# peterarmstrong/corda

Hardware: AMD Instinct MI355X
Metric: verified sigs/sec (whole node), Ed25519 + ECDSA-P256, at 1/2/4/8 MI355X (higher is better)
Workload: dtype u32

## Files before the change

corda_amd/csrc/cordagpu.cpp:

```cpp
#include <hip/hip_runtime.h>

#include <algorithm>
#include <atomic>
#include <chrono>
#include <cmath>
#include <cstdio>
#include <cstring>
#include <functional>
#include <initializer_list>
#include <memory>
#include <mutex>
#include <string>
#include <thread>
#include <vector>

#include "../../include/cordagpu.h"
#include "call_scope.h"
#include "engine.h"
#include "host_budget.h"
#include "host_pool.h"
#include "pool.h"
#include "rsa.h"
#include "table_budget.h"
#include "txsig_plan.h"
// ... 21 lines not shown
  snprintf(buf, sizeof buf, "%s: %s", where, hipGetErrorString(e));
  g_err = buf;
  return e == hipErrorOutOfMemory ? CG_ERR_NOMEM : CG_ERR_DEVICE;
}

#define HIP_TRY(expr, where)               \
  do {                                     \
    hipError_t _e = (expr);                \
    if (_e != hipSuccess) return hip_fail(_e, where); \
  } while (0)

bool env_flag(const char* name, bool dflt) {
  const char* v = getenv(name);
  return v ? (dflt ? v[0] != '0' : v[0] == '1') : dflt;
}
uint64_t env_u64(const char* name, uint64_t dflt) {
  const char* v = getenv(name);
  return v ? (uint64_t)strtoull(v, nullptr, 10) : dflt;
}

struct DevBuf {
  void* p = nullptr;
  size_t cap = 0;
  hipError_t ensure(size_t bytes) { return bytes <= cap ? hipSuccess : replace(bytes + bytes / 4 + 256); }
  hipError_t ensure_exact(size_t bytes) { return bytes <= cap ? hipSuccess : replace(bytes); }
  hipError_t replace(size_t want) {
    release();
    const hipError_t e = hipMalloc(&p, want);
    if (e == hipSuccess) cap = want;
    return e;
  }
  void release() {
    if (p) hipFree(p);
    p = nullptr;
    cap = 0;
  }
};

struct Need {
  DevBuf* buf;
  size_t bytes;
};
hipError_t ensure_all(std::initializer_list<Need> needs) {
  bool grow = false;
  for (const Need& n : needs) grow = grow || n.buf->cap < n.bytes;
  if (!grow) return hipSuccess;
  hipError_t e = hipDeviceSynchronize();
  for (const Need& n : needs)
    if (e == hipSuccess) e = n.buf->ensure(n.bytes);
  return e;
}

hipError_t stage(DevBuf& b, const void* src, size_t bytes, hipStream_t s, size_t room = 0) {
  hipError_t e = b.ensure(std::max<size_t>({bytes, room, 1}));
  if (e == hipSuccess && bytes) e = hipMemcpyAsync(b.p, src, bytes, hipMemcpyHostToDevice, s);
  return e;
}
size_t arena_room(uint64_t arena_len) { return ((arena_len + 3) & ~(uint64_t)3) + 16; }

struct HipStreams {
  using Stream = hipStream_t;
  using Event = hipEvent_t;
  using Error = hipError_t;
  static constexpr Error kOk = hipSuccess;
  Error record(Event e, Stream s) { return hipEventRecord(e, s); }
  Error wait(Stream s, Event e) { return hipStreamWaitEvent(s, e, 0); }
  Error sync(Stream s) { return hipStreamSynchronize(s); }
};

}

struct cg_ctx : cg::CallState<HipStreams> {
  int device = 0;
  uint64_t chunk = CG_DEFAULT_CHUNK_ITEMS;
  bool chunk_set = false;
  bool fault = false;
  cg::Fork fork = {{nullptr, nullptr, nullptr}, nullptr, {nullptr, nullptr, nullptr}, nullptr,
                   {nullptr, nullptr, nullptr}, nullptr};
  std::mutex mu;
  DevBuf keyprep, itemws, keys, items, arena, status, aux0, aux1, aux2;
  void* btab = nullptr;
  const cgt::EngineVariant* eng = nullptr;
  uint64_t tab_bytes = 0;
  DevBuf wide;
  bool rsa = false;
  DevBuf rsakeys, rsalist;
  uint32_t wide_max = cg::kKeyWideMax;
  DevBuf kcache;
  uint32_t wide_slots = 0;
  uint32_t wide_slots_max = cg::kKeyWideMax;
  uint32_t kc_bits = 32;
  bool kc_on = true;
  bool kc_dirty = true;
  bool kc_open = false;
  DevBuf txitems, msgs, tmpls, h_txs, h_comps, h_sigs, h_ids, h_txst;
  DevBuf sig12ws;
  DevBuf txvws, txvio;
  DevBuf ftxws;
  DevBuf signers, signws;
  uint32_t n_signers = 0;
  hipStream_t copy2 = nullptr;
  cg::CountScratch count_scratch;
  std::unique_ptr<cg::HostPool> hpool;
  uint32_t host_req = 0;
  uint32_t quota = 1;
  bool counted = false;
  std::vector<hipEvent_t> seg;
  hipEvent_t tev[4] = {};
  std::vector<hipEvent_t> segt;
  std::vector<hipEvent_t> segtab;
  hipEvent_t backt[2] = {nullptr, nullptr};
  std::vector<hipEvent_t> fbt;
  std::vector<double> fbh;
  bool htrace = false;
  cg::StageTimer timer;
};

namespace {

std::atomic<unsigned> g_live_ctx{0};

const cgt::EngineVariant* const kVariants[] = {&cg::variant(), &cg24::variant(), &cg22::variant()};
constexpr int kNumVariants = 3;

std::vector<cgb::TableSet> table_sets() {
  std::vector<cgb::TableSet> v;
  for (const cgt::EngineVariant* e : kVariants) v.push_back({e->fixed_base_bits, (uint64_t)e->btab_bytes()});
  return v;
}

struct SharedTables {
  int device;
  int variant;
  void* p;
  unsigned refs;
};
std::mutex g_tab_mu;
std::vector<SharedTables> g_tabs;

hipError_t acquire_tables(int device, hipStream_t s, uint64_t budget, void** out, int* variant) {
  std::lock_guard<std::mutex> g(g_tab_mu);
  const std::vector<cgb::TableSet> sets = table_sets();
  int held = -1;
  for (const SharedTables& t : g_tabs)
    if (t.device == device && (held < 0 || t.variant < held)) held = t.variant;
  size_t free_b = 0, total_b = 0;
  if (hipMemGetInfo(&free_b, &total_b) != hipSuccess) free_b = 0;
  const int pick = cgb::pick_tables(sets.data(), kNumVariants, budget, free_b, held);
  if (pick < 0) return hipErrorInvalidValue;
  for (SharedTables& t : g_tabs)
    if (t.device == device && t.variant == pick) {
      ++t.refs;
      *out = t.p;
      *variant = pick;
      return hipSuccess;
    }
  hipError_t e = hipErrorOutOfMemory;
  for (int v = pick; v < kNumVariants; ++v) {
    if (budget && sets[v].bytes > budget) continue;
    void* p = nullptr;
    e = hipMalloc(&p, sets[v].bytes);
    if (e == hipSuccess) {
      DevBuf scratch;
      e = scratch.ensure(kVariants[v]->btab_scratch_bytes());
      if (e == hipSuccess) e = kVariants[v]->upload_constants();
      if (e == hipSuccess) e = kVariants[v]->init_btab(p, scratch.p, s);
      if (e == hipSuccess) e = hipStreamSynchronize(s);
      scratch.release();
      if (e == hipSuccess) {
        g_tabs.push_back({device, v, p, 1u});
        *out = p;
        *variant = v;
        return hipSuccess;
      }
      hipFree(p);
    }
    (void)hipGetLastError();
    if (e != hipErrorOutOfMemory || budget) break;
  }
  return e;
}

void release_tables(int device, void* p) {
  std::lock_guard<std::mutex> g(g_tab_mu);
  for (size_t i = 0; i < g_tabs.size(); ++i)
    if (g_tabs[i].device == device && g_tabs[i].p == p) {
      if (--g_tabs[i].refs == 0) {
        hipSetDevice(device);
        hipFree(p);
        g_tabs.erase(g_tabs.begin() + (ptrdiff_t)i);
      }
      return;
    }
}

unsigned host_threads_of(cg_ctx* c, uint64_t n) {
  if (n < (1u << 16)) return 1;
  const unsigned nt = cg::host_threads_for(c->host_req, cg::host_threads_env(), c->quota, g_live_ctx.load());
  if (nt <= 1) c->hpool.reset();
  else if (!c->hpool || c->hpool->threads() != nt) c->hpool.reset(new cg::HostPool(nt - 1));
  return nt;
}

void host_par(cg_ctx* c, uint64_t m, const std::function<void(uint64_t)>& fn) {
  if (m > 1 && c->hpool) {
    c->hpool->run(m, fn);
  } else {
    for (uint64_t t = 0; t < m; ++t) fn(t);
  }
}

HipStreams g_hip;
struct Call : cg::CallScope<HipStreams> {
  Call(cg_ctx* c, Form form) : CallScope(g_hip, *c, form) {}
  hipError_t open(void* hip_stream = nullptr) { return CallScope::open((hipStream_t)hip_stream); }
};

int enter(cg_ctx* c, const char* fn) {
  if (c->fault) return fail(CG_ERR_DEVICE, "%s: device fault (injected by cg_pool_inject_fault)", fn);
  HIP_TRY(hipSetDevice(c->device), "hipSetDevice");
  return CG_OK;
}

uint64_t chunk_of(const cg_ctx* c, uint64_t n) { return cg::equal_chunk(c->chunk, n); }

size_t item_half_bytes(const cg_ctx* c, uint64_t ws_items) { return (c->eng->item_ws_bytes(ws_items) + 255) & ~(size_t)255; }
hipError_t ensure_rsa(cg_ctx* c, uint32_t n_keys, uint64_t n_items) {
  if (!c->rsa) return hipSuccess;
  return ensure_all({{&c->rsakeys, cg::rsa_keys_bytes(n_keys)}, {&c->rsalist, cg::rsa_list_bytes(n_items)}});
}
hipError_t rsa_keyprep(cg_ctx* c, const cg::VerifyReq& r, hipStream_t s) {
  if (!c->rsa) return hipSuccess;
  return cg::launch_rsa_keyprep(r, c->rsakeys.p, s);
}
hipError_t rsa_items(cg_ctx* c, const cg::VerifyReq& r, hipStream_t s) {
  if (!c->rsa || r.n_items == 0) return hipSuccess;
  return cg::launch_rsa_items(r, c->rsakeys.p, c->rsalist.p, s);
}

hipError_t ensure_ws(cg_ctx* c, uint32_t n_keys, uint64_t ws_items, uint64_t call_items = 0) {
  {
    const hipError_t re = ensure_rsa(c, n_keys, call_items > ws_items ? call_items : ws_items);
    if (re != hipSuccess) return re;
  }
  const uint32_t kmax = c->wide_slots_max;
  size_t wide = c->eng->wide_bytes(n_keys, call_items, kmax);
  const size_t items = item_half_bytes(c, ws_items) * (call_items > ws_items ? 2 : 1);
  if (c->keyprep.cap >= c->eng->keyprep_bytes(n_keys) && c->itemws.cap >= items && c->wide.cap >= wide) {
    c->wide_max = kmax;
    return hipSuccess;
  }
  uint32_t cap = kmax;
  if (wide > c->wide.cap) {
    size_t free_b = 0, total_b = 0;
    if (hipMemGetInfo(&free_b, &total_b) == hipSuccess) {
      const size_t need_other = (c->keyprep.cap >= c->eng->keyprep_bytes(n_keys) ? 0 : c->eng->keyprep_bytes(n_keys)) +
                                (c->itemws.cap >= items ? 0 : items);
      const size_t avail = free_b + c->wide.cap;
      const size_t spare = (size_t)1 << 30;
      if (wide + need_other + spare > avail) {
        const size_t room = avail > need_other + spare ? avail - need_other - spare : 0;
        cap = (uint32_t)std::min<size_t>(room / c->eng->wide_slot_bytes(), kmax);
        wide = c->eng->wide_bytes(n_keys, call_items, cap);
      }
    }
  }
  c->wide_max = cap;
  if (c->keyprep.cap >= c->eng->keyprep_bytes(n_keys) && c->itemws.cap >= items && c->wide.cap >= wide)
    return hipSuccess;
  hipError_t e = hipDeviceSynchronize();
  if (e == hipSuccess) e = c->keyprep.ensure(c->eng->keyprep_bytes(n_keys));
  if (e == hipSuccess) e = c->itemws.ensure(items);
  if (e == hipSuccess && wide > c->wide.cap) {
    e = c->wide.ensure_exact(wide);
    c->wide_slots = e == hipSuccess ? c->eng->wide_slots(n_keys, call_items, cap) : 0;
    c->kc_dirty = true;
    if (e == hipSuccess && c->kc_on) e = c->kcache.ensure(c->eng->key_cache_bytes(c->wide_slots));
  }
  return e;
}

cg::WidePool wide_for(cg_ctx* c, uint32_t n_keys, uint64_t n_items) {
  if (c->wide.cap < c->eng->wide_bytes(n_keys, n_items, c->wide_max)) return cg::WidePool{};
  cg::WidePool p = c->eng->make_wide_pool(c->wide.p, n_keys, n_items, c->wide_max, c->wide_slots);
  if (c->kc_on && p.cap_ed && c->kcache.p && c->kcache.cap >= c->eng->key_cache_bytes(p.slots)) {
    if (c->kc_open) {
      (void)hipDeviceSynchronize();
      c->kc_dirty = true;
    }
    p.cache = c->kcache.p;
    p.cache_bits = c->kc_bits;
    p.cache_dirty = c->kc_dirty;
    c->kc_dirty = false;
    c->kc_open = true;
  }
  static const uint32_t min_ed = (uint32_t)env_u64("CG_WIDE_MIN_USES_ED", 0);
  static const uint32_t min_ec = (uint32_t)env_u64("CG_WIDE_MIN_USES_EC", 0);
  if (min_ed) p.min_ed = min_ed;
  if (min_ec) p.min_ec = min_ec;
  return p;
}

struct ChunkOpts {
  const std::function<hipError_t(uint64_t, uint64_t, uint64_t)>* prepare = nullptr;
  const cg::KeyUses* uses = nullptr;
  bool prepare_blocks = false;
};

struct CallEng {
  using Error = hipError_t;
  static constexpr Error kOk = hipSuccess;
  using Clock = std::chrono::steady_clock;
  cg_ctx* c;
  const cg::VerifyReq& r;
  hipStream_t s;
  const cg::WidePool* wp;
  const std::vector<uint64_t>& bounds;
  const ChunkOpts& o;
  uint64_t half_bytes = 0;
  bool closes_cache = true;
  Clock::time_point h0;
  double prep_ms = 0, front_ms = 0, back_ms = 0;
  const char* where = "launch_items";

  static double ms(Clock::time_point a, Clock::time_point b) { return std::chrono::duration<double, std::milli>(b - a).count(); }
  cg::ItemArgs chunk(unsigned k, int half) const {
    cg::ItemArgs a = {r, c->keyprep.p, c->itemws.p, c->btab, wp};
    a.d_items = r.d_items + bounds[k];
    a.n_items = bounds[k + 1] - bounds[k];
    a.d_status = r.d_status + bounds[k];
    a.d_item_ws = (uint8_t*)c->itemws.p + (size_t)half * half_bytes;
    return a;
  }
  Error at(const char* w, Error e) {
    if (e != hipSuccess) where = w;
    return e;
  }
  Error keyprep() { return at("launch_keyprep", c->eng->launch_keyprep(r, c->keyprep.p, s, c->fork, wp, o.uses)); }
  Error rsa_keyprep() { return at("launch_rsa_keyprep", ::rsa_keyprep(c, r, s)); }
  Error key_tables() { return c->eng->launch_key_tables(c->fork, s); }
  Error prepare(unsigned k) {
    h0 = Clock::now();
    const hipError_t w = (*o.prepare)(k, bounds[k], bounds[k + 1] - bounds[k]);
    prep_ms = ms(h0, Clock::now());
    return w;
  }
  Error plan(unsigned k, int half) { return c->eng->launch_items_plan(chunk(k, half), s, c->fork); }
  Error front(unsigned k, int half, bool planned) {
    if (!o.prepare) h0 = Clock::now();
    const hipError_t e = c->eng->launch_items_front(chunk(k, half), s, c->fork, planned);
    front_ms = ms(h0, Clock::now());
    return e;
  }
  Error back(unsigned k, int half) {
    const auto h1 = Clock::now();
    if (k == 0 && c->htrace && c->backt[0]) {
      hipEventRecord(c->backt[0], s);
      hipStream_t t = c->copy2;
      for (int q = 0; q < 3; ++q) hipStreamWaitEvent(t, c->fork.ready[q], 0);
      hipEventRecord(c->backt[1], t);
    }
    c->fork.mark = c->htrace && 3 * (size_t)k + 2 < c->fbt.size() ? c->fbt[3 * k + 2] : nullptr;
    const hipError_t x = c->eng->launch_items_back(chunk(k, half), s, c->fork);
    c->fork.mark = nullptr;
    if (c->htrace && 3 * (size_t)k + 1 < c->fbt.size()) hipEventRecord(c->fbt[3 * k + 1], s);
    back_ms = ms(h1, Clock::now());
    return x;
  }
  void chunk_enqueued(unsigned k) const {
    if (c->htrace)
      fprintf(stderr, "[cg host] chunk %llu enqueue: front %.3f ms (prepare %.3f, with the copies), back %.3f ms\n",
              (unsigned long long)k, front_ms, prep_ms, back_ms);
  }
  Error rsa_pass(Error x) {
    if (x == hipSuccess && closes_cache) c->kc_open = false;
    return x != hipSuccess ? x : at("launch_rsa_items", rsa_items(c, r, s));
  }
  Error wait(cgs::Stream, cgs::Event e) {
    return at("hipStreamWaitEvent", hipStreamWaitEvent(s, c->fork.ready[e - cgs::EV_READY0], 0));
  }
};

hipError_t launch_chunked(cg_ctx* c, const cg::VerifyReq& r, const std::vector<uint64_t>& bounds, hipStream_t s,
                          const ChunkOpts& o) {
  if (r.n_items == 0) return hipSuccess;
  const cg::WidePool wp = wide_for(c, r.n_keys, r.n_items);
  const uint64_t per = cg::largest_chunk(bounds);
  CallEng g = {c, r, s, &wp, bounds, o};
  g.half_bytes = item_half_bytes(c, per);
  cgs::CallPlan p;
  p.chunks = (unsigned)(bounds.size() - 1);
  p.two = p.chunks > 1 && c->itemws.cap >= 2 * g.half_bytes;
  p.hook = o.prepare != nullptr;
  p.hook_blocks = o.prepare_blocks;
  return cgs::chunked(g, p);
}

using cg::Extent;

struct HostPlan {
  std::vector<uint64_t> first;
  std::vector<Extent> ext;
  Extent keys, win;
};

void plan_host(cg_ctx* c, const cg_key* keys, uint32_t n_keys, const cg_item* items, uint64_t n_items,
               uint64_t arena_len, uint64_t per, HostPlan& P) {
  for (uint32_t k = 0; k < n_keys; ++k) P.keys.add(keys[k].off, keys[k].len, arena_len);
  const uint64_t nch = (n_items + per - 1) / per;
  P.first.resize(nch + 1);
  for (uint64_t k = 0; k <= nch; ++k) P.first[k] = n_items * k / nch;
  P.ext.assign(nch, Extent());
  auto scan = [&](uint64_t k) {
    Extent x;
    for (uint64_t i = P.first[k]; i < P.first[k + 1]; ++i) {
      x.add(items[i].sig_off, items[i].sig_len, arena_len);
      x.add(items[i].msg_off, items[i].msg_len, arena_len);
    }
    P.ext[k] = x;
  };
  host_threads_of(c, n_items);
  host_par(c, nch, scan);
  P.win = P.keys;
  for (const Extent& e : P.ext) P.win.merge(e);
  if (P.win.empty()) P.win.lo = P.win.hi = 0;
  P.win.lo &= ~(uint64_t)15;
}

hipError_t copy_missing(cg::Resident& have, const Extent& e, const uint8_t* arena, uint8_t* dwin, uint64_t win_lo,
                        hipStream_t s) {
  for (const auto& g : have.missing(e)) {
    hipError_t r = hipMemcpyAsync(dwin + (g.first - win_lo), arena + g.first, g.second - g.first,
                                  hipMemcpyHostToDevice, s);
    if (r != hipSuccess) return r;
  }
  return hipSuccess;
}

hipError_t ensure_events(std::vector<hipEvent_t>& v, uint64_t n) {
  while (v.size() < n) {
    hipEvent_t e;
    const hipError_t r = hipEventCreateWithFlags(&e, hipEventDisableTiming);
    if (r != hipSuccess) return r;
    v.push_back(e);
  }
  return hipSuccess;
}

void fill_stats(cg_ctx* c, cg_stats* stats, uint64_t n_items, uint32_t n_keys, double ms_key_prep,
                std::chrono::steady_clock::time_point t0) {
  if (!stats) return;
  float a = 0, b = 0, d = 0;
  hipEventElapsedTime(&a, c->tev[0], c->tev[1]);
  hipEventElapsedTime(&b, c->tev[1], c->tev[2]);
  hipEventElapsedTime(&d, c->tev[2], c->tev[3]);
  stats->n_items = n_items;
  stats->n_keys = n_keys;
  stats->ms_h2d = a;
  stats->ms_key_prep = ms_key_prep;
  stats->ms_verify = b;
  stats->ms_d2h = d;
  stats->ms_total = std::chrono::duration<double, std::milli>(std::chrono::steady_clock::now() - t0).count();
}

int verify_host_locked(cg_ctx* c, const cg::VerifyReq& h, cg_stats* stats) {
  const auto t0 = std::chrono::steady_clock::now();
  if (const int rc = enter(c, "cg_verify_batch")) return rc;
  const uint32_t n_keys = h.n_keys;
  const uint64_t n_items = h.n_items;
  const uint64_t pipe = c->chunk < CG_PIPELINE_CHUNK_ITEMS ? c->chunk : CG_PIPELINE_CHUNK_ITEMS;
  HostPlan P;
  plan_host(c, h.d_keys, n_keys, h.d_items, n_items, h.arena_len, pipe, P);
  const uint64_t nch = P.ext.size();
  const uint64_t per_max = (n_items + nch - 1) / nch;
  HIP_TRY(c->keys.ensure(sizeof(cg_key) * (n_keys ? n_keys : 1)), "hipMalloc(keys)");
  HIP_TRY(c->items.ensure(sizeof(cg_item) * n_items), "hipMalloc(items)");
  HIP_TRY(c->arena.ensure((P.win.hi - P.win.lo) + 16), "hipMalloc(arena window)");
  HIP_TRY(c->status.ensure(n_items), "hipMalloc(status)");
  HIP_TRY(ensure_ws(c, n_keys, per_max, n_items), "hipMalloc(workspace)");
  HIP_TRY(ensure_events(c->seg, nch), "hipEventCreate");
  hipStream_t s = c->stream;
  uint8_t* dwin = (uint8_t*)c->arena.p;
  Call call(c, Call::kHost);
  HIP_TRY(call.open(), "hipStreamWaitEvent");
  HIP_TRY(hipEventRecord(c->tev[0], s), "hipEventRecord");
  HIP_TRY(hipStreamWaitEvent(c->copy, c->tev[0], 0), "hipStreamWaitEvent");
  cg::Resident have;
  if (n_keys)
    HIP_TRY(hipMemcpyAsync(c->keys.p, h.d_keys, sizeof(cg_key) * n_keys, hipMemcpyHostToDevice, c->copy), "H2D keys");
  HIP_TRY(copy_missing(have, P.keys, h.d_arena, dwin, P.win.lo, c->copy), "H2D key bytes");
  HIP_TRY(hipMemcpyAsync(c->items.p, h.d_items, sizeof(cg_item) * n_items, hipMemcpyHostToDevice, c->copy), "H2D items");
  HIP_TRY(hipEventRecord(c->seg[0], c->copy), "hipEventRecord");
  HIP_TRY(hipStreamWaitEvent(s, c->seg[0], 0), "hipStreamWaitEvent");
  cg::VerifyReq d = h;
  d.d_keys = (const cg_key*)c->keys.p;
  d.d_items = (const cg_item*)c->items.p;
  d.d_arena = dwin - P.win.lo;
  d.d_status = (uint8_t*)c->status.p;
  const cg::WidePool wp = wide_for(c, n_keys, n_items);
  HIP_TRY(c->eng->launch_keyprep(d, c->keyprep.p, s, c->fork, &wp, nullptr), "launch_keyprep");
  cg::ItemArgs a = {d, c->keyprep.p, c->itemws.p, c->btab, &wp};
  HIP_TRY(rsa_keyprep(c, d, s), "launch_rsa_keyprep");
  for (uint64_t k = 0; k < nch; ++k) {
    HIP_TRY(copy_missing(have, P.ext[k], h.d_arena, dwin, P.win.lo, c->copy), "H2D arena");
    HIP_TRY(hipEventRecord(c->seg[k], c->copy), "hipEventRecord");
    HIP_TRY(hipStreamWaitEvent(s, c->seg[k], 0), "hipStreamWaitEvent");
    if (k == 0) HIP_TRY(hipEventRecord(c->tev[1], s), "hipEventRecord");
    a.d_items = d.d_items + P.first[k];
    a.n_items = P.first[k + 1] - P.first[k];
    a.d_status = d.d_status + P.first[k];
    HIP_TRY(c->eng->launch_items(a, s, c->fork), "launch_items");
  }
  c->kc_open = false;
  HIP_TRY(rsa_items(c, d, s), "launch_rsa_items");
  HIP_TRY(hipEventRecord(c->tev[2], s), "hipEventRecord");
  HIP_TRY(hipMemcpyAsync(h.d_status, d.d_status, n_items, hipMemcpyDeviceToHost, s), "D2H status");
  HIP_TRY(hipEventRecord(c->tev[3], s), "hipEventRecord");
  HIP_TRY(call.close(), "hipEventRecord");
  HIP_TRY(hipStreamSynchronize(s), "hipStreamSynchronize");
  fill_stats(c, stats, n_items, n_keys, 0, t0);
  return CG_OK;
}

int batch_args(const char* fn, const cg::VerifyReq& r, bool host) {
  if (r.n_items && (!r.d_items || !r.d_status)) return fail(CG_ERR_ARG, "%s: NULL buffer", fn);
  if (host && r.n_keys && !r.d_keys) return fail(CG_ERR_ARG, "%s: keys is NULL", fn);
  if (host && r.arena_len && !r.d_arena) return fail(CG_ERR_ARG, "%s: arena is NULL", fn);
  if (r.mode > CG_MODE_ISVALID) return fail(CG_ERR_ARG, "%s: bad mode", fn);
  return CG_OK;
}

}

extern "C" {

int cg_abi_version(void) { return CG_ABI_VERSION; }

const char* cg_build_info(void) {
  return "corda_amd libcordagpu: HIP kernels for gfx950 (Ed25519 i2p-0.2.0 semantics, ECDSA BC-1.57 semantics, "
         "SHA-256/512, Merkle tx ids)";
}

int cg_device_count(void) {
  int n = 0;
  if (hipGetDeviceCount(&n) != hipSuccess) return 0;
  return n;
}

const char* cg_last_error(void) { return g_err.c_str(); }

namespace {
struct HostRange {
  uint64_t lo, hi;
};
std::mutex g_reg_mu;
std::vector<HostRange> g_reg;
}

int cg_host_register(const void* p, uint64_t len) {
  if (!p || !len) return fail(CG_ERR_ARG, "cg_host_register: NULL pointer or empty range");
  const uint64_t lo = (uint64_t)(uintptr_t)p, hi = lo + len;
  if (hi < lo) return fail(CG_ERR_ARG, "cg_host_register: range wraps the address space");
  std::lock_guard<std::mutex> g(g_reg_mu);
  for (const HostRange& r : g_reg)
    if (lo < r.hi && r.lo < hi) return fail(CG_ERR_ARG, "cg_host_register: range overlaps a registered one");
  HIP_TRY(hipHostRegister(const_cast<void*>(p), (size_t)len, hipHostRegisterPortable), "hipHostRegister");
  g_reg.push_back({lo, hi});
  return CG_OK;
}

int cg_host_unregister(const void* p) {
  const uint64_t lo = (uint64_t)(uintptr_t)p;
  std::lock_guard<std::mutex> g(g_reg_mu);
  for (size_t i = 0; i < g_reg.size(); ++i) {
    if (g_reg[i].lo != lo) continue;
    g_reg.erase(g_reg.begin() + (ptrdiff_t)i);
    HIP_TRY(hipHostUnregister(const_cast<void*>(p)), "hipHostUnregister");
    return CG_OK;
  }
  return fail(CG_ERR_ARG, "cg_host_unregister: pointer was not registered");
}

int cg_host_register_advised(uint32_t contexts_per_node) { return cg::host_register_advised(contexts_per_node) ? 1 : 0; }

int cg_host_registered(const void* p, uint64_t len) {
  const uint64_t lo = (uint64_t)(uintptr_t)p, hi = lo + len;
  std::lock_guard<std::mutex> g(g_reg_mu);
  for (const HostRange& r : g_reg)
    if (lo >= r.lo && hi <= r.hi && hi >= lo) return 1;
  return 0;
}

static_assert(sizeof(cg_config) == 56, "cg_config is 56 bytes in ABI v2");
static_assert(sizeof(cg_item) == 32 && sizeof(cg_key) == 16 && sizeof(cg_txsig) == 24 && sizeof(cg_txsig_packed) == 12,
              "ABI struct sizes");

int cg_open(cg_ctx** out, const cg_config* cfg) {
  if (!out) return fail(CG_ERR_ARG, "cg_open: out is NULL");
  *out = nullptr;
  if (cfg && (cfg->reserved0 || cfg->reserved1))
    return fail(CG_ERR_ARG, "cg_open: cg_config.reserved must be 0 (ABI v2: 56-byte cg_config)");
  const uint64_t tab_budget = cfg && cfg->table_bytes_max ? cfg->table_bytes_max
                                                          : cgb::table_bytes_env(getenv("CG_TABLE_BYTES_MAX"));
  if (tab_budget && tab_budget < table_sets().back().bytes) {
    char m[160];
    snprintf(m, sizeof m, "cg_open: table_bytes_max %llu is below the smallest fixed-base tables (%llu bytes, radix 2^%u)",
             (unsigned long long)tab_budget, (unsigned long long)table_sets().back().bytes, table_sets().back().bits);
    return fail(CG_ERR_ARG, "%s", m);
  }
  if (cfg && (cfg->flags & ~(CG_FLAG_STAGE_TIMING | CG_FLAG_RSA | CG_FLAG_NO_KEY_CACHE))) return fail(CG_ERR_ARG, "cg_open: unknown cg_config.flags bits");
  int dev = cfg ? cfg->device : 0;
  int n = 0;
  HIP_TRY(hipGetDeviceCount(&n), "hipGetDeviceCount");
  if (dev < 0 || dev >= n) return fail(CG_ERR_ARG, "cg_open: device ordinal out of range");
  HIP_TRY(hipSetDevice(dev), "hipSetDevice");
  hipDeviceProp_t prop;
  HIP_TRY(hipGetDeviceProperties(&prop, dev), "hipGetDeviceProperties");
  if (strncmp(prop.gcnArchName, "gfx950", 6) != 0)
    return fail(CG_ERR_DEVICE, "cg_open: kernels are built for gfx950, device is %s", prop.gcnArchName);
  cg_ctx* c = new cg_ctx();
  c->device = dev;
  c->host_req = cfg ? cfg->host_threads : 0u;
  c->quota = cg::cpu_quota();
  if (cfg && cfg->chunk_items) {
    c->chunk = cfg->chunk_items;
    c->chunk_set = true;
  }
  if (cfg && (cfg->flags & CG_FLAG_STAGE_TIMING)) c->fork.timer = &c->timer;
  c->rsa = cfg && (cfg->flags & CG_FLAG_RSA);
  c->kc_on = !(cfg && (cfg->flags & CG_FLAG_NO_KEY_CACHE)) && env_flag("CG_KEY_CACHE", true);
  c->wide_slots_max = (uint32_t)std::min<uint64_t>(env_u64("CG_TEST_WIDE_SLOTS", cg::kKeyWideMax), cg::kKeyWideMax);
  c->kc_bits = (uint32_t)std::min<uint64_t>(env_u64("CG_TEST_KEY_CACHE_BITS", 32), 32);
  hipError_t e = hipStreamCreateWithFlags(&c->stream, hipStreamNonBlocking);
  if (e != hipSuccess) {
    delete c;
    return hip_fail(e, "hipStreamCreate");
  }
  for (int k = 0; k < 3 && e == hipSuccess; ++k) e = hipStreamCreateWithFlags(&c->fork.side[k], hipStreamNonBlocking);
  if (e == hipSuccess) e = hipEventCreateWithFlags(&c->fork.start, hipEventDisableTiming);
  for (int k = 0; k < 3 && e == hipSuccess; ++k) e = hipEventCreateWithFlags(&c->fork.ready[k], hipEventDisableTiming);
  for (int k = 0; k < 3 && e == hipSuccess; ++k) e = hipEventCreateWithFlags(&c->fork.row0[k], hipEventDisableTiming);
  if (e == hipSuccess) e = hipEventCreateWithFlags(&c->fork.front, hipEventDisableTiming);
  if (e == hipSuccess) e = hipEventCreateWithFlags(&c->fork.planned, hipEventDisableTiming);
  if (e == hipSuccess) e = hipEventCreateWithFlags(&c->fork.ec_front_go, hipEventDisableTiming);
  for (int k = 0; k < 2 && e == hipSuccess; ++k)
    e = hipEventCreateWithFlags(&c->fork.ec_front_done[k], hipEventDisableTiming);
  {
    hipDeviceProp_t prop;
    const bool own = hipGetDeviceProperties(&prop, c->device) == hipSuccess && prop.multiProcessorCount > 0;
    std::vector<uint32_t> mask(own ? (prop.multiProcessorCount + 31) / 32 : 0, 0u);
    for (int cu = 0; own && cu < prop.multiProcessorCount; ++cu) mask[cu / 32] |= 1u << (cu % 32);
    for (hipStream_t* cs : {&c->copy, &c->copy2})
      if (e == hipSuccess)
        e = own ? hipExtStreamCreateWithCUMask(cs, (uint32_t)mask.size(), mask.data())
                : hipStreamCreateWithFlags(cs, hipStreamNonBlocking);
  }
  for (int k = 0; k < 4 && e == hipSuccess; ++k) e = hipEventCreate(&c->tev[k]);
  if (e == hipSuccess) e = hipEventCreateWithFlags(&c->done, hipEventDisableTiming);
  if (e == hipSuccess) e = hipEventCreateWithFlags(&c->bridge, hipEventDisableTiming);
  c->bridged = env_flag("CG_STREAM_BRIDGE", true);
  int var = 0;
  if (e == hipSuccess) e = acquire_tables(c->device, c->stream, tab_budget, &c->btab, &var);
  if (e == hipSuccess) {
    c->eng = kVariants[var];
    c->tab_bytes = c->eng->btab_bytes();
    e = c->eng->upload_constants();
  }
  if (e == hipSuccess) e = hipStreamSynchronize(c->stream);
  if (e != hipSuccess) {
    const int rc = hip_fail(e, "side streams / upload_constants / fixed-base tables");
    cg_close(c);
    return rc;
  }
  c->counted = true;
  ++g_live_ctx;
  *out = c;
  return CG_OK;
}

static void signers_drop(cg_ctx* c) {
  c->n_signers = 0;
  if (!c->signers.p) return;
  (void)hipDeviceSynchronize();
  (void)hipMemset(c->signers.p, 0, c->signers.cap);
  (void)hipDeviceSynchronize();
  c->signers.release();
}

void cg_close(cg_ctx* c) {
  if (!c) return;
  if (c->counted) --g_live_ctx;
  hipSetDevice(c->device);
  if (c->stream) hipStreamSynchronize(c->stream);
  signers_drop(c);
  c->signws.release();
// ... 198 lines not shown
  HIP_TRY(cgs::verify_items(items, (unsigned)(bounds.size() - 1)), items.where);
  HIP_TRY(call.close(), "hipEventRecord");
  return CG_OK;
}

int cg_verify_batch(cg_ctx* c, const cg_key* keys, uint32_t n_keys, const cg_item* items, uint64_t n_items,
                    const uint8_t* arena, uint64_t arena_len, uint32_t mode, uint8_t* status_out,
                    cg_stats* stats) {
  if (!c) return fail(CG_ERR_ARG, "cg_verify_batch: ctx is NULL");
  const cg::VerifyReq h = {keys, n_keys, items, n_items, arena, arena_len, mode, status_out};
  if (const int a = batch_args("cg_verify_batch", h, true)) return a;
  if (n_items) memset(status_out, CG_NOT_RUN, n_items);
  if (n_items == 0) return CG_OK;
  std::lock_guard<std::mutex> g(c->mu);
  const int rc = verify_host_locked(c, h, stats);
  if (rc != CG_OK) memset(status_out, CG_NOT_RUN, n_items);
  return rc;
}

int cg_sha256_batch_device(cg_ctx* c, const cg_span* d_spans, uint64_t n, const uint8_t* d_arena,
                           uint64_t arena_len, uint8_t* d_digests, void* hip_stream) {
  if (!c) return fail(CG_ERR_ARG, "cg_sha256_batch_device: ctx is NULL");
  std::lock_guard<std::mutex> g(c->mu);
  if (const int rc = enter(c, "cg_sha256_batch_device")) return rc;
  Call call(c, Call::kDevice);
  HIP_TRY(call.open(hip_stream), "hipStreamWaitEvent");
  HIP_TRY(cg::launch_sha256(d_spans, n, d_arena, arena_len, d_digests, call.stream()), "launch_sha256");
  HIP_TRY(call.close(), "hipEventRecord");
  return CG_OK;
}

static int hash_batch(cg_ctx* c, const cg_span* spans, uint64_t n, const uint8_t* arena, uint64_t arena_len,
                      uint8_t* out, int which) {
  if (!c) return fail(CG_ERR_ARG, "hash batch: ctx is NULL");
  if (n && (!spans || !out)) return fail(CG_ERR_ARG, "hash batch: NULL buffer");
  if (n == 0) return CG_OK;
  const size_t dlen = which == 256 ? 32 : 64;
  std::lock_guard<std::mutex> g(c->mu);
  if (const int rc = enter(c, which == 256 ? "cg_sha256_batch" : "cg_sha512_batch")) return rc;
  hipStream_t s = c->stream;
  Call call(c, Call::kHost);
  HIP_TRY(call.open(), "hipStreamWaitEvent");
  HIP_TRY(stage(c->items, spans, sizeof(cg_span) * n, s), "H2D spans");
  HIP_TRY(stage(c->arena, arena, arena_len, s, arena_room(arena_len)), "H2D arena");
  HIP_TRY(c->aux0.ensure(dlen * n), "hipMalloc(digests)");
  HIP_TRY((which == 256 ? cg::launch_sha256 : cg::launch_sha512)((const cg_span*)c->items.p, n, (const uint8_t*)c->arena.p,
                                                                 arena_len, (uint8_t*)c->aux0.p, s), "launch_sha");
  HIP_TRY(hipMemcpyAsync(out, c->aux0.p, dlen * n, hipMemcpyDeviceToHost, s), "D2H digests");
  HIP_TRY(call.close(), "hipEventRecord");
  HIP_TRY(hipStreamSynchronize(s), "hipStreamSynchronize");
  return CG_OK;
}

int cg_sha256_batch(cg_ctx* c, const cg_span* spans, uint64_t n, const uint8_t* arena, uint64_t arena_len,
                    uint8_t* out) {
  return hash_batch(c, spans, n, arena, arena_len, out, 256);
}
int cg_sha512_batch(cg_ctx* c, const cg_span* spans, uint64_t n, const uint8_t* arena, uint64_t arena_len,
                    uint8_t* out) {
  return hash_batch(c, spans, n, arena, arena_len, out, 512);
}

int cg_tx_ids_device(cg_ctx* c, const cg_tx* d_txs, uint64_t n_tx, const cg_component* d_comps, uint64_t n_comps,
                     const uint8_t* d_arena, uint64_t arena_len, uint8_t* d_ids, uint8_t* d_status,
                     void* hip_stream) {
  if (!c) return fail(CG_ERR_ARG, "cg_tx_ids_device: ctx is NULL");
  std::lock_guard<std::mutex> g(c->mu);
  if (const int rc = enter(c, "cg_tx_ids_device")) return rc;
  HIP_TRY(ensure_all({{&c->aux2, cg::tx_ws_bytes(n_comps)}}), "hipMalloc(leaf ws)");
  Call call(c, Call::kDevice);
  HIP_TRY(call.open(hip_stream), "hipStreamWaitEvent");
  HIP_TRY(cg::launch_tx_ids(d_txs, n_tx, d_comps, n_comps, d_arena, arena_len, d_ids, d_status,
                            (uint8_t*)c->aux2.p, call.stream()), "launch_tx_ids");
  HIP_TRY(call.close(), "hipEventRecord");
  return CG_OK;
}

int cg_tx_ids(cg_ctx* c, const cg_tx* txs, uint64_t n_tx, const cg_component* comps, uint64_t n_comps,
              const uint8_t* arena, uint64_t arena_len, uint8_t* ids_out, uint8_t* status_out) {
  if (!c) return fail(CG_ERR_ARG, "cg_tx_ids: ctx is NULL");
  if (n_tx && (!txs || !ids_out || !status_out)) return fail(CG_ERR_ARG, "cg_tx_ids: NULL buffer");
  if (n_tx == 0) return CG_OK;
  std::lock_guard<std::mutex> g(c->mu);
  if (const int rc = enter(c, "cg_tx_ids")) return rc;
  hipStream_t s = c->stream;
  Call call(c, Call::kHost);
  HIP_TRY(call.open(), "hipStreamWaitEvent");
  HIP_TRY(stage(c->keys, txs, sizeof(cg_tx) * n_tx, s), "H2D txs");
  HIP_TRY(stage(c->items, comps, sizeof(cg_component) * n_comps, s), "H2D comps");
  HIP_TRY(stage(c->arena, arena, arena_len, s, arena_room(arena_len)), "H2D arena");
  HIP_TRY(c->aux0.ensure(32 * n_tx), "hipMalloc(ids)");
  HIP_TRY(c->status.ensure(n_tx), "hipMalloc(status)");
  HIP_TRY(c->aux2.ensure(cg::tx_ws_bytes(n_comps)), "hipMalloc(leaf ws)");
  HIP_TRY(cg::launch_tx_ids((const cg_tx*)c->keys.p, n_tx, (const cg_component*)c->items.p, n_comps,
                            (const uint8_t*)c->arena.p, arena_len, (uint8_t*)c->aux0.p, (uint8_t*)c->status.p,
                            (uint8_t*)c->aux2.p, s), "launch_tx_ids");
  HIP_TRY(hipMemcpyAsync(ids_out, c->aux0.p, 32 * n_tx, hipMemcpyDeviceToHost, s), "D2H ids");
  HIP_TRY(hipMemcpyAsync(status_out, c->status.p, n_tx, hipMemcpyDeviceToHost, s), "D2H status");
  HIP_TRY(call.close(), "hipEventRecord");
  HIP_TRY(hipStreamSynchronize(s), "hipStreamSynchronize");
  return CG_OK;
}

int cg_merkle_roots(cg_ctx* c, const uint8_t* leaves, const uint64_t* first, const uint32_t* count, uint64_t n,
                    uint8_t* roots_out, uint8_t* status_out) {
  if (!c) return fail(CG_ERR_ARG, "cg_merkle_roots: ctx is NULL");
  if (n && (!first || !count || !roots_out || !status_out)) return fail(CG_ERR_ARG, "cg_merkle_roots: NULL buffer");
  if (n == 0) return CG_OK;
  uint64_t total = 0, ws = 0;
  std::vector<uint64_t> wsoff(n);
  for (uint64_t j = 0; j < n; ++j) {
    if (first[j] + count[j] > total) total = first[j] + count[j];
    wsoff[j] = ws;
    ws += count[j];
  }
  std::lock_guard<std::mutex> g(c->mu);
  if (const int rc = enter(c, "cg_merkle_roots")) return rc;
  hipStream_t s = c->stream;
  Call call(c, Call::kHost);
  HIP_TRY(call.open(), "hipStreamWaitEvent");
  HIP_TRY(stage(c->arena, leaves, 32 * total, s), "H2D leaves");
  HIP_TRY(stage(c->keys, first, 8 * n, s), "H2D first");
  HIP_TRY(stage(c->items, count, 4 * n, s), "H2D count");
  HIP_TRY(stage(c->aux2, wsoff.data(), 8 * n, s), "H2D wsoff");
  HIP_TRY(c->aux0.ensure(32 * n), "hipMalloc(roots)");
  HIP_TRY(c->status.ensure(n), "hipMalloc(status)");
  HIP_TRY(c->aux1.ensure(32 * (ws ? ws : 1)), "hipMalloc(ws)");
  HIP_TRY(cg::launch_merkle_roots((const uint8_t*)c->arena.p, (const uint64_t*)c->keys.p, (const uint32_t*)c->items.p,
                                  n, (uint8_t*)c->aux0.p, (uint8_t*)c->status.p, (uint8_t*)c->aux1.p,
                                  (const uint64_t*)c->aux2.p, s),
          "launch_merkle_roots");
  HIP_TRY(hipMemcpyAsync(roots_out, c->aux0.p, 32 * n, hipMemcpyDeviceToHost, s), "D2H roots");
  HIP_TRY(hipMemcpyAsync(status_out, c->status.p, n, hipMemcpyDeviceToHost, s), "D2H status");
  HIP_TRY(call.close(), "hipEventRecord");
  HIP_TRY(hipStreamSynchronize(s), "hipStreamSynchronize");
  return CG_OK;
}

static uint64_t tmpl_slot(const cg_signable_tmpl* tmpls, uint32_t n_tmpls) {
  uint64_t maxlen = 0;
  for (uint32_t k = 0; k < n_tmpls; ++k) {
    const uint64_t l = (uint64_t)tmpls[k].prefix_len + 32u + tmpls[k].suffix_len;
    if (l > maxlen) maxlen = l;
  }
  const uint64_t slot = (maxlen + 15) & ~(uint64_t)15;
  return slot ? slot : 16;
}

struct TxnReq {
  const cg_tx* txs;
  uint64_t n_tx;
  const cg_component* comps;
  uint64_t n_comps;
  const cg_key* keys;
  uint32_t n_keys;
  const cg_txsig* sigs;
  uint64_t n_sigs;
  const cg_signable_tmpl* tmpls;
  uint32_t n_tmpls;
  const uint8_t* arena;
  uint64_t arena_len;
  uint32_t mode;
  uint8_t *ids, *tx_status, *sig_status;
};
static int txn_args(const char* fn, const TxnReq& q, bool host) {
  if (q.n_tx && (!q.txs || !q.ids || !q.tx_status)) return fail(CG_ERR_ARG, "%s: NULL tx buffer", fn);
  if (q.n_sigs && (!q.sigs || !q.sig_status)) return fail(CG_ERR_ARG, "%s: NULL sig buffer", fn);
  if (host && q.n_comps && !q.comps) return fail(CG_ERR_ARG, "%s: comps is NULL", fn);
  if (host && q.n_keys && !q.keys) return fail(CG_ERR_ARG, "%s: keys is NULL", fn);
  if (q.n_tmpls && !q.tmpls) return fail(CG_ERR_ARG, "%s: templates is NULL", fn);
  if (host && q.arena_len && !q.arena) return fail(CG_ERR_ARG, "%s: arena is NULL", fn);
  if (q.mode > CG_MODE_ISVALID) return fail(CG_ERR_ARG, "%s: bad mode", fn);
  return CG_OK;
}

static int verify_transactions_locked(cg_ctx* c, const TxnReq& d, hipStream_t s) {
  const uint64_t slot = tmpl_slot(d.tmpls, d.n_tmpls), msgs_len = cg::tx_msgs_head(d.n_tmpls, slot);
  HIP_TRY(ensure_all({{&c->aux2, cg::tx_ws_bytes(d.n_comps)},
                      {&c->txitems, sizeof(cg_item) * (d.n_sigs ? d.n_sigs : 1)},
                      {&c->msgs, msgs_len ? msgs_len : 16},
                      {&c->tmpls, sizeof(cg_signable_tmpl) * (d.n_tmpls ? d.n_tmpls : 1)}}),
          "hipMalloc(transaction workspace)");
  HIP_TRY(ensure_ws(c, d.n_keys, chunk_of(c, d.n_sigs), d.n_sigs), "hipMalloc(workspace)");
  if (d.n_tmpls)
    HIP_TRY(hipMemcpyAsync(c->tmpls.p, d.tmpls, sizeof(cg_signable_tmpl) * d.n_tmpls, hipMemcpyHostToDevice, s),
            "H2D templates");
  HIP_TRY(cg::launch_tx_ids(d.txs, d.n_tx, d.comps, d.n_comps, d.arena, d.arena_len, d.ids, d.tx_status,
                            (uint8_t*)c->aux2.p, s), "launch_tx_ids");
  if (d.n_sigs) {
    HIP_TRY(cg::launch_tx_sig_items(d.sigs, d.n_sigs, (const cg_signable_tmpl*)c->tmpls.p, d.n_tmpls, d.tx_status,
                                    d.n_tx, d.ids, d.arena, d.arena_len, slot, (cg_item*)c->txitems.p,
                                    (uint8_t*)c->msgs.p, s),
            "launch_tx_sig_items");
    const cg::VerifyReq r = {d.keys, d.n_keys, (const cg_item*)c->txitems.p, d.n_sigs, d.arena, d.arena_len, d.mode,
                             d.sig_status, (const uint8_t*)c->msgs.p, msgs_len};
    HIP_TRY(launch_chunked(c, r, cg::equal_bounds(d.n_sigs, chunk_of(c, d.n_sigs)), s, ChunkOpts{}), "launch_verify");
  }
  return CG_OK;
}

int cg_verify_transactions_device(cg_ctx* c, const cg_tx* d_txs, uint64_t n_tx, const cg_component* d_comps,
                                  uint64_t n_comps, const cg_key* d_keys, uint32_t n_keys, const cg_txsig* d_sigs,
                                  uint64_t n_sigs, const cg_signable_tmpl* tmpls, uint32_t n_tmpls,
                                  const uint8_t* d_arena, uint64_t arena_len, uint32_t mode, uint8_t* d_ids,
                                  uint8_t* d_tx_status, uint8_t* d_sig_status, void* hip_stream) {
  if (!c) return fail(CG_ERR_ARG, "cg_verify_transactions_device: ctx is NULL");
  const TxnReq d = {d_txs, n_tx,  d_comps,   n_comps, d_keys, n_keys, d_sigs,      n_sigs,
                    tmpls, n_tmpls, d_arena, arena_len, mode, d_ids,  d_tx_status, d_sig_status};
  if (const int a = txn_args("cg_verify_transactions_device", d, false)) return a;
  std::lock_guard<std::mutex> g(c->mu);
  if (const int rc = enter(c, "cg_verify_transactions_device")) return rc;
  Call call(c, Call::kDevice);
  HIP_TRY(call.open(hip_stream), "hipStreamWaitEvent");
  if (const int rc = verify_transactions_locked(c, d, call.stream())) return rc;
  HIP_TRY(call.close(), "hipEventRecord");
  return CG_OK;
}

static int verify_transactions_host_locked(cg_ctx* c, const TxnReq& h) {
  if (const int rc = enter(c, "cg_verify_transactions")) return rc;
  hipStream_t s = c->stream;
  Call call(c, Call::kHost);
  HIP_TRY(call.open(), "hipStreamWaitEvent");
  HIP_TRY(stage(c->h_txs, h.txs, sizeof(cg_tx) * h.n_tx, s), "H2D txs");
  HIP_TRY(stage(c->h_comps, h.comps, sizeof(cg_component) * h.n_comps, s), "H2D comps");
  HIP_TRY(stage(c->keys, h.keys, sizeof(cg_key) * h.n_keys, s), "H2D keys");
  HIP_TRY(stage(c->h_sigs, h.sigs, sizeof(cg_txsig) * h.n_sigs, s), "H2D sigs");
  HIP_TRY(stage(c->arena, h.arena, h.arena_len, s, arena_room(h.arena_len)), "H2D arena");
  HIP_TRY(c->h_ids.ensure(32 * (h.n_tx ? h.n_tx : 1)), "hipMalloc(ids)");
  HIP_TRY(c->h_txst.ensure(h.n_tx ? h.n_tx : 1), "hipMalloc(tx status)");
  HIP_TRY(c->status.ensure(h.n_sigs ? h.n_sigs : 1), "hipMalloc(sig status)");
  TxnReq d = h;
  d.txs = (const cg_tx*)c->h_txs.p;
  d.comps = (const cg_component*)c->h_comps.p;
  d.keys = (const cg_key*)c->keys.p;
  d.sigs = (const cg_txsig*)c->h_sigs.p;
  d.arena = (const uint8_t*)c->arena.p;
  d.ids = (uint8_t*)c->h_ids.p;
  d.tx_status = (uint8_t*)c->h_txst.p;
  d.sig_status = (uint8_t*)c->status.p;
  if (const int rc = verify_transactions_locked(c, d, s)) return rc;
  if (h.n_tx) {
    HIP_TRY(hipMemcpyAsync(h.ids, d.ids, 32 * h.n_tx, hipMemcpyDeviceToHost, s), "D2H ids");
    HIP_TRY(hipMemcpyAsync(h.tx_status, d.tx_status, h.n_tx, hipMemcpyDeviceToHost, s), "D2H tx status");
  }
  if (h.n_sigs) HIP_TRY(hipMemcpyAsync(h.sig_status, d.sig_status, h.n_sigs, hipMemcpyDeviceToHost, s), "D2H sig status");
  HIP_TRY(call.close(), "hipEventRecord");
  HIP_TRY(hipStreamSynchronize(s), "hipStreamSynchronize");
  return CG_OK;
}

int cg_verify_transactions(cg_ctx* c, const cg_tx* txs, uint64_t n_tx, const cg_component* comps, uint64_t n_comps,
                           const cg_key* keys, uint32_t n_keys, const cg_txsig* sigs, uint64_t n_sigs,
                           const cg_signable_tmpl* tmpls, uint32_t n_tmpls, const uint8_t* arena,
                           uint64_t arena_len, uint32_t mode, uint8_t* ids_out, uint8_t* tx_status_out,
                           uint8_t* sig_status_out) {
  if (!c) return fail(CG_ERR_ARG, "cg_verify_transactions: ctx is NULL");
  const TxnReq h = {txs,   n_tx,    comps, n_comps,   keys, n_keys,  sigs,          n_sigs,
                    tmpls, n_tmpls, arena, arena_len, mode, ids_out, tx_status_out, sig_status_out};
  if (const int a = txn_args("cg_verify_transactions", h, true)) return a;
  for (uint64_t i = 0; i < n_sigs; ++i) sig_status_out[i] = CG_NOT_RUN;
  if (n_tx == 0 && n_sigs == 0) return CG_OK;
  std::lock_guard<std::mutex> g(c->mu);
  return verify_transactions_host_locked(c, h);
}

static hipError_t ensure_txsig_ws(cg_ctx* c, uint64_t n_sigs, uint32_t n_tmpls, uint64_t slot) {
  return ensure_all({{&c->txitems, sizeof(cg_item) * (n_sigs ? n_sigs : 1)},
                     {&c->msgs, cg::tx_msgs_head(n_tmpls, slot)},
                     {&c->tmpls, sizeof(cg_signable_tmpl) * (n_tmpls ? n_tmpls : 1)}});
}

struct TxsigReq {
  const cg_key* keys;
  uint32_t n_keys;
  const uint8_t* ids;
  uint64_t n_ids;
  cg::SigTable sigs;
  uint64_t n_sigs;
  const cg_signable_tmpl* tmpls;
  uint32_t n_tmpls;
  const uint8_t* arena;
  uint64_t arena_len;
  uint32_t mode;
  uint8_t* status;
  const uint8_t* sig_bytes = nullptr;
  uint64_t sig_bytes_off = 0, sig_bytes_len = 0;
};

struct TxsigSched {
  const std::vector<uint64_t>& bounds;
  cg::KeyUses uses;
  const std::function<hipError_t(uint64_t, uint64_t, uint64_t)>* ready = nullptr;
  const std::vector<uint64_t>* chunk_base = nullptr;
  const uint64_t* d_bases = nullptr;
};
static hipError_t launch_txsig(cg_ctx* c, const TxsigReq& d, uint64_t slot, const TxsigSched& p, hipStream_t s) {
  if (d.n_sigs == 0) return hipSuccess;
  hipError_t e = hipSuccess;
  const cg_signable_tmpl* dt = (const cg_signable_tmpl*)c->tmpls.p;
  if (d.n_tmpls) e = hipMemcpyAsync(c->tmpls.p, d.tmpls, sizeof(cg_signable_tmpl) * d.n_tmpls, hipMemcpyHostToDevice, s);
  if (e == hipSuccess)
    e = cg::launch_tx_sig_templates(dt, d.n_tmpls, d.arena, d.arena_len, slot, d.ids, d.n_ids, (uint8_t*)c->msgs.p, s);
  const std::function<hipError_t(uint64_t, uint64_t, uint64_t)> prepare = [&](uint64_t k, uint64_t first,
                                                                               uint64_t cnt) {
    hipError_t r = p.ready ? (*p.ready)(k, first, cnt) : hipSuccess;
    if (r == hipSuccess && d.sigs.packed())
      r = cg::launch_tx_sig12_range((const cg_txsig_packed*)d.sigs.p, first, cnt, d.sig_bytes_off, d.sig_bytes_len,
                                    p.chunk_base ? (*p.chunk_base)[k] : 0, p.d_bases, dt, d.n_tmpls, d.n_ids,
                                    d.arena_len, (cg_item*)c->txitems.p, c->sig12ws.p, s);
    else if (r == hipSuccess)
      r = cg::launch_tx_sig_range((const cg_txsig*)d.sigs.p, first, cnt, dt, d.n_tmpls, nullptr, d.n_ids, d.ids,
                                  d.arena_len, slot, (cg_item*)c->txitems.p, (uint8_t*)c->msgs.p, s);
    return r;
  };
  const cg::VerifyReq r = {d.keys, d.n_keys, (const cg_item*)c->txitems.p, d.n_sigs, d.arena, d.arena_len, d.mode,
                           d.status, (const uint8_t*)c->msgs.p, cg::tx_msgs_head(d.n_tmpls, slot)};
  if (e == hipSuccess) e = launch_chunked(c, r, p.bounds, s, ChunkOpts{&prepare, &p.uses, p.ready != nullptr});
  return e;
}

static double ms_since(std::chrono::steady_clock::time_point t0) {
  return std::chrono::duration<double, std::milli>(std::chrono::steady_clock::now() - t0).count();
}

struct HostTrace {
  cg_ctx* c;
  const std::chrono::steady_clock::time_point t0;
  const bool on;
  std::vector<double> ht;

  double ms() const { return on ? ms_since(t0) : 0; }
  hipError_t begin(uint64_t nch) {
    c->htrace = on;
    if (!on) return hipSuccess;
    hipError_t e = hipSuccess;
    for (int q = 0; q < 2 && e == hipSuccess; ++q)
      if (!c->backt[q]) e = hipEventCreate(&c->backt[q]);
    while (e == hipSuccess && c->fbt.size() < 3 * nch) {
      hipEvent_t ev;
      e = hipEventCreate(&ev);
      if (e == hipSuccess) c->fbt.push_back(ev);
    }
    c->fbh.assign(nch, 0.0);
    ht.assign(3 * nch, 0.0);
    return e;
  }
  void table_staged(uint64_t k, double h0, double h1) {
    if (!on) return;
    ht[3 * k] = h0;
    ht[3 * k + 1] = h1 - h0;
    ht[3 * k + 2] = ms() - h1;
  }
  hipError_t bytes_staged(uint64_t k, hipStream_t cs, double h2, double h3, double table_mb, const Extent& ek) {
    if (!on) return hipSuccess;
    hipError_t e = hipSuccess;
    while (c->segt.size() <= k) {
      hipEvent_t ev;
      if (hipEventCreate(&ev) != hipSuccess) break;
      c->segt.push_back(ev);
    }
    if (c->segt.size() > k) e = hipEventRecord(c->segt[k], cs);
    fprintf(stderr, "[cg host] chunk %llu at %.3f: scan %.3f sigs %.3f (%.1f MB) ids %.3f arena %.3f (%.1f MB) ms\n",
            (unsigned long long)k, ht[3 * k], ht[3 * k + 1], ht[3 * k + 2], table_mb, h3 - h2, ms() - h3,
            ek.empty() ? 0.0 : (ek.hi - ek.lo) / 1e6);
    return e;
  }
  hipError_t front_reached(uint64_t k, hipStream_t s) {
    if (!on || 3 * k >= c->fbt.size()) return hipSuccess;
    c->fbh[k] = ms();
    return hipEventRecord(c->fbt[3 * k], s);
  }
  void report(uint64_t nch, double h_enq) {
    if (!on) return;
    fprintf(stderr, "[cg host] enqueued at %.3f, done at %.3f ms; copies landed (device ms after the call's first event):",
            h_enq, ms());
    for (uint64_t k = 0; k < nch && k < c->segt.size(); ++k) {
      float t = 0;
      hipEventElapsedTime(&t, c->tev[0], c->segt[k]);
      fprintf(stderr, " %.3f", t);
    }
    float t = 0, f0 = 0, tb = 0;
    hipEventElapsedTime(&t, c->tev[0], c->tev[2]);
    hipEventElapsedTime(&f0, c->tev[0], c->backt[0]);
    hipEventElapsedTime(&tb, c->tev[0], c->backt[1]);
    fprintf(stderr, "; chunk 0 front done %.3f, tables built %.3f, verify done %.3f\n", f0, tb, t);
    for (uint64_t k = 0; k < nch && 3 * k + 2 < c->fbt.size(); ++k) {
      float fs = 0, be = 0, bj = 0;
      hipEventElapsedTime(&fs, c->tev[0], c->fbt[3 * k]);
      hipEventElapsedTime(&bj, c->tev[0], c->fbt[3 * k + 2]);
      hipEventElapsedTime(&be, c->tev[0], c->fbt[3 * k + 1]);
      fprintf(stderr, "[cg host] chunk %llu: front enqueued (host) %.3f, front reached (device) %.3f, back's "
              "kernels done %.3f, joins done %.3f\n", (unsigned long long)k, c->fbh[k], fs, bj, be);
    }
  }
};

struct TxsigFeed {
  cg_ctx* c;
  HostTrace& tr;
  const std::vector<uint64_t>& bounds;
  const TxsigReq& h;
  const TxsigReq& d;
  const uint64_t nt;
  const cg::ParFor& par;
  std::vector<Extent> ext_e, ext_i;
  std::vector<uint64_t> cbase;
  cg::Resident have, have_ids, have_sig;
  hipError_t copy_err = hipSuccess;
  uint64_t mid_k = 0;
  const std::function<hipError_t()> mid_hook = [this] { return mid(); };
  const std::function<hipError_t(uint64_t, uint64_t, uint64_t)> before_hook = [this](uint64_t k, uint64_t, uint64_t) {
    return before(k);
  };

  TxsigFeed(cg_ctx* ctx, HostTrace& trace, const std::vector<uint64_t>& b, const TxsigReq& host, const TxsigReq& dev,
            uint64_t threads, const cg::ParFor& pf)
      : c(ctx), tr(trace), bounds(b), h(host), d(dev), nt(threads), par(pf), ext_e(b.size() - 1),
        ext_i(b.size() - 1), cbase(b.size(), 0) {}
  TxsigFeed(const TxsigFeed&) = delete;
  ~TxsigFeed() { c->fork.mid_front = nullptr; }

  hipError_t copy_table(uint64_t k) {
    const uint64_t first = bounds[k], cnt = bounds[k + 1] - bounds[k];
    const double h0 = tr.ms();
    const cg::ChunkScan x = cg::with_records(h.sigs, [&](auto* recs) {
      return cg::scan_chunk(recs, first, first + cnt, h.n_ids, d.arena_len, nt, par);
    });
    ext_e[k] = x.sig;
    ext_i[k] = x.ids;
    if (h.sigs.packed()) {
      cbase[k + 1] = cbase[k] + x.span;
      ext_e[k] = Extent();
      ext_e[k].add(cbase[k], x.span, h.sig_bytes_len);
    }
    const double h1 = tr.ms();
    const hipError_t e = hipMemcpyAsync((uint8_t*)c->h_sigs.p + (size_t)h.sigs.stride * first, h.sigs.from(first).p,
                                        (size_t)h.sigs.stride * cnt, hipMemcpyHostToDevice, c->copy);
    tr.table_staged(k, h0, h1);
    return e;
  }
  hipError_t copy_bytes(uint64_t k) {
    const Extent& ek = ext_e[k];
    uint8_t* dwin = (uint8_t*)c->arena.p;
    const double h2 = tr.ms();
    hipError_t e = copy_missing(have_ids, ext_i[k], h.ids, (uint8_t*)c->h_ids.p, 0, c->copy);
    const double h3 = tr.ms();
    if (e == hipSuccess && h.sigs.packed()) e = copy_missing(have_sig, ek, h.sig_bytes, dwin + d.sig_bytes_off, 0, c->copy);
    else if (e == hipSuccess) e = copy_missing(have, ek, h.arena, dwin, 0, c->copy);
    if (e == hipSuccess) e = hipEventRecord(c->seg[k], c->copy);
    if (e == hipSuccess) e = tr.bytes_staged(k, c->copy, h2, h3, h.sigs.stride * (bounds[k + 1] - bounds[k]) / 1e6, ek);
    return e;
  }
  hipError_t mid() {
    c->fork.mid_front = nullptr;
    const uint64_t k = mid_k;
    hipStream_t s = c->stream;
    hipError_t e = copy_bytes(k);
    if (e == hipSuccess) e = hipStreamWaitEvent(s, c->seg[k], 0);
    if (e == hipSuccess) e = tr.front_reached(k, s);
    if (e == hipSuccess && k == 0) e = hipEventRecord(c->tev[1], s);
    if (e != hipSuccess) copy_err = e;
    return e;
  }
  hipError_t before(uint64_t k) {
    hipStream_t s = c->stream;
    hipError_t e = c->fork.mid_front ? mid() : hipSuccess;
    if (e == hipSuccess) e = copy_table(k);
    if (e == hipSuccess) e = hipEventRecord(c->segtab[k], c->copy);
    if (e == hipSuccess) e = hipStreamWaitEvent(s, c->segtab[k], 0);
    if (e == hipSuccess) {
      mid_k = k;
      c->fork.mid_front = &mid_hook;
    }
    if (e != hipSuccess) copy_err = e;
    return e;
  }
};

static hipError_t txv_stage(cg_ctx* c, const cg::TxvSet& h, uint32_t n_keys, cg::TxvSet* d) {
  auto up = [](size_t x) { return (x + 15) & ~(size_t)15; };
  const size_t o_checks = 0, o_nodes = o_checks + up(sizeof(cg_tx_check) * h.n_tx),
               o_verd = o_nodes + up(sizeof(cg_req_node) * h.n_nodes),
               o_reqs = o_verd + up(sizeof(cg_tx_verdict) * h.n_tx),
               o_class = o_reqs + up(sizeof(uint32_t) * h.n_reqs),
               o_rst = o_class + up(h.key_class ? sizeof(uint32_t) * n_keys : 0), need = o_rst + up(h.n_reqs) + 16;
  const hipError_t e = ensure_all({{&c->txvws, cg::tx_verdicts_ws_bytes(h.n_tx)}, {&c->txvio, need}});
  if (e != hipSuccess) return e;
  uint8_t* b = (uint8_t*)c->txvio.p;
  *d = h;
  d->checks = (cg_tx_check*)(b + o_checks);
  d->nodes = (cg_req_node*)(b + o_nodes);
  d->verdicts = (cg_tx_verdict*)(b + o_verd);
  d->reqs = (uint32_t*)(b + o_reqs);
  d->key_class = h.key_class ? (uint32_t*)(b + o_class) : nullptr;
  d->req_status = b + o_rst;
  return hipSuccess;
}
static hipError_t txv_upload(const cg::TxvSet& h, uint32_t n_keys, const cg::TxvSet& d, hipStream_t s) {
  hipError_t e = hipSuccess;
  if (h.n_tx) e = hipMemcpyAsync((void*)d.checks, h.checks, sizeof(cg_tx_check) * h.n_tx, hipMemcpyHostToDevice, s);
  if (e == hipSuccess && h.n_nodes)
    e = hipMemcpyAsync((void*)d.nodes, h.nodes, sizeof(cg_req_node) * h.n_nodes, hipMemcpyHostToDevice, s);
  if (e == hipSuccess && h.n_reqs)
    e = hipMemcpyAsync((void*)d.reqs, h.reqs, sizeof(uint32_t) * h.n_reqs, hipMemcpyHostToDevice, s);
  if (e == hipSuccess && h.key_class && n_keys)
    e = hipMemcpyAsync((void*)d.key_class, h.key_class, sizeof(uint32_t) * n_keys, hipMemcpyHostToDevice, s);
  return e;
}
static hipError_t txv_download(const cg::TxvSet& h, const cg::TxvSet& d, hipStream_t s) {
  hipError_t e = hipSuccess;
  if (h.n_tx) e = hipMemcpyAsync(h.verdicts, d.verdicts, sizeof(cg_tx_verdict) * h.n_tx, hipMemcpyDeviceToHost, s);
  if (e == hipSuccess && h.n_reqs) e = hipMemcpyAsync(h.req_status, d.req_status, h.n_reqs, hipMemcpyDeviceToHost, s);
  return e;
}
static void txv_fill_not_run(const cg::TxvSet& h) {
  for (uint64_t t = 0; t < h.n_tx; ++t) h.verdicts[t] = cg_tx_verdict{0xFFFFFFFFu, CG_NOT_RUN, CG_TXV_SPAN_BAD, 0};
  if (h.n_reqs) memset(h.req_status, CG_REQ_HOST, h.n_reqs);
}

static int verify_txsig_host_locked(cg_ctx* c, const TxsigReq& q, cg_stats* stats, const cg::TxvSet* txv) {
  const auto t0 = std::chrono::steady_clock::now();
  const bool packed = q.sigs.packed();
  const uint32_t n_keys = q.n_keys, n_tmpls = q.n_tmpls;
  const uint64_t n_sigs = q.n_sigs, n_ids = q.n_ids;
  TxsigReq h = q;
  TxsigReq d = q;
  d.sig_bytes_off = packed ? ((q.arena_len + 15) & ~(uint64_t)15) : 0;
  if (packed) d.arena_len = d.sig_bytes_off + q.sig_bytes_len;
  std::vector<cg_key> keys_fix;
  std::vector<cg_signable_tmpl> tmpls_fix;
  if (packed) {
    cg::txsig_packed_fixup(q.keys, n_keys, q.tmpls, n_tmpls, q.arena_len, keys_fix, tmpls_fix);
    if (!keys_fix.empty()) h.keys = keys_fix.data();
    if (!tmpls_fix.empty()) h.tmpls = tmpls_fix.data();
  }
  d.tmpls = h.tmpls;
  if (const int rc = enter(c, "cg_verify_tx_signatures")) return rc;
  static const uint64_t first_div = env_u64("CG_TXSIG_FIRST_DIV", cg::kTxsigFirstDiv);
  const std::vector<uint64_t> bounds = cg::txsig_bounds(n_sigs, c->chunk, c->chunk_set, first_div);
  const uint64_t nch = bounds.size() - 1, per = cg::largest_chunk(bounds);
  const Extent head = cg::txsig_head_extent(h.keys, n_keys, h.tmpls, n_tmpls, q.arena_len);
  const uint64_t nt = host_threads_of(c, n_sigs);
  const cg::ParFor par = [c](uint64_t m, const std::function<void(uint64_t)>& fn) { host_par(c, m, fn); };
  std::vector<uint32_t> counts(n_keys ? n_keys : 1, 0u);
  const uint64_t slot = tmpl_slot(h.tmpls, n_tmpls);
  HIP_TRY(c->keys.ensure(sizeof(cg_key) * (n_keys ? n_keys : 1)), "hipMalloc(keys)");
  HIP_TRY(c->h_sigs.ensure(q.sigs.stride * n_sigs), "hipMalloc(sigs)");
  if (packed) HIP_TRY(c->sig12ws.ensure(cg::tx_sig12_scratch_bytes(per)), "hipMalloc(signature offsets)");
  HIP_TRY(c->aux1.ensure(sizeof(uint32_t) * counts.size()), "hipMalloc(key use counts)");
  HIP_TRY(c->h_ids.ensure(32 * (n_ids ? n_ids : 1)), "hipMalloc(ids)");
  HIP_TRY(c->arena.ensure(d.arena_len + 16), "hipMalloc(arena window)");
  HIP_TRY(c->status.ensure(n_sigs), "hipMalloc(status)");
  HIP_TRY(ensure_txsig_ws(c, n_sigs, n_tmpls, slot), "hipMalloc(tx signature workspace)");
  HIP_TRY(ensure_ws(c, n_keys, per, n_sigs), "hipMalloc(workspace)");
  cg::TxvSet txd;
  if (txv) HIP_TRY(txv_stage(c, *txv, n_keys, &txd), "hipMalloc(verdict tables)");
  HIP_TRY(ensure_events(c->seg, nch + 1), "hipEventCreate");
  HIP_TRY(ensure_events(c->segtab, nch), "hipEventCreate");
  static const bool htrace = env_flag("CG_HOST_TRACE", false);
  HostTrace tr{c, t0, htrace, {}};
  HIP_TRY(tr.begin(nch), "hipEventCreate");
  hipStream_t s = c->stream;
  d.keys = (const cg_key*)c->keys.p;
  d.ids = (const uint8_t*)c->h_ids.p;
  d.sigs.p = c->h_sigs.p;
  d.arena = (const uint8_t*)c->arena.p;
  d.status = (uint8_t*)c->status.p;
  Call call(c, Call::kHost);
  HIP_TRY(call.open(), "hipStreamWaitEvent");
  HIP_TRY(hipEventRecord(c->tev[0], s), "hipEventRecord");
  HIP_TRY(hipStreamWaitEvent(c->copy, c->tev[0], 0), "hipStreamWaitEvent");
  TxsigFeed feed(c, tr, bounds, h, d, nt, par);
  if (n_keys)
    HIP_TRY(hipMemcpyAsync(c->keys.p, h.keys, sizeof(cg_key) * n_keys, hipMemcpyHostToDevice, c->copy), "H2D keys");
  HIP_TRY(copy_missing(feed.have, head, h.arena, (uint8_t*)c->arena.p, 0, c->copy), "H2D key / template bytes");
  {
    static const uint32_t S_env = cg::sample_override((uint32_t)env_u64("CG_TXSIG_SAMPLE", 0));
    static const uint32_t B = cg::sample_block((uint32_t)env_u64("CG_TXSIG_SAMPLE_BLOCK", cg::kTxsigSampleBlock));
    const uint32_t S = cg::sample_rate(S_env, n_sigs, n_keys);
    const cg::WidePool thr = c->eng->make_wide_pool(nullptr, n_keys, n_sigs, cg::kKeyWideMax, 0);
    cg::with_records(h.sigs, [&](auto* recs) {
      cg::key_use_counts(recs, n_sigs, h.keys, n_keys, nt, par, S, B, thr.min_ed, thr.min_ec, c->count_scratch,
                         counts.data());
    });
  }
  const double ms_plan = ms_since(t0);
  HIP_TRY(hipMemcpyAsync(c->aux1.p, counts.data(), sizeof(uint32_t) * counts.size(), hipMemcpyHostToDevice, c->copy),
          "H2D key use counts");
  HIP_TRY(hipEventRecord(c->seg[nch], c->copy), "hipEventRecord");
  HIP_TRY(hipStreamWaitEvent(s, c->seg[nch], 0), "hipStreamWaitEvent");
  TxsigSched sched{bounds, {}, &feed.before_hook, packed ? &feed.cbase : nullptr, nullptr};
  sched.uses.counts = (const uint32_t*)c->aux1.p;
  sched.uses.n = n_sigs;
  sched.uses.host_keys = h.keys;
  sched.uses.host_counts = counts.data();
  const hipError_t le = launch_txsig(c, d, slot, sched, s);
  if (le == hipSuccess && c->fork.mid_front) feed.mid();
  if (feed.copy_err != hipSuccess) return hip_fail(feed.copy_err, "H2D signature bytes");
  HIP_TRY(le, "launch_txsig");
  if (txv) {
    HIP_TRY(txv_upload(*txv, n_keys, txd, c->copy), "H2D verdict tables");
    HIP_TRY(hipEventRecord(c->seg[nch], c->copy), "hipEventRecord");
    HIP_TRY(hipStreamWaitEvent(s, c->seg[nch], 0), "hipStreamWaitEvent");
    HIP_TRY(cg::launch_tx_verdicts(d.sigs, n_sigs, d.status, d.keys, n_keys, txd, c->txvws.p, s), "launch_tx_verdicts");
  }
  HIP_TRY(hipEventRecord(c->tev[2], s), "hipEventRecord");
  if (q.status) HIP_TRY(hipMemcpyAsync(q.status, d.status, n_sigs, hipMemcpyDeviceToHost, s), "D2H status");
  if (txv) HIP_TRY(txv_download(*txv, txd, s), "D2H verdicts");
  HIP_TRY(hipEventRecord(c->tev[3], s), "hipEventRecord");
  HIP_TRY(call.close(), "hipEventRecord");
  const double h_enq = tr.ms();
  HIP_TRY(hipStreamSynchronize(s), "hipStreamSynchronize");
  tr.report(nch, h_enq);
  fill_stats(c, stats, n_sigs, n_keys, ms_plan, t0);
  return CG_OK;
// ... 794 lines not shown
```

corda_amd/csrc/engine.h:

```cpp
#pragma once
#include <functional>
#include <stdlib.h>
#include <hip/hip_runtime.h>
#include <stdint.h>

#include <vector>

#include "../../include/cordagpu.h"
#include "launch_schedule.h"

namespace cgt {


struct DeviceConsts;
struct WidePool {
  void* ed = nullptr;
  void* ec = nullptr;
  uint32_t cap_ed = 0, cap_ec = 0;
  uint32_t min_ed = 0, min_ec = 0;
  uint32_t slots = 0;
  void* cache = nullptr;
  uint32_t cache_bits = 32;
  bool cache_dirty = false;
};

struct StageTimer {
  struct Rec {
    int stage;
    hipEvent_t a, b;
  };
  static constexpr size_t kMaxRecs = 4096;
  std::vector<Rec> recs, spare;
  int mark(int stage, hipStream_t s) {
    if (recs.size() >= kMaxRecs) return -1;
    Rec r{stage, nullptr, nullptr};
    if (!spare.empty()) {
      r.a = spare.back().a;
      r.b = spare.back().b;
      spare.pop_back();
    } else {
      if (hipEventCreate(&r.a) != hipSuccess) return -1;
      if (hipEventCreate(&r.b) != hipSuccess) {
        (void)hipEventDestroy(r.a);
        return -1;
      }
    }
    (void)hipEventRecord(r.a, s);
    recs.push_back(r);
    return (int)recs.size() - 1;
  }
  void done(int idx, hipStream_t s) {
    if (idx >= 0) (void)hipEventRecord(recs[idx].b, s);
  }
};
#define CG_TIME(fork, stage, stream, launch)                                   \
  do {                                                                          \
    const int _t = (fork).timer ? (fork).timer->mark((stage), (stream)) : -1;  \
    launch;                                                                     \
    if (_t >= 0) (fork).timer->done(_t, (stream));                             \
  } while (0)

struct PendingTabs : cgs::Pending {
  const cg_key* keys = nullptr;
  uint32_t n_keys = 0;
  void* keyprep = nullptr;
  WidePool wide;
};

struct Fork {
  hipStream_t side[3];
  hipEvent_t start, ready[3], front, row0[3];
  StageTimer* timer;
  hipEvent_t planned = nullptr;
  hipEvent_t ec_front_go = nullptr, ec_front_done[2] = {nullptr, nullptr};
  mutable PendingTabs pending;
  hipEvent_t mark = nullptr;
  const std::function<hipError_t()>* mid_front = nullptr;
};

struct SigTable {
  const void* p = nullptr;
  uint32_t stride = sizeof(cg_txsig);
  bool packed() const { return stride == sizeof(cg_txsig_packed); }
  SigTable from(uint64_t first) const { return {(const uint8_t*)p + first * stride, stride}; }
};
template <class F>
auto with_records(const SigTable& t, F&& f) {
  return !t.packed() ? f((const cg_txsig*)t.p) : f((const cg_txsig_packed*)t.p);
}

struct VerifyReq {
  const cg_key* d_keys;
  uint32_t n_keys;
  const cg_item* d_items;
  uint64_t n_items;
  const uint8_t* d_arena;
  uint64_t arena_len;
  uint32_t mode;
  uint8_t* d_status;
  const uint8_t* d_msgs = nullptr;
  uint64_t msgs_len = 0;
};

struct ItemArgs : VerifyReq {
  const void* d_keyprep;
  void* d_item_ws;
  const void* d_btab;
  const WidePool* wide;
};

struct KeyUses {
  SigTable sigs;
  const uint32_t* counts = nullptr;
  uint64_t n = 0;
  const cg_key* host_keys = nullptr;
  const uint32_t* host_counts = nullptr;
};

struct SignArgs {
  const void* d_reqs;
  uint64_t n;
  bool fused;
  const void* d_signers;
  uint32_t n_signers;
  const uint8_t* d_arena;
  uint64_t arena_len;
  const uint8_t* d_msgs;
  const cg_signable_tmpl* d_tmpls;
  uint32_t n_tmpls;
  uint64_t n_ids;
  uint8_t* d_sigs;
  uint8_t* d_status;
  void* d_ws;
  const void* d_btab;
};

struct EngineVariant {
  uint32_t fixed_base_bits;
  hipError_t (*upload_constants)();
  size_t (*keyprep_bytes)(uint32_t n_keys);
  size_t (*wide_bytes)(uint32_t n_keys, uint64_t n_items, uint32_t max_slots);
  size_t (*wide_slot_bytes)();
  WidePool (*make_wide_pool)(void* base, uint32_t n_keys, uint64_t n_items, uint32_t max_slots, uint32_t alloc_slots);
  uint32_t (*wide_slots)(uint32_t n_keys, uint64_t n_items, uint32_t max_slots);
  size_t (*key_cache_bytes)(uint32_t slots);
  size_t (*btab_bytes)();
  size_t (*btab_scratch_bytes)();
  hipError_t (*init_btab)(void* d_btab, void* d_scratch, hipStream_t stream);
  size_t (*item_ws_bytes)(uint64_t n_items);
  hipError_t (*launch_keyprep)(const VerifyReq& r, void* d_keyprep, hipStream_t stream, const Fork& fork,
                               const WidePool* wide, const KeyUses* src);
  hipError_t (*launch_key_tables)(const Fork& fork, hipStream_t stream);
  hipError_t (*launch_items)(const ItemArgs& a, hipStream_t stream, const Fork& fork);
  hipError_t (*launch_items_plan)(const ItemArgs& a, hipStream_t stream, const Fork& fork);
  hipError_t (*launch_items_front)(const ItemArgs& a, hipStream_t stream, const Fork& fork, bool planned);
  hipError_t (*launch_items_back)(const ItemArgs& a, hipStream_t stream, const Fork& fork);
  size_t (*signer_bytes)();
  size_t (*sign_ws_bytes)(uint64_t n);
  hipError_t (*launch_signer_expand)(const uint8_t* d_seeds, uint32_t n, void* d_signers, uint8_t* d_pubkeys,
                                     const void* d_btab, hipStream_t stream);
  hipError_t (*launch_sign)(const SignArgs& a, hipStream_t stream);
};

}

namespace cg {

using cgt::EngineVariant;
using cgt::Fork;
using cgt::ItemArgs;
using cgt::PendingTabs;
using cgt::SignArgs;
using cgt::SigTable;
using cgt::StageTimer;
using cgt::VerifyReq;
using cgt::WidePool;
using cgt::with_records;

const EngineVariant& variant();

hipError_t upload_constants();

size_t keyprep_bytes(uint32_t n_keys);
size_t wide_bytes(uint32_t n_keys, uint64_t n_items, uint32_t max_slots = 8192u);
size_t wide_slot_bytes();
constexpr uint32_t kKeyWideMax = 8192u;
WidePool make_wide_pool(void* base, uint32_t n_keys, uint64_t n_items, uint32_t max_slots = 8192u,
                        uint32_t alloc_slots = 0);
uint32_t wide_slots(uint32_t n_keys, uint64_t n_items, uint32_t max_slots);
size_t key_cache_bytes(uint32_t slots);

size_t btab_bytes();
size_t btab_scratch_bytes();
hipError_t init_btab(void* d_btab, void* d_scratch, hipStream_t stream);
size_t item_ws_bytes(uint64_t n_items);
using cgt::KeyUses;
hipError_t launch_keyprep(const VerifyReq& r, void* d_keyprep, hipStream_t stream, const Fork& fork,
                          const WidePool* wide, const KeyUses* src);
hipError_t launch_key_tables(const Fork& fork, hipStream_t stream);
hipError_t launch_items(const ItemArgs& a, hipStream_t stream, const Fork& fork);
hipError_t launch_items_plan(const ItemArgs& a, hipStream_t stream, const Fork& fork);
hipError_t launch_items_front(const ItemArgs& a, hipStream_t stream, const Fork& fork, bool planned);
hipError_t launch_items_back(const ItemArgs& a, hipStream_t stream, const Fork& fork);

size_t signer_bytes();
size_t sign_ws_bytes(uint64_t n);
hipError_t launch_signer_expand(const uint8_t* d_seeds, uint32_t n, void* d_signers, uint8_t* d_pubkeys,
                                const void* d_btab, hipStream_t stream);
hipError_t launch_sign(const SignArgs& a, hipStream_t stream);

constexpr uint64_t kRsaSegment = 1ull << 30;
size_t rsa_keys_bytes(uint32_t n_keys);
size_t rsa_list_bytes(uint64_t n_items);
hipError_t launch_rsa_keyprep(const VerifyReq& r, void* d_rsakeys, hipStream_t stream);
hipError_t launch_rsa_items(const VerifyReq& r, const void* d_rsakeys, void* d_rsalist, hipStream_t stream);

hipError_t launch_sha256(const cg_span* d_spans, uint64_t n, const uint8_t* d_arena, uint64_t arena_len,
                         uint8_t* d_out, hipStream_t stream);
hipError_t launch_sha512(const cg_span* d_spans, uint64_t n, const uint8_t* d_arena, uint64_t arena_len,
                         uint8_t* d_out, hipStream_t stream);

size_t tx_ws_bytes(uint64_t n_comps);
hipError_t launch_tx_ids(const cg_tx* d_txs, uint64_t n_tx, const cg_component* d_comps, uint64_t n_comps,
                         const uint8_t* d_arena, uint64_t arena_len, uint8_t* d_ids, uint8_t* d_status,
                         uint8_t* d_leaf_ws, hipStream_t stream);

uint64_t tx_msgs_head(uint32_t n_tmpls, uint64_t slot);
hipError_t launch_tx_sig_items(const cg_txsig* d_sigs, uint64_t n_sigs, const cg_signable_tmpl* d_tmpls,
                               uint32_t n_tmpls, const uint8_t* d_tx_status, uint64_t n_tx, const uint8_t* d_ids,
                               const uint8_t* d_arena, uint64_t arena_len, uint64_t slot, cg_item* d_items,
                               uint8_t* d_msgs, hipStream_t stream);
hipError_t launch_tx_sig_templates(const cg_signable_tmpl* d_tmpls, uint32_t n_tmpls, const uint8_t* d_arena,
                                   uint64_t arena_len, uint64_t slot, const uint8_t* d_ids, uint64_t n_ids,
                                   uint8_t* d_msgs, hipStream_t stream);
hipError_t launch_tx_sig_range(const cg_txsig* d_sigs, uint64_t first, uint64_t n, const cg_signable_tmpl* d_tmpls,
                               uint32_t n_tmpls, const uint8_t* d_tx_status, uint64_t n_tx, const uint8_t* d_ids,
                               uint64_t arena_len, uint64_t slot, cg_item* d_items, uint8_t* d_msgs,
                               hipStream_t stream);

size_t tx_sig12_scratch_bytes(uint64_t n);
hipError_t launch_tx_sig12_bases(const cg_txsig_packed* d_sigs, uint64_t first, uint64_t n, uint64_t base,
                                 uint64_t* d_bases, hipStream_t stream);
hipError_t launch_tx_sig12_range(const cg_txsig_packed* d_sigs, uint64_t first, uint64_t n, uint64_t sig_region,
                                 uint64_t sig_bytes_len, uint64_t base, const uint64_t* d_bases,
                                 const cg_signable_tmpl* d_tmpls,
                                 uint32_t n_tmpls, uint64_t n_tx, uint64_t arena_len, cg_item* d_items,
                                 void* d_scratch, hipStream_t stream);

hipError_t launch_merkle_roots(const uint8_t* d_leaves, const uint64_t* d_first, const uint32_t* d_count,
                               uint64_t n, uint8_t* d_roots, uint8_t* d_status, uint8_t* d_ws,
                               const uint64_t* d_wsoff, hipStream_t stream);

size_t ftx_ws_bytes(uint64_t n_leaves);
hipError_t launch_filtered(const cg_filtered_tx* d_ftxs, uint64_t n_ftx, const cg_pmt_node* d_nodes, uint64_t n_nodes,
                           const cg_filtered_leaf* d_leaves, uint64_t n_leaves, const uint8_t* d_arena,
                           uint64_t arena_len, uint8_t* d_status, uint8_t* d_ws, hipStream_t stream);


struct TxvSet {
  const uint32_t* key_class = nullptr;
  const cg_tx_check* checks = nullptr;
  uint64_t n_tx = 0;
  const uint32_t* reqs = nullptr;
  uint32_t n_reqs = 0;
  const cg_req_node* nodes = nullptr;
  uint32_t n_nodes = 0;
  cg_tx_verdict* verdicts = nullptr;
  uint8_t* req_status = nullptr;
};
size_t tx_verdicts_ws_bytes(uint64_t n_tx);
hipError_t launch_tx_verdicts(const SigTable& d_sigs, uint64_t n_sigs, const uint8_t* d_status, const cg_key* d_keys,
                              uint32_t n_keys, const TxvSet& d, void* d_ws, hipStream_t stream);

}
```

corda_amd/csrc/keyws.h:

```cpp
#pragma once
#include <hip/hip_runtime.h>

#include "ecdsa.h"
#include "ecdsa_rows.h"
#include "ed25519.h"
#include "ed25519_rows.h"
#include "engine.h"
#include "key_cache.h"
#include "sha2.h"

namespace cg {

__device__ __forceinline__ uint64_t round4(uint64_t x) { return (x + 3) & ~(uint64_t)3; }

#define CG_XCDS 8u
struct Walk {
  uint64_t u, end, step;
};
__device__ __forceinline__ Walk walk_units(uint64_t n) {
  const uint32_t groups = gridDim.x >= CG_XCDS ? CG_XCDS : 1u;
  const uint32_t g = blockIdx.x % groups;
  const uint32_t bpg = gridDim.x / groups;
  const uint64_t span = (n + groups - 1) / groups;
  const uint64_t lo = (uint64_t)g * span;
  const uint64_t hi = lo + span < n ? lo + span : n;
  Walk w;
  w.u = lo + (uint64_t)(blockIdx.x / groups) * blockDim.x + threadIdx.x;
  w.end = hi;
  w.step = (uint64_t)bpg * blockDim.x;
  return w;
}
static inline unsigned walk_grid(uint64_t units, uint32_t block, uint32_t cap) {
  uint64_t g = (units + block - 1) / block;
  if (g > cap) g = cap;
  g = (g + CG_XCDS - 1) / CG_XCDS * CG_XCDS;
  return (unsigned)(g ? g : CG_XCDS);
}
#define CG_CUS 256u
#define WALK_CAP(waves_per_simd) (CG_CUS * (waves_per_simd) * 2u)

__device__ __forceinline__ bool in_arena(uint64_t off, uint64_t len, uint64_t arena_len) {
  return off <= arena_len && len <= arena_len - off;
}

#define CG_ITEM_MSG_WS 1u
#define CG_ITEM_TMPL 2u
#define CG_ITEM_FUSED 4u
struct SpliceHdr {
  uint64_t ids;
  uint64_t n_ids;
  uint64_t img_off;
  uint64_t slot;
  uint64_t w512_off;
};
#define SPLICE_HDR_BYTES 256u
struct TmplMid {
  uint32_t state[8];
  uint32_t blocks;
  uint32_t prefix_len;
  uint32_t ed_mid;
  uint32_t pad;
};
static_assert(sizeof(TmplMid) == 48, "template midstate record");
struct TmplW512 {
  uint64_t wk[80];
};
#define TMPL_ED_MID_MIN_PREFIX 192u
CG_HD uint64_t tmpl_w512_off(uint32_t n_tmpls) {
  return SPLICE_HDR_BYTES + (((uint64_t)n_tmpls * sizeof(TmplMid) + 255) & ~(uint64_t)255);
}
CG_HD uint64_t tmpl_mid_bytes(uint32_t n_tmpls) { return tmpl_w512_off(n_tmpls) + (uint64_t)n_tmpls * sizeof(TmplW512); }
__device__ __forceinline__ bool item_fused(const cg_item& it, const uint8_t* msgs) {
  return msgs && (it.reserved0 & (CG_ITEM_MSG_WS | CG_ITEM_TMPL | CG_ITEM_FUSED)) ==
                     (CG_ITEM_MSG_WS | CG_ITEM_TMPL | CG_ITEM_FUSED);
}
__device__ __forceinline__ const TmplMid* item_tmpl_mid(const cg_item& it, const uint8_t* msgs) {
  return (it.reserved0 & CG_ITEM_TMPL) && (it.reserved0 & CG_ITEM_MSG_WS) && msgs
             ? (const TmplMid*)(msgs + SPLICE_HDR_BYTES) + it.reserved1
             : nullptr;
}
__device__ __forceinline__ SpliceLd tmpl_splice(uint32_t tmpl, uint64_t tx, const uint8_t* msgs) {
  const SpliceHdr* h = (const SpliceHdr*)msgs;
  const TmplMid* m = (const TmplMid*)(msgs + SPLICE_HDR_BYTES) + tmpl;
  SpliceLd ld;
  ld.img = msgs + h->img_off + (uint64_t)tmpl * h->slot;
  ld.img_len = h->slot;
  ld.id = (const uint32_t*)(uintptr_t)h->ids + 8ull * tx;
  ld.at = m->prefix_len;
  return ld;
}
__device__ __forceinline__ SpliceLd item_splice(const cg_item& it, const uint8_t* msgs) {
  return tmpl_splice(it.reserved1, it.msg_off, msgs);
}
__device__ __forceinline__ bool item_in_ws(const cg_item& it, const uint8_t* msgs) {
  return (it.reserved0 & CG_ITEM_MSG_WS) && msgs != nullptr;
}
__device__ __forceinline__ const uint8_t* item_msg_arena(const cg_item& it, const uint8_t* arena,
                                                         const uint8_t* msgs) {
  return item_in_ws(it, msgs) ? msgs : arena;
}
__device__ __forceinline__ uint64_t item_msg_len(const cg_item& it, uint64_t arena_len, uint64_t msgs_len,
                                                 const uint8_t* msgs) {
  return item_in_ws(it, msgs) ? msgs_len : arena_len;
}

typedef EdRowsCfg<ED_W, ED_K> EdCfg;
typedef EdRowTabW<ED_W, ED_K> EdTab;
#define ED_QK 11
typedef EdRowsCfg<ED_W, ED_QK> EdQCfg;
typedef EdRowTabW<ED_W, ED_QK> EdQTab;
static_assert(EdQCfg::kRows <= EdCfg::kRows && EdQCfg::kMult == EdCfg::kMult, "quarter rows fit the full table");
#define KEY_BASES (EdCfg::kRows > EC_ROWS ? EdCfg::kRows : EC_ROWS)
static_assert(EC_QROWS <= EC_ROWS, "ECDSA quarter rows fit the full table");
typedef EdBCfg<ED_W, ED_K, ED_WB> EdBCfgT;
typedef EdBTabW<ED_W, ED_K, ED_WB> EdBTab;

__device__ __forceinline__ void chain_prio() { __builtin_amdgcn_s_setprio(3); }

struct EdKeyHdr {
  uint32_t status;
  uint32_t abyte[8];
  uint32_t pad[7];
};

union TabSlot {
  EdTab ed;
  EcRowTab ec;
};
union BaseSlot {
  ge_p3 ed;
  Jac ec;
};

#define PLAN_ED 0
#define PLAN_R1 1
#define PLAN_K1 2
#define PLAN_CLASSES 3
#define PLAN_FULL 4
#define PLAN_WIDE 7
#define PLAN_QUART 10
#define PLAN_MODE_ROW0 0u
#define PLAN_MODE_QUART 1u
#define PLAN_MODE_FULL 2u
#define PLAN_MODE_WIDE 3u
#define ITEM_LONG_MIN 1024u
__device__ __forceinline__ int plan_class_of_curve(int curve) { return curve == 1 ? PLAN_R1 : PLAN_K1; }

static inline size_t al256(size_t x) { return (x + 255) & ~(size_t)255; }
#define TAB_PARK_LANES 131072u
static inline uint32_t tab_park_lanes(uint32_t n_keys, uint32_t rows) {
  uint64_t l = (uint64_t)(n_keys ? n_keys : 1) * rows;
  if (l > TAB_PARK_LANES) l = TAB_PARK_LANES;
  return (uint32_t)((l + 63) & ~(uint64_t)63);
}
#define KC_CTR_HITS 0
#define KC_CTR_BUILT 1
#define KC_CTR_EVICTED 2
#define KC_CTR_FELL_BACK 3
#define KC_CTRS 8
struct KeyCache {
  uint32_t* ctr = nullptr;
  KcOwner* owners[2] = {nullptr, nullptr};
  uint32_t* live[2] = {nullptr, nullptr};
  uint32_t* freel[2] = {nullptr, nullptr};
  uint32_t* index[2] = {nullptr, nullptr};
  uint32_t slots = 0, size = 0, bits = 0;
  bool dirty = false;
  __host__ __device__ bool on() const { return ctr != nullptr; }
};
static inline size_t key_cache_total(uint32_t slots) {
  if (!slots) return 0;
  return 256 + 2 * (al256((size_t)slots * sizeof(KcOwner)) + 2 * al256((size_t)slots * sizeof(uint32_t)) +
                    al256((size_t)kc_index_size(slots) * sizeof(uint32_t)));
}
static inline KeyCache key_cache(void* base, uint32_t slots, uint32_t bits, bool dirty) {
  KeyCache k;
  if (!base || !slots) return k;
  uint8_t* p = (uint8_t*)base;
  k.ctr = (uint32_t*)p;
  p += 256;
  for (int q = 0; q < 2; ++q) {
    k.owners[q] = (KcOwner*)p;
    p += al256((size_t)slots * sizeof(KcOwner));
  }
  for (int q = 0; q < 2; ++q) {
    k.live[q] = (uint32_t*)p;
    p += al256((size_t)slots * sizeof(uint32_t));
  }
  for (int q = 0; q < 2; ++q) {
    k.freel[q] = (uint32_t*)p;
    p += al256((size_t)slots * sizeof(uint32_t));
  }
  k.size = kc_index_size(slots);
  for (int q = 0; q < 2; ++q) {
    k.index[q] = (uint32_t*)p;
    p += al256((size_t)k.size * sizeof(uint32_t));
  }
  k.slots = slots;
  k.bits = bits;
  k.dirty = dirty;
  return k;
}

#define ED_ROW_PARK_BYTES ((size_t)EdCfg::kMult * ED_PARK_DWORDS * 4)
#define EC_ROW_PARK_BYTES ((size_t)EC_MULT * EC_ROW_PARK * 4)
#define ROW0_COUNT_AT 8
#define QUART_COUNT_AT 16
#define SKIP_MISMATCH_AT 24
struct KeyWs {
  EdKeyHdr* hdr;
  TabSlot* tab;
  BaseSlot* bases;
  uint32_t* park_ed;
  uint32_t* park_ec[2];
  uint32_t park_lanes_ed, park_lanes_ec;
  uint32_t* uses;
  uint32_t* full;
  uint32_t* full_count;
  uint32_t* row0;
  uint32_t* row0_count;
  uint32_t* quart;
  uint32_t* quart_count;
  uint8_t* seen;
  uint32_t* wide_idx;
  uint32_t* wide;
  uint32_t* wide_count;
  struct EdWideSlot* wed;
  struct EcWideSlot* wec;
  uint32_t cap_ed, cap_ec;
  uint32_t min_ed, min_ec;
  KeyCache kc;
};

#ifndef KEY_WIDE_MIN_USES_ED
#define KEY_WIDE_MIN_USES_ED 1536u
#endif
#ifndef KEY_WIDE_MIN_USES_EC
#define KEY_WIDE_MIN_USES_EC 512u
#endif
#define KEY_WIDE_MIN_USES (KEY_WIDE_MIN_USES_EC < KEY_WIDE_MIN_USES_ED ? KEY_WIDE_MIN_USES_EC : KEY_WIDE_MIN_USES_ED)
#define KEY_NOT_WIDE 0xffffffffu
#define KEY_WIDE_MAX 8192u
#define KEY_USES_ALL 0xffffffffu
#define KEY_USES_SAMPLE 4u
#ifndef KEY_QUARTER_MIN_USES
#define KEY_QUARTER_MIN_USES 3u
#endif
#ifndef ED_DIRECT_MAX_USES
#define ED_DIRECT_MAX_USES 32u
#endif
struct EdWideSlot {
  EdWideTab tab;
  ge_p3 bases[EdWideCfg::kRows];
  union {
    fe zpre[EdWideCfg::kRows][EdWideCfg::kMult];
    uint32_t park[EdWideCfg::kRows * EdWideCfg::kMult * ED_PARK_DWORDS];
  };
};
struct EcWideSlot {
  EcWideTab tab;
  EcAff bases[EC_WIDE_DIGITS];
  Jac jbases[EC_WIDE_DIGITS];
  union {
    EcWideScratch s[EC_WIDE_ROWS];
    uint32_t park[EC_WIDE_ROWS * EC_WIDE_MULT * EC_PARK_DWORDS];
  };
};
static_assert(sizeof(EdWideSlot) == 1184768 && sizeof(EcWideSlot) == 766080, "the wide pools' layout is fixed");
static inline uint32_t wide_cap(uint32_t n_keys, uint64_t n_items, uint32_t max_slots = KEY_WIDE_MAX,
                                uint32_t min_uses = KEY_WIDE_MIN_USES) {
  uint64_t c = n_items / min_uses;
  if (c > n_keys) c = n_keys;
  if (c > KEY_WIDE_MAX) c = KEY_WIDE_MAX;
  if (c > max_slots) c = max_slots;
  return (uint32_t)c;
}
static inline size_t wide_pool_bytes(uint32_t cap) {
  return cap ? al256((size_t)cap * sizeof(EdWideSlot)) + al256((size_t)cap * sizeof(EcWideSlot)) : 0;
}
static inline WidePool wide_pool(void* base, uint32_t cap, uint32_t slots = 0) {
  WidePool p;
  p.min_ed = KEY_WIDE_MIN_USES_ED;
  p.min_ec = KEY_WIDE_MIN_USES_EC;
  if (!slots) slots = cap;
  if (!base || !cap || cap > slots) return p;
  p.ed = base;
  p.ec = (uint8_t*)base + al256((size_t)slots * sizeof(EdWideSlot));
  p.cap_ed = p.cap_ec = cap;
  p.slots = slots;
  return p;
}

static inline KeyWs key_ws(void* base, uint32_t n_keys, const WidePool* wp = nullptr) {
  const size_t n = n_keys ? n_keys : 1;
  uint8_t* p = (uint8_t*)base;
  KeyWs w;
  w.hdr = (EdKeyHdr*)p;
  p += al256(n * sizeof(EdKeyHdr));
  w.tab = (TabSlot*)p;
  p += al256(n * sizeof(TabSlot));
  w.bases = (BaseSlot*)p;
  p += al256(n * KEY_BASES * sizeof(BaseSlot));
  w.park_lanes_ed = tab_park_lanes(n_keys, EdCfg::kRows);
  w.park_lanes_ec = tab_park_lanes(n_keys, EC_ROWS);
  w.park_ed = (uint32_t*)p;
  p += al256(w.park_lanes_ed * ED_ROW_PARK_BYTES);
  for (int c = 0; c < 2; ++c) {
    w.park_ec[c] = (uint32_t*)p;
    p += al256(w.park_lanes_ec * EC_ROW_PARK_BYTES);
  }
  w.uses = (uint32_t*)p;
  p += al256(n * sizeof(uint32_t));
  w.full = (uint32_t*)p;
  p += al256(3 * n * sizeof(uint32_t));
  w.full_count = (uint32_t*)p;
  w.row0_count = w.full_count + ROW0_COUNT_AT;
  p += 256;
  w.quart_count = w.full_count + QUART_COUNT_AT;
  w.row0 = (uint32_t*)p;
  p += al256(3 * n * sizeof(uint32_t));
  w.quart = (uint32_t*)p;
  p += al256(3 * n * sizeof(uint32_t));
  w.seen = p;
  p += al256(n);
  w.wide_idx = (uint32_t*)p;
  p += al256(n * sizeof(uint32_t));
  w.wide = (uint32_t*)p;
  p += al256(3 * n * sizeof(uint32_t));
  w.wide_count = (uint32_t*)p;
  p += 256;
  w.wed = wp ? (EdWideSlot*)wp->ed : nullptr;
  w.wec = wp ? (EcWideSlot*)wp->ec : nullptr;
  w.cap_ed = wp ? wp->cap_ed : 0;
  w.cap_ec = wp ? wp->cap_ec : 0;
  w.min_ed = wp && wp->min_ed ? wp->min_ed : KEY_WIDE_MIN_USES_ED;
  w.min_ec = wp && wp->min_ec ? wp->min_ec : KEY_WIDE_MIN_USES_EC;
  w.kc = wp && wp->cache && wp->cap_ed ? key_cache(wp->cache, wp->slots, wp->cache_bits, wp->cache_dirty) : KeyCache{};
  return w;
}
static inline size_t key_ws_bytes(uint32_t n_keys) {
  const size_t n = n_keys ? n_keys : 1;
  return al256(n * sizeof(EdKeyHdr)) + al256(n * sizeof(TabSlot)) + al256(n * KEY_BASES * sizeof(BaseSlot)) +
         al256(tab_park_lanes(n_keys, EdCfg::kRows) * ED_ROW_PARK_BYTES) +
         2 * al256(tab_park_lanes(n_keys, EC_ROWS) * EC_ROW_PARK_BYTES) + al256(n * sizeof(uint32_t)) +
         al256(3 * n * sizeof(uint32_t)) + 256 + 2 * al256(3 * n * sizeof(uint32_t)) + al256(n) +
         al256(n * sizeof(uint32_t)) + al256(3 * n * sizeof(uint32_t)) + 256;
}

constexpr size_t ITEM_SLOT = sizeof(ge_p2);
static_assert(sizeof(EcItemWs) == ITEM_SLOT, "ECDSA stage hand-off must fill one item slot");
size_t plan_sort_temp_bytes(uint64_t n_items);
struct EdCols {
  uint32_t* r;
  uint8_t* pend;
  uint32_t* key;
  uint64_t n;
};
struct ItemWs {
  void* slots;
  uint32_t* perm;
  uint32_t* ranges;
  uint32_t *skey_in, *skey_out, *sval_in;
  void* sort_temp;
  size_t sort_temp_bytes;
  EdCols ed;
};
static inline ItemWs item_ws(void* base, uint64_t n_items) {
  const size_t n = n_items ? n_items : 1;
  uint8_t* p = (uint8_t*)base;
  ItemWs w;
  w.slots = p;
  p += al256(n * ITEM_SLOT);
  w.perm = (uint32_t*)p;
  p += al256(n * sizeof(uint32_t));
  w.ranges = (uint32_t*)p;
  p += 256;
  w.skey_in = (uint32_t*)p;
  p += al256(n * sizeof(uint32_t));
  w.skey_out = (uint32_t*)p;
  p += al256(n * sizeof(uint32_t));
  w.sval_in = (uint32_t*)p;
  p += al256(n * sizeof(uint32_t));
  w.sort_temp = p;
  w.sort_temp_bytes = plan_sort_temp_bytes(n);
  p += al256(w.sort_temp_bytes);
  w.ed.n = n;
  w.ed.r = (uint32_t*)p;
  p += al256(8 * n * sizeof(uint32_t));
  w.ed.key = (uint32_t*)p;
  p += al256(n * sizeof(uint32_t));
  w.ed.pend = p;
  return w;
}
static inline size_t item_ws_total(uint64_t n_items) {
  const size_t n = n_items ? n_items : 1;
  return al256(n * ITEM_SLOT) + 4 * al256(n * sizeof(uint32_t)) + 256 + al256(plan_sort_temp_bytes(n)) +
         al256(8 * n * sizeof(uint32_t)) + al256(n * sizeof(uint32_t)) + al256(n);
}
hipError_t launch_plan(const cg_item* d_items, uint64_t n_items, const cg_key* d_keys, uint32_t n_keys,
                       const KeyWs& w, const ItemWs& iw, hipStream_t stream);

#define EC_GTAB_LANES (EC_G_DIGITS * (EC_G_MULT / EC_MULT))
#define EC_GWIDE_LANES (EC_WIDE_GDIGITS * (EC_WIDE_GMULT / EC_MULT))
#define CONST_SCRATCH_MAX 131072
#define CONST_SCRATCH_LANES                                                                        \
  ((EC_GWIDE_LANES < CONST_SCRATCH_MAX ? EC_GWIDE_LANES : CONST_SCRATCH_MAX) > EC_GTAB_LANES       \
       ? (EC_GWIDE_LANES < CONST_SCRATCH_MAX ? EC_GWIDE_LANES : CONST_SCRATCH_MAX)                 \
       : EC_GTAB_LANES)
static inline size_t const_tab_bytes() {
  return sizeof(EdBTab) + 2 * sizeof(EcGTab) + sizeof(EdBWideTab) + 2 * sizeof(EcGWideTab);
}
static inline size_t const_scratch_bytes() { return (size_t)CONST_SCRATCH_LANES * sizeof(EcRowScratch); }
static inline const EcGTab* gtab(const void* d_btab, int curve) {
  return (const EcGTab*)((const uint8_t*)d_btab + sizeof(EdBTab)) + curve;
}
static inline const EdBWideTab* bwide(const void* d_btab) {
  return (const EdBWideTab*)((const uint8_t*)d_btab + sizeof(EdBTab) + 2 * sizeof(EcGTab));
}
static inline const EcGWideTab* gwide(const void* d_btab, int curve) {
  return (const EcGWideTab*)((const uint8_t*)bwide(d_btab) + sizeof(EdBWideTab)) + curve;
}

#define ED_PENDING 254u
#define EC_PENDING_BASE 250u

void kc_launch_commit(int c, uint32_t n_keys, const KeyWs& w, hipStream_t stream);

hipError_t ed_upload_constants();
hipError_t ed_init_const(void* d_btab, void* d_scratch, hipStream_t stream);
void ed_launch_key_abyte(const cg_key* d_keys, uint32_t n_keys, const uint8_t* d_arena, uint64_t arena_len,
                         const KeyWs& w, hipStream_t stream);
void ed_launch_keyprep_chains(const cg_key* d_keys, uint32_t n_keys, const uint8_t* d_arena, uint64_t arena_len,
                              const KeyWs& w, hipStream_t stream);
void ed_launch_keyprep_tabs(const cg_key* d_keys, uint32_t n_keys, const KeyWs& w, hipStream_t stream, bool full,
                            bool wide);
void ed_launch_front(const cg_item* d_items, uint64_t n_items, const uint8_t* d_arena, uint64_t arena_len,
                     uint32_t mode, uint8_t* d_status, const KeyWs& w, const uint8_t* d_msgs, uint64_t msgs_len,
                     const ItemWs& iw, hipStream_t stream);
void ed_launch_ladder(bool full, const cg_item* d_items, uint64_t n_items, uint8_t* d_status, const KeyWs& w,
                      const ItemWs& iw, const void* d_btab, hipStream_t stream);
void ed_launch_ladder_wide(const cg_item* d_items, uint64_t n_items, uint8_t* d_status, const KeyWs& w,
                           const ItemWs& iw, const void* d_btab, hipStream_t stream);
void ed_launch_finish(const cg_item* d_items, uint64_t n_items, const uint8_t* d_arena, uint64_t arena_len,
                      uint8_t* d_status, const ItemWs& iw, hipStream_t stream);
hipError_t ec_upload_constants();
hipError_t ec_init_const(void* d_btab, void* d_scratch, hipStream_t stream);
void ec_launch_keyprep_chains(int curve, const cg_key* d_keys, uint32_t n_keys, const uint8_t* d_arena,
                              uint64_t arena_len, const KeyWs& w, hipStream_t stream);
void ec_launch_keyprep_tabs(int curve, const cg_key* d_keys, uint32_t n_keys, const KeyWs& w, hipStream_t stream,
                            bool full, bool wide);
void ec_launch_front(int curve, const cg_item* d_items, uint64_t n_items, const uint8_t* d_arena,
                     uint64_t arena_len, uint32_t mode, uint8_t* d_status, const KeyWs& w, const uint8_t* d_msgs,
                     uint64_t msgs_len, const ItemWs& iw, hipStream_t stream);
void ec_launch_ladder(int curve, bool full, const cg_item* d_items, uint64_t n_items, uint8_t* d_status,
                      const KeyWs& w, const ItemWs& iw, const void* d_btab, hipStream_t stream);
void ec_launch_ladder_wide(int curve, const cg_item* d_items, uint64_t n_items, uint8_t* d_status, const KeyWs& w,
                           const ItemWs& iw, const void* d_btab, hipStream_t stream);

}
```

corda_amd/csrc/plan_sort.hip:

```cpp
#include <hip/hip_runtime.h>

#include <rocprim/device/device_radix_sort.hpp>

#include "keyws.h"

namespace cg {

typedef rocprim::radix_sort_config<rocprim::default_config, rocprim::default_config, rocprim::default_config, 0>
    PlanSortConfig;

static uint32_t key_bits(uint32_t n_keys) {
  uint32_t b = 1;
  while (b < 27 && (1u << b) < n_keys) ++b;
  return b;
}

__global__ void __launch_bounds__(256) k_plan_keys(const cg_item* __restrict__ items, uint64_t n_items,
                                                   const cg_key* __restrict__ keys, uint32_t n_keys, uint32_t kb,
                                                   const uint32_t* __restrict__ uses,
                                                   const uint32_t* __restrict__ wide_idx,
                                                   uint32_t* __restrict__ skey, uint32_t* __restrict__ sval) {
  const uint64_t i = (uint64_t)blockIdx.x * blockDim.x + threadIdx.x;
  if (i >= n_items) return;
  const uint32_t k = items[i].key_idx;
  uint32_t c = PLAN_CLASSES;
  if (k < n_keys) {
    const uint8_t s = keys[k].scheme;
    c = s == CG_EDDSA_ED25519_SHA512 ? PLAN_ED
      : s == CG_ECDSA_SECP256R1_SHA256 ? PLAN_R1
      : s == CG_ECDSA_SECP256K1_SHA256 ? PLAN_K1
                                       : PLAN_CLASSES;
  }
  uint32_t mode = 0;
  if (c < PLAN_CLASSES)
    mode = wide_idx[k] != KEY_NOT_WIDE         ? PLAN_MODE_WIDE
         : uses[k] >= ED_DIRECT_MAX_USES      ? PLAN_MODE_FULL
         : uses[k] >= KEY_QUARTER_MIN_USES    ? PLAN_MODE_QUART
                                              : PLAN_MODE_ROW0;
  const uint32_t lng = items[i].msg_len > ITEM_LONG_MIN ? 1u : 0u;
  skey[i] = (c << kb) |
            (c < PLAN_CLASSES ? (mode << (kb - 2)) | (lng << (kb - 3)) | (k & ((1u << (kb - 3)) - 1u)) : 0u);
  sval[i] = (uint32_t)i;
}

__global__ void k_plan_ranges(const uint32_t* __restrict__ skey, uint64_t n_items, uint32_t kb,
                              uint32_t* __restrict__ ranges) {
  const uint32_t t = threadIdx.x;
  if (t >= PLAN_QUART + PLAN_CLASSES) return;
  uint32_t c, target;
  if (t <= PLAN_CLASSES) {
    c = t;
    target = c << kb;
  } else if (t < PLAN_WIDE) {
    c = t - PLAN_FULL;
    target = (c << kb) | (PLAN_MODE_FULL << (kb - 2));
  } else if (t < PLAN_QUART) {
    c = t - PLAN_WIDE;
    target = (c << kb) | (PLAN_MODE_WIDE << (kb - 2));
  } else {
    c = t - PLAN_QUART;
    target = (c << kb) | (PLAN_MODE_QUART << (kb - 2));
  }
  uint64_t lo = 0, hi = n_items;
  while (lo < hi) {
    const uint64_t mid = (lo + hi) >> 1;
    if (skey[mid] < target) lo = mid + 1;
    else hi = mid;
  }
  ranges[t] = (uint32_t)lo;
}

size_t plan_sort_temp_bytes(uint64_t n_items) {
  size_t bytes = 0;
  rocprim::radix_sort_pairs<PlanSortConfig>((void*)nullptr, bytes, (const uint32_t*)nullptr, (uint32_t*)nullptr,
                            (const uint32_t*)nullptr, (uint32_t*)nullptr, (size_t)(n_items ? n_items : 1), 0u,
                            32u);
  return bytes;
}

hipError_t launch_plan(const cg_item* d_items, uint64_t n_items, const cg_key* d_keys, uint32_t n_keys,
                       const KeyWs& w, const ItemWs& iw, hipStream_t stream) {
  const uint32_t B = 256;
  const uint32_t kb = key_bits(n_keys) + 3;
  hipLaunchKernelGGL(k_plan_keys, dim3((unsigned)((n_items + B - 1) / B)), dim3(B), 0, stream, d_items, n_items,
                     d_keys, n_keys, kb, (const uint32_t*)w.uses, (const uint32_t*)w.wide_idx, iw.skey_in, iw.sval_in);
  size_t bytes = iw.sort_temp_bytes;
  hipError_t e = rocprim::radix_sort_pairs<PlanSortConfig>(iw.sort_temp, bytes, (const uint32_t*)iw.skey_in, iw.skey_out,
                                           (const uint32_t*)iw.sval_in, iw.perm, (size_t)n_items, 0u, kb + 2,
                                           stream);
  if (e != hipSuccess) return e;
  hipLaunchKernelGGL(k_plan_ranges, dim3(1), dim3(64), 0, stream, (const uint32_t*)iw.skey_out, n_items, kb,
                     iw.ranges);
  return hipGetLastError();
}

}
```

corda_amd/csrc/txpipe.hip:

```cpp
#include <hip/hip_runtime.h>

#include "engine.h"
#include "keyws.h"
#include "sha2.h"

namespace cg {

__device__ __forceinline__ bool tmpl_ok(const cg_signable_tmpl& t, uint64_t arena_len) {
  return in_arena(t.prefix_off, t.prefix_len, arena_len) && in_arena(t.suffix_off, t.suffix_len, arena_len);
}

__global__ void __launch_bounds__(256) k_txsig_items(const cg_txsig* __restrict__ sigs, uint64_t first, uint64_t n_sigs,
                                                     const cg_signable_tmpl* __restrict__ tmpls, uint32_t n_tmpls,
                                                     const uint8_t* __restrict__ tx_status, uint64_t n_tx,
                                                     uint64_t arena_len, cg_item* __restrict__ items) {
  const uint64_t j = first + (uint64_t)blockIdx.x * blockDim.x + threadIdx.x;
  if (j >= first + n_sigs) return;
  const cg_txsig s = sigs[j];
  cg_item it;
  it.sig_off = s.sig_off;
  it.sig_len = s.sig_len;
  it.reserved1 = 0;
  bool ok = s.tx_idx < n_tx && s.tmpl < n_tmpls;
  if (ok && tx_status) ok = tx_status[s.tx_idx] == 0;
  cg_signable_tmpl t = {0, 0, 0, 0};
  if (ok) {
    t = tmpls[s.tmpl];
    ok = tmpl_ok(t, arena_len);
  }
  if (ok) {
    it.msg_off = s.tx_idx;
    it.msg_len = t.prefix_len + 32u + t.suffix_len;
    it.key_idx = s.key_idx;
    it.reserved0 = CG_ITEM_MSG_WS | CG_ITEM_TMPL | CG_ITEM_FUSED;
    it.reserved1 = s.tmpl;
  } else {
    it.msg_off = 0;
    it.msg_len = 0;
    it.key_idx = 0xffffffffu;
    it.reserved0 = 0;
  }
  items[j] = it;
}

#define SIG12_BLOCK 256
__device__ __forceinline__ uint32_t sig12_span(uint32_t len) { return (len + 3u) & ~3u; }

__device__ __forceinline__ uint32_t wave_incl_scan(uint32_t v) {
  const int lane = (int)(threadIdx.x & 63);
#pragma unroll
  for (int d = 1; d < 64; d <<= 1) {
    const uint32_t u = __shfl_up(v, d, 64);
    if (lane >= d) v += u;
  }
  return v;
}

__global__ void __launch_bounds__(SIG12_BLOCK) k_sig12_blocksum(const cg_txsig_packed* __restrict__ sigs,
                                                                uint64_t first, uint64_t n, uint64_t* __restrict__ sums) {
  const uint64_t j = (uint64_t)blockIdx.x * SIG12_BLOCK + threadIdx.x;
  uint32_t v = j < n ? sig12_span(sigs[first + j].sig_len) : 0u;
#pragma unroll
  for (int d = 32; d >= 1; d >>= 1) v += __shfl_xor(v, d, 64);
  __shared__ uint32_t part[SIG12_BLOCK / 64];
  if ((threadIdx.x & 63) == 0) part[threadIdx.x >> 6] = v;
  __syncthreads();
  if (threadIdx.x == 0) {
    uint64_t t = 0;
    for (int w = 0; w < SIG12_BLOCK / 64; ++w) t += part[w];
    sums[blockIdx.x] = t;
  }
}

__global__ void __launch_bounds__(1024) k_sig12_scan(uint64_t* __restrict__ sums, uint64_t nb, uint64_t base) {
  __shared__ uint64_t sh[1024];
  const uint32_t t = threadIdx.x;
  const uint64_t per = (nb + 1023) / 1024, lo = t * per, hi = lo + per < nb ? lo + per : nb;
  uint64_t s = 0;
  for (uint64_t i = lo; i < hi; ++i) s += sums[i];
  sh[t] = s;
  __syncthreads();
  for (uint32_t d = 1; d < 1024; d <<= 1) {
    const uint64_t u = t >= d ? sh[t - d] : 0;
    __syncthreads();
    sh[t] += u;
    __syncthreads();
  }
  uint64_t run = base + sh[t] - s;
  for (uint64_t i = lo; i < hi; ++i) {
    const uint64_t x = sums[i];
    sums[i] = run;
    run += x;
  }
}

__global__ void __launch_bounds__(SIG12_BLOCK) k_txsig12_items(const cg_txsig_packed* __restrict__ sigs, uint64_t first,
                                                               uint64_t n_sigs, const uint64_t* __restrict__ bases,
                                                               uint64_t sig_region, uint64_t sig_bytes_len,
                                                               const cg_signable_tmpl* __restrict__ tmpls,
                                                               uint32_t n_tmpls, uint64_t n_tx, uint64_t arena_len,
                                                               cg_item* __restrict__ items) {
  const uint64_t jj = (uint64_t)blockIdx.x * SIG12_BLOCK + threadIdx.x;
  const bool live = jj < n_sigs;
  cg_txsig_packed s = {0, 0, 0, 0};
  if (live) s = sigs[first + jj];
  const uint32_t span = live ? sig12_span(s.sig_len) : 0u;
  const uint32_t incl = wave_incl_scan(span);
  __shared__ uint32_t wtot[SIG12_BLOCK / 64];
  if ((threadIdx.x & 63) == 63) wtot[threadIdx.x >> 6] = incl;
  __syncthreads();
  uint32_t wbase = 0;
  for (uint32_t w = 0; w < (threadIdx.x >> 6); ++w) wbase += wtot[w];
  if (!live) return;
  cg_item it;
  const uint64_t so = bases[blockIdx.x] + (wbase + incl - span);
  it.sig_off = sig_region + so;
  it.sig_len = s.sig_len;
  it.reserved1 = 0;
  bool ok = s.tx_idx < n_tx && s.tmpl < n_tmpls && so <= sig_bytes_len && s.sig_len <= sig_bytes_len - so;
  cg_signable_tmpl t = {0, 0, 0, 0};
  if (ok) {
    t = tmpls[s.tmpl];
    ok = tmpl_ok(t, arena_len);
  }
  if (ok) {
    it.msg_off = s.tx_idx;
    it.msg_len = t.prefix_len + 32u + t.suffix_len;
    it.key_idx = s.key_idx;
    it.reserved0 = CG_ITEM_MSG_WS | CG_ITEM_TMPL | CG_ITEM_FUSED;
    it.reserved1 = s.tmpl;
  } else {
    it.msg_off = 0;
    it.msg_len = 0;
    it.key_idx = 0xffffffffu;
    it.reserved0 = 0;
  }
  items[first + jj] = it;
}

size_t tx_sig12_scratch_bytes(uint64_t n) { return 8 * ((n + SIG12_BLOCK - 1) / SIG12_BLOCK + 1); }

hipError_t launch_tx_sig12_bases(const cg_txsig_packed* d_sigs, uint64_t first, uint64_t n, uint64_t base,
                                 uint64_t* d_bases, hipStream_t stream) {
  if (n == 0) return hipSuccess;
  const uint64_t nb = (n + SIG12_BLOCK - 1) / SIG12_BLOCK;
  hipLaunchKernelGGL(k_sig12_blocksum, dim3((unsigned)nb), dim3(SIG12_BLOCK), 0, stream, d_sigs, first, n, d_bases);
  hipLaunchKernelGGL(k_sig12_scan, dim3(1), dim3(1024), 0, stream, d_bases, nb, base);
  return hipGetLastError();
}

hipError_t launch_tx_sig12_range(const cg_txsig_packed* d_sigs, uint64_t first, uint64_t n, uint64_t sig_region,
                                 uint64_t sig_bytes_len, uint64_t base, const uint64_t* d_bases,
                                 const cg_signable_tmpl* d_tmpls,
                                 uint32_t n_tmpls, uint64_t n_tx, uint64_t arena_len, cg_item* d_items,
                                 void* d_scratch, hipStream_t stream) {
  if (n == 0) return hipSuccess;
  const uint64_t* bases = d_bases ? d_bases + first / SIG12_BLOCK : (const uint64_t*)d_scratch;
  if (d_bases && first % SIG12_BLOCK) return hipErrorInvalidValue;
  if (!d_bases) {
    const hipError_t e = launch_tx_sig12_bases(d_sigs, first, n, base, (uint64_t*)d_scratch, stream);
    if (e != hipSuccess) return e;
  }
  hipLaunchKernelGGL(k_txsig12_items, dim3((unsigned)((n + SIG12_BLOCK - 1) / SIG12_BLOCK)), dim3(SIG12_BLOCK), 0,
                     stream, d_sigs, first, n, bases, sig_region, sig_bytes_len, d_tmpls, n_tmpls, n_tx, arena_len,
                     d_items);
  return hipGetLastError();
}

static __host__ __device__ inline uint64_t tx_img_off(uint32_t n_tmpls) { return tmpl_mid_bytes(n_tmpls); }
uint64_t tx_msgs_head(uint32_t n_tmpls, uint64_t slot) {
  return (tx_img_off(n_tmpls) + (uint64_t)n_tmpls * slot + 255) & ~(uint64_t)255;
}

__global__ void __launch_bounds__(64) k_tmpl_prep(const cg_signable_tmpl* __restrict__ tmpls, uint32_t n_tmpls,
                                                  const uint8_t* __restrict__ arena, uint64_t arena_len,
                                                  uint64_t slot, const uint8_t* __restrict__ ids, uint64_t n_ids,
                                                  uint8_t* __restrict__ msgs) {
  const uint32_t t = blockIdx.x;
  if (t == 0 && threadIdx.x == 0) {
    SpliceHdr h;
    h.ids = (uint64_t)(uintptr_t)ids;
    h.n_ids = n_ids;
    h.img_off = tx_img_off(n_tmpls);
    h.slot = slot;
    h.w512_off = tmpl_w512_off(n_tmpls);
    *(SpliceHdr*)msgs = h;
  }
  if (t >= n_tmpls) return;
  const cg_signable_tmpl tm = tmpls[t];
  const bool ok = tmpl_ok(tm, arena_len);
  const uint64_t lr = round4(arena_len);
  auto byte_at = [&](uint64_t x) -> uint32_t {
    if (!ok) return 0u;
    if (x < tm.prefix_len) return cg_ld_bytes4(arena, lr, tm.prefix_off + x) & 0xffu;
    if (x < tm.prefix_len + 32u) return 0u;
    if (x < (uint64_t)tm.prefix_len + 32u + tm.suffix_len)
      return cg_ld_bytes4(arena, lr, tm.suffix_off + (x - tm.prefix_len - 32u)) & 0xffu;
    return 0u;
  };
  uint32_t* img = (uint32_t*)(msgs + tx_img_off(n_tmpls) + (uint64_t)t * slot);
  for (uint32_t w = threadIdx.x; w < slot / 4; w += 64) {
    uint32_t v = 0;
    for (int q = 0; q < 4; ++q) v |= byte_at(4ull * w + q) << (8 * q);
    img[w] = v;
  }
  const bool ed_mid = ok && tm.prefix_len >= TMPL_ED_MID_MIN_PREFIX;
  if (threadIdx.x == 1) {
    uint64_t* wk = ((TmplW512*)(msgs + tmpl_w512_off(n_tmpls)) + t)->wk;
    uint64_t w[16];
    for (int j = 0; j < 16; ++j) {
      uint64_t v = 0;
      for (int q = 0; q < 8; ++q) v = (v << 8) | (ed_mid ? byte_at(64ull + 8u * j + q) : 0u);
      w[j] = v;
      wk[j] = v + cg_k512(j);
    }
    for (int r = 16; r < 80; r += 16)
      for (int j = 0; j < 16; ++j) wk[r + j] = sha512_sched(w, j) + cg_k512(r + j);
  }
  if (threadIdx.x != 0) return;
  TmplMid r;
  sha256_init(r.state);
  r.blocks = 0;
  r.prefix_len = tm.prefix_len;
  r.ed_mid = ed_mid ? 1u : 0u;
  r.pad = 0;
  if (ok) {
    for (uint32_t b = 0; b < tm.prefix_len / 64; ++b) {
      uint32_t w[16];
      for (int j = 0; j < 16; ++j) {
        uint32_t v = 0;
        for (int q = 0; q < 4; ++q) v = (v << 8) | byte_at(64ull * b + 4u * j + q);
        w[j] = v;
      }
      sha256_compress(r.state, w);
      r.blocks = b + 1;
    }
  }
  ((TmplMid*)(msgs + SPLICE_HDR_BYTES))[t] = r;
}

hipError_t launch_tx_sig_templates(const cg_signable_tmpl* d_tmpls, uint32_t n_tmpls, const uint8_t* d_arena,
                                   uint64_t arena_len, uint64_t slot, const uint8_t* d_ids, uint64_t n_ids,
                                   uint8_t* d_msgs, hipStream_t stream) {
  hipLaunchKernelGGL(k_tmpl_prep, dim3(n_tmpls ? n_tmpls : 1), dim3(64), 0, stream, d_tmpls, n_tmpls, d_arena,
                     arena_len, slot, d_ids, n_ids, d_msgs);
  return hipGetLastError();
}

hipError_t launch_tx_sig_range(const cg_txsig* d_sigs, uint64_t first, uint64_t n, const cg_signable_tmpl* d_tmpls,
                               uint32_t n_tmpls, const uint8_t* d_tx_status, uint64_t n_tx, const uint8_t* d_ids,
                               uint64_t arena_len, uint64_t slot, cg_item* d_items, uint8_t* d_msgs,
                               hipStream_t stream) {
  if (n == 0) return hipSuccess;
  const uint32_t B = 256;
  (void)d_ids;
  (void)slot;
  (void)d_msgs;
  hipLaunchKernelGGL(k_txsig_items, dim3((unsigned)((n + B - 1) / B)), dim3(B), 0, stream, d_sigs, first, n, d_tmpls,
                     n_tmpls, d_tx_status, n_tx, arena_len, d_items);
  return hipGetLastError();
}

hipError_t launch_tx_sig_items(const cg_txsig* d_sigs, uint64_t n_sigs, const cg_signable_tmpl* d_tmpls,
                               uint32_t n_tmpls, const uint8_t* d_tx_status, uint64_t n_tx, const uint8_t* d_ids,
                               const uint8_t* d_arena, uint64_t arena_len, uint64_t slot, cg_item* d_items,
                               uint8_t* d_msgs, hipStream_t stream) {
  if (n_sigs == 0) return hipSuccess;
  hipError_t e = launch_tx_sig_templates(d_tmpls, n_tmpls, d_arena, arena_len, slot, d_ids, n_tx, d_msgs, stream);
  if (e == hipSuccess)
    e = launch_tx_sig_range(d_sigs, 0, n_sigs, d_tmpls, n_tmpls, d_tx_status, n_tx, d_ids, arena_len, slot, d_items,
                            d_msgs, stream);
  return e;
}

}
```

corda_amd/csrc/verify.hip:

```cpp
#include "keyws.h"

namespace cg {

__global__ void k_misc_status(const cg_item* __restrict__ items, uint64_t n_items, const cg_key* __restrict__ keys,
                              uint32_t n_keys, uint8_t* __restrict__ status) {
  const uint64_t i = (uint64_t)blockIdx.x * blockDim.x + threadIdx.x;
  if (i >= n_items) return;
  const uint32_t ki = items[i].key_idx;
  if (ki >= n_keys) {
    status[i] = CG_NOT_RUN;
    return;
  }
  const uint8_t s = keys[ki].scheme;
  if (s != CG_EDDSA_ED25519_SHA512 && s != CG_ECDSA_SECP256R1_SHA256 && s != CG_ECDSA_SECP256K1_SHA256)
    status[i] = CG_UNSUPPORTED;
  else if (s == CG_EDDSA_ED25519_SHA512)
    status[i] = CG_NOT_RUN;
}

__global__ void __launch_bounds__(256) k_key_init(uint32_t n_keys, uint32_t all, uint32_t* __restrict__ uses,
                                                  uint8_t* __restrict__ seen, uint32_t* __restrict__ full_count,
                                                  uint32_t* __restrict__ wide_idx, uint32_t* __restrict__ wide_count) {
  const uint32_t i = blockIdx.x * blockDim.x + threadIdx.x;
  if (i < PLAN_CLASSES) full_count[i] = full_count[ROW0_COUNT_AT + i] = full_count[QUART_COUNT_AT + i] = 0;
  if (i == 0) full_count[SKIP_MISMATCH_AT] = 0;
  if (i < PLAN_CLASSES + 2) wide_count[i] = 0;
  if (i >= n_keys) return;
  uses[i] = all ? KEY_USES_ALL : 0u;
  seen[i] = all ? 1 : 0;
  wide_idx[i] = KEY_NOT_WIDE;
}

__global__ void __launch_bounds__(256) k_key_uses(const cg_item* __restrict__ items, uint64_t n_items,
                                                  uint32_t n_keys, uint32_t* __restrict__ uses,
                                                  uint8_t* __restrict__ seen) {
  const uint64_t i = (uint64_t)blockIdx.x * blockDim.x + threadIdx.x;
  if (i >= n_items) return;
  const uint32_t k = items[i].key_idx;
  if (k >= n_keys) return;
  seen[k] = 1;
  if (((uint32_t)i * 0x9E3779B1u) >> 30 == 0) atomicAdd(&uses[k], KEY_USES_SAMPLE);
}

template <class Sig>
__global__ void __launch_bounds__(256) k_key_uses_txsig(const Sig* __restrict__ sigs, uint64_t n,
                                                        uint32_t n_keys, uint32_t* __restrict__ uses,
                                                        uint8_t* __restrict__ seen) {
  const uint64_t i = (uint64_t)blockIdx.x * blockDim.x + threadIdx.x;
  if (i >= n) return;
  const uint32_t k = sigs[i].key_idx;
  if (k >= n_keys) return;
  seen[k] = 1;
  if (((uint32_t)i * 0x9E3779B1u) >> 30 == 0) atomicAdd(&uses[k], KEY_USES_SAMPLE);
}

__global__ void __launch_bounds__(256) k_key_counts(const uint32_t* __restrict__ counts, uint32_t n_keys,
                                                    uint32_t* __restrict__ uses, uint8_t* __restrict__ seen) {
  const uint32_t i = blockIdx.x * blockDim.x + threadIdx.x;
  if (i >= n_keys) return;
  uses[i] = counts[i];
  seen[i] = counts[i] != 0;
}

__device__ __forceinline__ void list_append(int c, uint32_t i, uint32_t n_keys, uint32_t* __restrict__ list,
                                            uint32_t* __restrict__ count) {
  const uint32_t lane = threadIdx.x & 63u;
#pragma unroll
  for (int k = 0; k < PLAN_CLASSES; ++k) {
    const uint64_t m = __ballot(c == k);
    if (m == 0) continue;
    const int leader = __ffsll((long long)m) - 1;
    uint32_t base = 0;
    if ((int)lane == leader) base = atomicAdd(&count[k], (uint32_t)__popcll(m));
    base = __shfl(base, leader, 64);
    if (c == k) list[(size_t)k * n_keys + base + (uint32_t)__popcll(m & ((1ull << lane) - 1ull))] = i;
  }
}

#define KC_BLOCK 1024
__global__ void __launch_bounds__(KC_BLOCK) k_kc_begin(KeyCache kc) {
  const int pool = blockIdx.x;
  KcOwner* owners = kc.owners[pool];
  uint32_t* index = kc.index[pool];
  if (threadIdx.x < KC_CTRS) kc.ctr[pool * KC_CTRS + threadIdx.x] = 0;
  for (uint32_t b = threadIdx.x; b < kc.size; b += KC_BLOCK) index[b] = 0;
  for (uint32_t s = threadIdx.x; s < kc.slots; s += KC_BLOCK) kc_begin_slot(owners, kc.live[pool], s, kc.dirty);
  __syncthreads();
  for (uint32_t s = threadIdx.x; s < kc.slots; s += KC_BLOCK)
    if (owners[s].state == KC_VALID) kc_index_insert(index, kc.size, kc.bits, owners, s);
}

__device__ __forceinline__ void kc_load_key(KcKey& k, const cg_key& key, const uint8_t* arena, uint64_t arena_len) {
  kc_key_load(k, key.scheme, key.fmt, key.len, arena, arena_len, key.off);
}

__global__ void __launch_bounds__(64) k_key_classify(const cg_key* __restrict__ keys, uint32_t n_keys,
                                                     uint32_t* __restrict__ uses, const uint8_t* __restrict__ seen,
                                                     uint32_t* __restrict__ full, uint32_t* __restrict__ full_count,
                                                     uint32_t* __restrict__ wide_idx, uint32_t* __restrict__ wide,
                                                     uint32_t* __restrict__ wide_count, uint32_t* __restrict__ row0,
                                                     uint32_t* __restrict__ quart, uint32_t cap_ed, uint32_t cap_ec,
                                                     uint32_t min_ed, uint32_t min_ec, uint32_t skip_mask,
                                                     const uint8_t* __restrict__ arena, uint64_t arena_len,
                                                     KeyCache kc) {
  const uint32_t i = blockIdx.x * 64 + threadIdx.x;
  int c = -1, cw = -1, c0 = -1, cq = -1;
  bool is_wide = false;
  uint32_t u = 0;
  if (i < n_keys) {
    u = uses[i];
    if (!seen[i]) u = 0;
    else if (u == 0) u = 1;
    uses[i] = u;
  }
  if (i < n_keys && u >= ED_DIRECT_MAX_USES) {
    const uint8_t s = keys[i].scheme;
    c = s == CG_EDDSA_ED25519_SHA512 ? PLAN_ED
      : s == CG_ECDSA_SECP256R1_SHA256 ? PLAN_R1
      : s == CG_ECDSA_SECP256K1_SHA256 ? PLAN_K1
                                       : -1;
    const int pool = c == PLAN_ED ? 0 : 1;
    if (c >= 0 && u >= (pool == 0 ? min_ed : min_ec) && u != KEY_USES_ALL) {
      const uint32_t cap = pool == 0 ? cap_ed : cap_ec;
      if (cap) {
        const uint32_t slot = atomicAdd(&wide_count[PLAN_CLASSES + pool], 1u);
        if (slot < cap) {
          is_wide = true;
          if (!kc.on()) {
            wide_idx[i] = slot;
            cw = c;
          } else {
            KcKey k;
            kc_load_key(k, keys[i], arena, arena_len);
            const uint32_t hit = kc_probe(kc.index[pool], kc.size, kc.bits, kc.owners[pool], k);
            if (hit != KC_NONE) {
              wide_idx[i] = hit;
              kc.live[pool][hit] = 1;
              atomicAdd(&kc.ctr[pool * KC_CTRS + KC_CTR_HITS], 1u);
            } else {
              cw = c;
            }
          }
          c = -1;
        } else if (kc.on()) {
          atomicAdd(&kc.ctr[pool * KC_CTRS + KC_CTR_FELL_BACK], 1u);
        }
      }
    }
  }
  if (i < n_keys && u >= 1 && !is_wide) {
    const uint8_t s = keys[i].scheme;
    c0 = s == CG_EDDSA_ED25519_SHA512 ? PLAN_ED
       : s == CG_ECDSA_SECP256R1_SHA256 ? PLAN_R1
       : s == CG_ECDSA_SECP256K1_SHA256 ? PLAN_K1
                                        : -1;
    if (u >= KEY_QUARTER_MIN_USES && u < ED_DIRECT_MAX_USES) cq = c0;
  }
  if (skip_mask && (c >= 0 || c0 >= 0)) {
    const int cls = c >= 0 ? c : c0;
    const uint32_t f = cls == PLAN_R1 ? 0u : cls == PLAN_K1 ? 1u : 2u;
    if ((skip_mask >> f) & 1u) atomicOr(&full_count[SKIP_MISMATCH_AT], 1u << f);
  }
  list_append(c, i, n_keys, full, full_count);
  list_append(cw, i, n_keys, wide, wide_count);
  list_append(c0, i, n_keys, row0, full_count + ROW0_COUNT_AT);
  list_append(cq, i, n_keys, quart, full_count + QUART_COUNT_AT);
}

__global__ void __launch_bounds__(KC_BLOCK) k_kc_claim(const cg_key* __restrict__ keys, uint32_t n_keys,
                                                       const uint8_t* __restrict__ arena, uint64_t arena_len,
                                                       uint32_t* __restrict__ wide_idx, uint32_t* __restrict__ wide,
                                                       uint32_t* __restrict__ wide_count, uint32_t* __restrict__ full,
                                                       uint32_t* __restrict__ full_count, uint32_t* __restrict__ row0,
                                                       uint32_t skip_mask, KeyCache kc) {
  __shared__ uint32_t sc[2][KC_BLOCK];
  __shared__ uint32_t tot[2];
  const int pool = blockIdx.x;
  const uint32_t t = threadIdx.x;
  KcOwner* owners = kc.owners[pool];
  uint32_t cnt[2];
  kc_free_count(owners, kc.live[pool], kc.slots, t, KC_BLOCK, cnt);
  sc[0][t] = cnt[0];
  sc[1][t] = cnt[1];
  __syncthreads();
  for (uint32_t d = 1; d < KC_BLOCK; d <<= 1) {
    const uint32_t a = t >= d ? sc[0][t - d] : 0u, b = t >= d ? sc[1][t - d] : 0u;
    __syncthreads();
    sc[0][t] += a;
    sc[1][t] += b;
    __syncthreads();
  }
  if (t == KC_BLOCK - 1) {
    tot[0] = sc[0][t];
    tot[1] = sc[1][t];
  }
  __syncthreads();
  kc_free_fill(owners, kc.live[pool], kc.slots, t, KC_BLOCK, sc[0][t] - cnt[0], tot[0] + sc[1][t] - cnt[1],
               kc.freel[pool]);
  const uint32_t nfree = tot[0] + tot[1];
  const int c_lo = pool == 0 ? PLAN_ED : PLAN_R1, c_hi = pool == 0 ? PLAN_ED : PLAN_K1;
  static_assert(PLAN_R1 + 1 == PLAN_K1, "the ECDSA pool's classes are adjacent");
  uint32_t n_c[2] = {0, 0};
  for (int c = c_lo; c <= c_hi; ++c) n_c[c - c_lo] = wide_count[c];
  __syncthreads();
  uint32_t base = 0;
  for (int c = c_lo; c <= c_hi; ++c) {
    const uint32_t n = n_c[c - c_lo];
    for (uint32_t l = t; l < n; l += KC_BLOCK) {
      const uint32_t i = wide[(size_t)c * n_keys + l];
      KcKey k;
      kc_load_key(k, keys[i], arena, arena_len);
      bool evicted;
      const uint32_t s = kc_claim(owners, kc.freel[pool], nfree, base + l, k, &evicted);
      if (s != KC_NONE) {
        wide_idx[i] = s;
        if (evicted) atomicAdd(&kc.ctr[pool * KC_CTRS + KC_CTR_EVICTED], 1u);
      } else {
        full[(size_t)c * n_keys + atomicAdd(&full_count[c], 1u)] = i;
        row0[(size_t)c * n_keys + atomicAdd(&full_count[ROW0_COUNT_AT + c], 1u)] = i;
        const uint32_t f = c == PLAN_R1 ? 0u : c == PLAN_K1 ? 1u : 2u;
        if ((skip_mask >> f) & 1u) atomicOr(&full_count[SKIP_MISMATCH_AT], 1u << f);
        atomicAdd(&kc.ctr[pool * KC_CTRS + KC_CTR_FELL_BACK], 1u);
      }
    }
    if (t == 0) wide_count[c] = base >= nfree ? 0u : (n < nfree - base ? n : nfree - base);
    base += n;
  }
}

__global__ void __launch_bounds__(256) k_kc_commit(int c, uint32_t n_keys, const EdKeyHdr* __restrict__ hdr,
                                                   const uint32_t* __restrict__ wide,
                                                   const uint32_t* __restrict__ wide_count,
                                                   const uint32_t* __restrict__ wide_idx, KeyCache kc) {
  const int pool = c == PLAN_ED ? 0 : 1;
  const uint32_t n = wide_count[c];
  for (uint32_t l = blockIdx.x * blockDim.x + threadIdx.x; l < n; l += gridDim.x * blockDim.x) {
    const uint32_t i = wide[(size_t)c * n_keys + l];
    if (kc_commit(kc.owners[pool], wide_idx[i], hdr[i].status == 0))
      atomicAdd(&kc.ctr[pool * KC_CTRS + KC_CTR_BUILT], 1u);
  }
}
void kc_launch_commit(int c, uint32_t n_keys, const KeyWs& w, hipStream_t stream) {
  if (!w.kc.on()) return;
  hipLaunchKernelGGL(k_kc_commit, dim3(8), dim3(256), 0, stream, c, n_keys, (const EdKeyHdr*)w.hdr,
                     (const uint32_t*)w.wide, (const uint32_t*)w.wide_count, (const uint32_t*)w.wide_idx, w.kc);
}

__global__ void __launch_bounds__(256) k_mode_guard(const uint32_t* __restrict__ ranges,
                                                    const uint32_t* __restrict__ perm,
                                                    const uint32_t* __restrict__ full_count, uint32_t skip_mask,
                                                    uint8_t* __restrict__ status) {
  const uint32_t bad = full_count[SKIP_MISMATCH_AT] & skip_mask;
  if (!bad) return;
  for (int f = 0; f < 3; ++f) {
    if (!((bad >> f) & 1u)) continue;
    const int cls = f == 0 ? PLAN_R1 : f == 1 ? PLAN_K1 : PLAN_ED;
    const uint32_t beg = ranges[cls], end = ranges[PLAN_WIDE + cls];
    for (uint32_t p = beg + blockIdx.x * blockDim.x + threadIdx.x; p < end; p += gridDim.x * blockDim.x)
      status[perm[p]] = CG_NOT_RUN;
  }
}

hipError_t upload_constants() {
  hipError_t e = ed_upload_constants();
  if (e != hipSuccess) return e;
  return ec_upload_constants();
}

size_t keyprep_bytes(uint32_t n_keys) { return key_ws_bytes(n_keys); }
size_t wide_bytes(uint32_t n_keys, uint64_t n_items, uint32_t max_slots) {
  return wide_pool_bytes(wide_cap(n_keys, n_items, max_slots));
}
size_t wide_slot_bytes() { return wide_pool_bytes(1); }
static_assert(kKeyWideMax == KEY_WIDE_MAX, "engine.h mirrors keyws.h");
WidePool make_wide_pool(void* base, uint32_t n_keys, uint64_t n_items, uint32_t max_slots, uint32_t alloc_slots) {
  return wide_pool(base, wide_cap(n_keys, n_items, max_slots), alloc_slots);
}
uint32_t wide_slots(uint32_t n_keys, uint64_t n_items, uint32_t max_slots) { return wide_cap(n_keys, n_items, max_slots); }
size_t key_cache_bytes(uint32_t slots) { return key_cache_total(slots); }
size_t item_ws_bytes(uint64_t n_items) { return item_ws_total(n_items); }
size_t btab_bytes() { return const_tab_bytes(); }
size_t btab_scratch_bytes() { return const_scratch_bytes(); }

hipError_t init_btab(void* d_btab, void* d_scratch, hipStream_t stream) {
  hipError_t e = ed_init_const(d_btab, d_scratch, stream);
  if (e != hipSuccess) return e;
  return ec_init_const(d_btab, d_scratch, stream);
}


static void families_needing_full(const KeyUses& src, uint32_t n_keys, const KeyWs& w, bool need[3]) {
  uint32_t hot[2] = {0, 0};
  bool low[3] = {false, false, false};
  for (uint32_t i = 0; i < n_keys; ++i) {
    const uint32_t u = src.host_counts[i];
    if (u == 0) continue;
    const uint8_t s = src.host_keys[i].scheme;
    const int f = s == CG_ECDSA_SECP256R1_SHA256 ? 0 : s == CG_ECDSA_SECP256K1_SHA256 ? 1 : s == CG_EDDSA_ED25519_SHA512 ? 2 : -1;
    if (f < 0) continue;
    const int pool = f == 2 ? 0 : 1;
    const uint32_t cap = pool == 0 ? w.cap_ed : w.cap_ec;
    if (u >= ED_DIRECT_MAX_USES && u >= (pool == 0 ? w.min_ed : w.min_ec) && u != KEY_USES_ALL && cap) ++hot[pool];
    else low[f] = true;
  }
  const bool over[2] = {hot[0] > w.cap_ed, hot[1] > w.cap_ec};
  for (int f = 0; f < 3; ++f) need[f] = low[f] || over[f == 2 ? 0 : 1];
}

struct KeyArgs {
  const VerifyReq& r;
  const cg_item* d_items;
  uint64_t n_items;
  const KeyUses* src;
  KeyWs w;
  uint32_t all;
};

struct HipOps {
  using Error = hipError_t;
  static constexpr Error kOk = hipSuccess;
  hipStream_t main;
  const Fork& fork;
  const KeyArgs* key = nullptr;
  const ItemArgs* a = nullptr;
  KeyWs w{};
  ItemWs iw{};

  HipOps(hipStream_t s, const Fork& f, const KeyArgs* k, const ItemArgs* items) : main(s), fork(f), key(k), a(items) {
    if (!a) return;
    w = key_ws((void*)a->d_keyprep, a->n_keys, a->wide);
    iw = item_ws(a->d_item_ws, a->n_items);
  }
  hipStream_t st(cgs::Stream s) const { return s == cgs::MAIN ? main : fork.side[s - cgs::SIDE0]; }
  hipEvent_t ev(cgs::Event e) const {
    switch (e) {
      case cgs::EV_START: return fork.start;
      case cgs::EV_PLANNED: return fork.planned;
      case cgs::EV_READY0: case cgs::EV_READY1: case cgs::EV_READY2: return fork.ready[e - cgs::EV_READY0];
      case cgs::EV_FRONT: return fork.front;
      case cgs::EV_ROW0_0: case cgs::EV_ROW0_1: case cgs::EV_ROW0_2: return fork.row0[e - cgs::EV_ROW0_0];
      case cgs::EV_EC_FRONT_GO: return fork.ec_front_go;
      case cgs::EV_EC_FRONT_DONE0: case cgs::EV_EC_FRONT_DONE1: return fork.ec_front_done[e - cgs::EV_EC_FRONT_DONE0];
      default: return nullptr;
    }
  }
  Error record(cgs::Event e, cgs::Stream s) { return hipEventRecord(ev(e), st(s)); }
  Error wait(cgs::Stream s, cgs::Event e) { return hipStreamWaitEvent(st(s), ev(e), 0); }
  bool mid_hook() const { return fork.mid_front != nullptr; }
  void before_joins() {
    if (fork.mark) hipEventRecord(fork.mark, main);
  }

  Error run(cgs::Stage stage, cgs::Stream on, int, int) {
    hipStream_t s = st(on);
    switch (stage) {
      case cgs::ST_KEY_INIT: {
        const uint32_t n = key->r.n_keys, kl = n > PLAN_CLASSES + 2 ? n : PLAN_CLASSES + 2;
        hipLaunchKernelGGL(k_key_init, dim3((kl + 255) / 256), dim3(256), 0, s, n, key->all, key->w.uses, key->w.seen,
                           key->w.full_count, key->w.wide_idx, key->w.wide_count);
        return kOk;
      }
      case cgs::ST_KEY_USES:
        hipLaunchKernelGGL(k_key_uses, dim3((unsigned)((key->n_items + 255) / 256)), dim3(256), 0, s, key->d_items,
                           key->n_items, key->r.n_keys, key->w.uses, key->w.seen);
        return kOk;
      case cgs::ST_KEY_COUNTS:
        hipLaunchKernelGGL(k_key_counts, dim3((key->r.n_keys + 255) / 256), dim3(256), 0, s, key->src->counts,
                           key->r.n_keys, key->w.uses, key->w.seen);
        return kOk;
      case cgs::ST_KEY_USES_TXSIG:
        with_records(key->src->sigs, [&](auto* recs) {
          using Rec = std::remove_const_t<std::remove_pointer_t<decltype(recs)>>;
          hipLaunchKernelGGL(k_key_uses_txsig<Rec>, dim3((unsigned)((key->src->n + 255) / 256)), dim3(256), 0, s, recs,
                             key->src->n, key->r.n_keys, key->w.uses, key->w.seen);
        });
        return kOk;
      case cgs::ST_KC_BEGIN:
        hipLaunchKernelGGL(k_kc_begin, dim3(2), dim3(KC_BLOCK), 0, s, key->w.kc);
        return kOk;
      case cgs::ST_KEY_CLASSIFY: {
        const KeyWs& kw = key->w;
        hipLaunchKernelGGL(k_key_classify, dim3((key->r.n_keys + 63) / 64), dim3(64), 0, s, key->r.d_keys, key->r.n_keys,
                           kw.uses, (const uint8_t*)kw.seen, kw.full, kw.full_count, kw.wide_idx, kw.wide, kw.wide_count,
                           kw.row0, kw.quart, kw.cap_ed, kw.cap_ec, kw.min_ed, kw.min_ec, fork.pending.skip_mask,
                           key->r.d_arena, key->r.arena_len, kw.kc);
        return kOk;
      }
      case cgs::ST_KC_CLAIM: {
        const KeyWs& kw = key->w;
        hipLaunchKernelGGL(k_kc_claim, dim3(2), dim3(KC_BLOCK), 0, s, key->r.d_keys, key->r.n_keys, key->r.d_arena,
                           key->r.arena_len, kw.wide_idx, kw.wide, kw.wide_count, kw.full, kw.full_count, kw.row0,
                           fork.pending.skip_mask, kw.kc);
        return kOk;
      }
      case cgs::ST_CHAINS_R1: case cgs::ST_CHAINS_K1:
        ec_launch_keyprep_chains(stage == cgs::ST_CHAINS_R1 ? CG_CURVE_R1 : CG_CURVE_K1, key->r.d_keys, key->r.n_keys,
                                 key->r.d_arena, key->r.arena_len, key->w, s);
        return kOk;
      case cgs::ST_CHAINS_ED:
        ed_launch_keyprep_chains(key->r.d_keys, key->r.n_keys, key->r.d_arena, key->r.arena_len, key->w, s);
        return kOk;
      case cgs::ST_WIDE_TABS_R1: case cgs::ST_WIDE_TABS_K1: case cgs::ST_WIDE_TABS_ED:
      case cgs::ST_FULL_TABS_R1: case cgs::ST_FULL_TABS_K1: case cgs::ST_FULL_TABS_ED: {
        const PendingTabs& p = fork.pending;
        const KeyWs pw = key_ws(p.keyprep, p.n_keys, &p.wide);
        const bool full = stage >= cgs::ST_FULL_TABS_R1;
        const int k = stage - (full ? cgs::ST_FULL_TABS_R1 : cgs::ST_WIDE_TABS_R1);
        if (k == 2) ed_launch_keyprep_tabs(p.keys, p.n_keys, pw, s, full, !full);
        else ec_launch_keyprep_tabs(k == 0 ? CG_CURVE_R1 : CG_CURVE_K1, p.keys, p.n_keys, pw, s, full, !full);
        return kOk;
      }
      case cgs::ST_ED_ABYTE:
        ed_launch_key_abyte(key->r.d_keys, key->r.n_keys, key->r.d_arena, key->r.arena_len, key->w, s);
        return kOk;
      case cgs::ST_MISC_STATUS:
        hipLaunchKernelGGL(k_misc_status, dim3((unsigned)((a->n_items + 255) / 256)), dim3(256), 0, s, a->d_items,
                           a->n_items, a->d_keys, a->n_keys, a->d_status);
        return kOk;
      case cgs::ST_PLAN: {
        Error e = kOk;
        CG_TIME(fork, CG_STAGE_PLAN, s, e = launch_plan(a->d_items, a->n_items, a->d_keys, a->n_keys, w, iw, s));
        return e;
      }
      case cgs::ST_MID_HOOK: return (*fork.mid_front)();
      case cgs::ST_EC_FRONT_R1: case cgs::ST_EC_FRONT_K1: {
        const bool r1 = stage == cgs::ST_EC_FRONT_R1;
        CG_TIME(fork, r1 ? CG_STAGE_R1_FRONT : CG_STAGE_K1_FRONT, s,
                ec_launch_front(r1 ? CG_CURVE_R1 : CG_CURVE_K1, a->d_items, a->n_items, a->d_arena, a->arena_len, a->mode,
                                a->d_status, w, a->d_msgs, a->msgs_len, iw, s));
        return kOk;
      }
      case cgs::ST_ED_FRONT:
        CG_TIME(fork, CG_STAGE_ED_HASH, s,
                ed_launch_front(a->d_items, a->n_items, a->d_arena, a->arena_len, a->mode, a->d_status, w, a->d_msgs,
                                a->msgs_len, iw, s));
        return kOk;
      case cgs::ST_ROW0_LADDER_ED:
        CG_TIME(fork, CG_STAGE_ED_LADDER_ROW0, s,
                ed_launch_ladder(false, a->d_items, a->n_items, a->d_status, w, iw, a->d_btab, s));
        return kOk;
      case cgs::ST_ROW0_LADDER_R1: case cgs::ST_ROW0_LADDER_K1: {
        const bool r1 = stage == cgs::ST_ROW0_LADDER_R1;
        CG_TIME(fork, r1 ? CG_STAGE_R1_LADDER_ROW0 : CG_STAGE_K1_LADDER_ROW0, s,
                ec_launch_ladder(r1 ? CG_CURVE_R1 : CG_CURVE_K1, false, a->d_items, a->n_items, a->d_status, w, iw,
                                 a->d_btab, s));
        return kOk;
      }
      case cgs::ST_FULL_LADDER_ED:
        CG_TIME(fork, CG_STAGE_ED_LADDER, s,
                ed_launch_ladder(true, a->d_items, a->n_items, a->d_status, w, iw, a->d_btab, s));
        return kOk;
      case cgs::ST_WIDE_LADDER_ED:
        CG_TIME(fork, CG_STAGE_ED_LADDER_WIDE, s,
                ed_launch_ladder_wide(a->d_items, a->n_items, a->d_status, w, iw, a->d_btab, s));
        return kOk;
      case cgs::ST_ED_FINISH:
        CG_TIME(fork, CG_STAGE_ED_FINISH, s,
                ed_launch_finish(a->d_items, a->n_items, a->d_arena, a->arena_len, a->d_status, iw, s));
        return kOk;
      case cgs::ST_FULL_LADDER_R1: case cgs::ST_FULL_LADDER_K1: {
        const bool r1 = stage == cgs::ST_FULL_LADDER_R1;
        CG_TIME(fork, r1 ? CG_STAGE_R1_LADDER : CG_STAGE_K1_LADDER, s,
                ec_launch_ladder(r1 ? CG_CURVE_R1 : CG_CURVE_K1, true, a->d_items, a->n_items, a->d_status, w, iw,
                                 a->d_btab, s));
        return kOk;
      }
      case cgs::ST_WIDE_LADDER_R1: case cgs::ST_WIDE_LADDER_K1: {
        const bool r1 = stage == cgs::ST_WIDE_LADDER_R1;
        CG_TIME(fork, r1 ? CG_STAGE_R1_LADDER_WIDE : CG_STAGE_K1_LADDER_WIDE, s,
                ec_launch_ladder_wide(r1 ? CG_CURVE_R1 : CG_CURVE_K1, a->d_items, a->n_items, a->d_status, w, iw,
                                      a->d_btab, s));
        return kOk;
      }
      case cgs::ST_MODE_GUARD:
        hipLaunchKernelGGL(k_mode_guard, dim3(64), dim3(256), 0, s, (const uint32_t*)iw.ranges, (const uint32_t*)iw.perm,
                           (const uint32_t*)w.full_count, fork.pending.skip_mask, a->d_status);
        return kOk;
      default: return hipErrorInvalidValue;
    }
  }
};
using Sched = cgs::Schedule<HipOps>;

static cgs::Chunk chunk_of(const HipOps& ops) {
  cgs::Chunk c;
  c.wide_ed = ops.w.cap_ed != 0;
  c.wide_ec = ops.w.cap_ec != 0;
  return c;
}

hipError_t launch_key_tables(const Fork& fork, hipStream_t stream) {
  HipOps ops(stream, fork, nullptr, nullptr);
  return Sched(ops, fork.pending).key_tables();
}

hipError_t launch_keyprep(const VerifyReq& r, void* d_keyprep, hipStream_t stream, const Fork& fork,
                          const WidePool* wide, const KeyUses* src) {
  const uint32_t n_keys = r.n_keys;
  const cg_item* d_items = src ? nullptr : r.d_items;
  const uint64_t n_items = src ? src->n : r.n_items;
  const bool counted = d_items || src;
  const KeyArgs key = {r, d_items, n_items, src, key_ws(d_keyprep, n_keys, counted ? wide : nullptr), counted ? 0u : 1u};
  cgs::KeyPlan k;
  k.any_keys = n_keys != 0;
  k.counted = counted;
  if (d_items && n_items) k.uses = cgs::ST_KEY_USES;
  else if (src && src->counts) k.uses = cgs::ST_KEY_COUNTS;
  else if (src && src->sigs.p && src->n) k.uses = cgs::ST_KEY_USES_TXSIG;
  if (n_keys && !d_items && src && src->counts && src->host_counts && src->host_keys)
    families_needing_full(*src, n_keys, key.w, k.need_full);
  static const uint32_t test_skip = [] {
    const char* v = getenv("CG_TEST_SKIP_FAMILIES");
    return v ? (uint32_t)strtoul(v, nullptr, 0) & 7u : 0u;
  }();
  for (int f = 0; f < 3; ++f)
    if ((test_skip >> f) & 1u) k.need_full[f] = false;
  k.cache = key.w.kc.on();
  k.wide_ed = key.w.cap_ed != 0;
  k.wide_ec = key.w.cap_ec != 0;
  if (n_keys) {
    fork.pending.keys = r.d_keys;
    fork.pending.n_keys = n_keys;
    fork.pending.keyprep = d_keyprep;
    fork.pending.wide = counted && wide ? *wide : WidePool{};
  }
  HipOps ops(stream, fork, &key, nullptr);
  const hipError_t e = Sched(ops, fork.pending).keyprep(k);
  return e != hipSuccess || n_keys == 0 ? e : hipGetLastError();
}

hipError_t launch_items_plan(const ItemArgs& a, hipStream_t stream, const Fork& fork) {
  if (a.n_items == 0) return hipSuccess;
  HipOps ops(stream, fork, nullptr, &a);
  return Sched(ops, fork.pending).items_plan(chunk_of(ops));
}

hipError_t launch_items_front(const ItemArgs& a, hipStream_t stream, const Fork& fork, bool planned) {
  if (a.n_items == 0) return hipSuccess;
  HipOps ops(stream, fork, nullptr, &a);
  const hipError_t e = Sched(ops, fork.pending).items_front(chunk_of(ops), planned);
  return e != hipSuccess ? e : hipGetLastError();
}

hipError_t launch_items_back(const ItemArgs& a, hipStream_t stream, const Fork& fork) {
  if (a.n_items == 0) return hipSuccess;
  HipOps ops(stream, fork, nullptr, &a);
  const hipError_t e = Sched(ops, fork.pending).items_back(chunk_of(ops));
  return e != hipSuccess ? e : hipGetLastError();
}

hipError_t launch_items(const ItemArgs& a, hipStream_t stream, const Fork& fork) {
  const hipError_t e = launch_items_front(a, stream, fork, false);
  return e != hipSuccess ? e : launch_items_back(a, stream, fork);
}

static_assert(ED_WIDE_BW == EC_WIDE_GW, "one fixed-base radix per build (Makefile VARIANTS)");
const EngineVariant& variant() {
  static const EngineVariant v = {(uint32_t)ED_WIDE_BW, upload_constants, keyprep_bytes, wide_bytes, wide_slot_bytes,
                                  make_wide_pool, wide_slots, key_cache_bytes, btab_bytes, btab_scratch_bytes, init_btab, item_ws_bytes,
                                  launch_keyprep, launch_key_tables, launch_items, launch_items_plan,
                                  launch_items_front, launch_items_back,
                                  signer_bytes, sign_ws_bytes, launch_signer_expand, launch_sign};
  return v;
}

}
```

corda_amd/csrc/verify_ed.hip:

```cpp
#include "ed_lds.h"
#include "keyws.h"

namespace cg {

__constant__ Ed25519Consts c_ed;

static const uint8_t ED_SPKI_PREFIX[12] = {0x30, 0x2a, 0x30, 0x05, 0x06, 0x03, 0x2b, 0x65, 0x70, 0x03, 0x21, 0x00};
static const uint8_t ED_SPKI_PREFIX_NULL[14] = {0x30, 0x2c, 0x30, 0x07, 0x06, 0x03, 0x2b,
                                                0x65, 0x70, 0x05, 0x00, 0x03, 0x21, 0x00};

__device__ __forceinline__ bool ed_key_locate(const cg_key& k, const uint8_t* arena, uint64_t arena_len,
                                              uint64_t& a_off) {
  const uint64_t lr = round4(arena_len);
  a_off = k.off;
  if (!in_arena(k.off, k.len, arena_len)) return false;
  if (k.fmt == CG_KEY_RAW) return k.len == 32;
  if (k.fmt != CG_KEY_SPKI) return false;
  if (k.len == 44) {
    for (int b = 0; b < 12; ++b)
      if ((cg_ld_bytes4(arena, lr, k.off + b) & 0xffu) != ED_SPKI_PREFIX[b]) return false;
    a_off = k.off + 12;
    return true;
  }
  if (k.len == 46) {
// ... 336 lines not shown
  const uint32_t beg = ranges[PLAN_ED], wbeg = ranges[PLAN_WIDE + PLAN_ED];
  for (Walk w = walk_units(ranges[PLAN_ED + 1] - beg); w.u < w.end; w.u += w.step)
    ed_hash_one<Fused>(beg + w.u, items, perm, hdr, arena, arena_len, msgs, msgs_len, mode, status, dig,
                       beg + w.u >= wbeg, ec);
}

struct PickGlobal {
  __device__ __forceinline__ void operator()(ge_niels& out, const ge_niels* row, int d) const { pick(out, row, d); }
};

#ifndef ED_LADDER_WAVES_PER_SIMD
#define ED_LADDER_WAVES_PER_SIMD 3
#endif


struct EdOps {
  static constexpr int kNa1 = (EdCfg::kDigits - 1 + ED_K - 1) / ED_K;
  static constexpr int kNa0 = (EdCfg::kDigits + ED_K - 1) / ED_K;
  static constexpr int kOps1 = kNa1;
  static constexpr int kOps = kNa1 + kNa0 + EdWideCfg::kBDigits;
  static constexpr uint32_t kWaveBytes = 64 * sizeof(ge_niels);
};
static_assert(ED_K == 2, "the flat op sequence is written for 2 windows");
static_assert(sizeof(ge_niels) == 120, "LDS chunking assumes 120-B niels entries");

__device__ __forceinline__ void ed_op_info(int o, int& widx, int& sh, bool& is_b, int& row) {
  if (o < EdOps::kNa1 + EdOps::kNa0) {
    const bool w1 = o < EdOps::kOps1;
    const int k = w1 ? o : o - EdOps::kOps1;
    const int t = ED_K * k + (w1 ? 1 : 0);
    widx = t >> 2;
    sh = (t & 3) * 8;
    is_b = false;
    row = k;
  } else {
    constexpr int per = 32 / EdWideCfg::kBBits;
    const int u = o - EdOps::kNa1 - EdOps::kNa0;
    widx = EdCfg::kPackedWords + u / per;
    sh = (u % per) * EdWideCfg::kBBits;
    is_b = true;
    row = u;
  }
}

__device__ __forceinline__ int ed_op_digit(uint32_t w, int sh, bool is_b) {
  if (!is_b) return (int)(int8_t)(uint8_t)(w >> sh);
  return EdWideCfg::kBBits == 16 ? (int)(int16_t)(uint16_t)(w >> sh) : (int)w;
}

__device__ __forceinline__ void ed_glds_niels(const ge_niels* src, uint32_t wave_lds_off) {
  const uint8_t* s = (const uint8_t*)src;
#pragma unroll
  for (int c = 0; c < 7; ++c)
    __builtin_amdgcn_global_load_lds((cg_gbl_ptr)(s + 16 * c), ed_lds_at(wave_lds_off, 64 * 16 * c), 16, 0, 0);
  __builtin_amdgcn_global_load_lds((cg_gbl_ptr)(s + 112), ed_lds_at(wave_lds_off, 64 * 112), 4, 0, 0);
  __builtin_amdgcn_global_load_lds((cg_gbl_ptr)(s + 116), ed_lds_at(wave_lds_off, 64 * 116), 4, 0, 0);
}

__device__ __forceinline__ void ed_lds_niels(ge_niels& n, const uint8_t* wave_lds, uint32_t lane) {
  uint32_t* d = (uint32_t*)&n;
#pragma unroll
  for (int c = 0; c < 7; ++c) {
    const uint4 v = *(const uint4*)(wave_lds + 64 * 16 * c + 16 * lane);
    d[4 * c] = v.x;
    d[4 * c + 1] = v.y;
    d[4 * c + 2] = v.z;
    d[4 * c + 3] = v.w;
  }
  d[28] = *(const uint32_t*)(wave_lds + 64 * 112 + 4 * lane);
  d[29] = *(const uint32_t*)(wave_lds + 64 * 116 + 4 * lane);
}

static_assert(64 * 7 * 16 <= EdOps::kWaveBytes, "the LDS image (7 chunks a lane) holds either entry form");

__device__ __forceinline__ const ge_niels* ed_op_src(const EdTab& TA, int row, int d) {
  const int a = d < 0 ? -d : d;
  return &TA.t[row][a > 0 ? a - 1 : 0];
}

__device__ __forceinline__ void ed_double_scalar_pf(ge_p2& out, const uint32_t* __restrict__ dw, const EdTab& TA,
                                                    const EdBWideTab& TB, uint8_t* wave_lds, uint32_t lane) {
  constexpr int N = EdOps::kOps, NA = EdOps::kNa1 + EdOps::kNa0;
  const uint32_t wl = __builtin_amdgcn_readfirstlane((uint32_t)(uintptr_t)(cg_lds_ptr)wave_lds);
  int widx, sh, row;
  bool is_b;
  ed_op_info(0, widx, sh, is_b, row);
  int d_cur = ed_op_digit(dw[widx], sh, is_b);
  ed_glds_niels(ed_op_src(TA, row, d_cur), wl);
  ed_op_info(1, widx, sh, is_b, row);
  uint32_t w_next = dw[widx];
  ge_p3 R;
  ge_p3_0(R);
  ge_p1p1 t;
  ge_p2 q;
  for (int o = 0; o < NA; ++o) {
    if (o == EdOps::kOps1) {
      for (int d = 0; d < ED_W - 1; ++d) {
        ge_p2_dbl(t, q);
        ge_p1p1_to_p2(q, t);
      }
      ge_p2_dbl(t, q);
      ge_p1p1_to_p3(R, t);
    }
    asm volatile("s_waitcnt vmcnt(0)" ::: "memory");
    ge_niels n;
    ed_lds_niels(n, wave_lds, lane);
    asm volatile("s_waitcnt lgkmcnt(0)" ::: "memory");
    if (d_cur == 0) ge_niels_identity(n);
    const bool neg = d_cur < 0;
    ed_op_info(o + 1, widx, sh, is_b, row);
    d_cur = ed_op_digit(w_next, sh, is_b);
    if (is_b) ed_glds_niels9(ed_b_src(TB, row, d_cur), wl);
    else ed_glds_niels(ed_op_src(TA, row, d_cur), wl);
    ed_op_info(o + 2, widx, sh, is_b, row);
    w_next = dw[widx];
    ge_madd_signed(t, R, n, neg);
    if (o + 1 == EdOps::kOps1) ge_p1p1_to_p2(q, t);
    else ge_p1p1_to_p3(R, t);
  }
  ge9_p3 R9;
  ge9_from_p3(R9, R);
  for (int o = NA; o < N; ++o) {
    asm volatile("s_waitcnt vmcnt(0)" ::: "memory");
    ge9_niels n;
    ed_lds_niels9(n, wave_lds, lane);
    asm volatile("s_waitcnt lgkmcnt(0)" ::: "memory");
    const bool neg = d_cur < 0;
    if (o + 1 < N) {
      ed_op_info(o + 1, widx, sh, is_b, row);
      d_cur = ed_op_digit(w_next, sh, is_b);
      ed_glds_niels9(ed_b_src(TB, row, d_cur), wl);
      if (o + 2 < N) {
        ed_op_info(o + 2, widx, sh, is_b, row);
        w_next = dw[widx];
      }
      ge9_madd_half<true>(R9, R9, n, neg);
    } else {
      ge9_madd_half<false>(R9, R9, n, neg);
    }
  }
  ge9_to_p2(out, R9);
}

#ifndef ED_LADDER_PF_WAVES
#define ED_LADDER_PF_WAVES 2
#endif
__global__ void __launch_bounds__(256, ED_LADDER_PF_WAVES) k_ed_ladder_pf(
    const cg_item* __restrict__ items, const uint32_t* __restrict__ perm, const uint32_t* __restrict__ ranges,
    const EdKeyHdr* __restrict__ hdr, const TabSlot* __restrict__ tabs, const EdBWideTab* __restrict__ btab,
    uint8_t* __restrict__ status, void* __restrict__ slots, EdCols ec) {
  __shared__ __attribute__((aligned(16))) uint8_t stage[4 * EdOps::kWaveBytes];
  const uint32_t beg = ranges[PLAN_FULL + PLAN_ED];
  uint8_t* wave_lds = stage + (threadIdx.x >> 6) * EdOps::kWaveBytes;
  for (Walk w = walk_units(ranges[PLAN_WIDE + PLAN_ED] - beg); w.u < w.end; w.u += w.step) {
    const uint64_t p = beg + w.u;
    const uint32_t key = ec.key[p];
    if (hdr[key].status != 0) {
      status[perm[p]] = CG_KEY_INVALID;
      ec.pend[p] = 0;
      continue;
    }
    if (!ec.pend[p]) continue;
    ge_p2 q;
    ed_double_scalar_pf(q, (const uint32_t*)((const uint8_t*)slots + (size_t)p * ITEM_SLOT), tabs[key].ed, *btab,
                        wave_lds, __lane_id());
    ((ge_p2*)slots)[p] = q;
  }
}

__device__ __forceinline__ void ed_wide_op(int o, int& widx, int& sh, bool& is_b, int& row) {
  is_b = o >= EdWideCfg::kRows;
  if (!is_b) {
    widx = o >> 2;
    sh = (o & 3) * 8;
    row = o;
  } else {
    constexpr int per = 32 / EdWideCfg::kBBits;
    const int u = o - EdWideCfg::kRows;
    widx = EdWideCfg::kPackedWords + u / per;
    sh = (u % per) * EdWideCfg::kBBits;
    row = u;
  }
}
__device__ __forceinline__ int ed_wide_digit(uint32_t w, int sh, bool is_b) {
  if (!is_b) return (int)(int8_t)(uint8_t)(w >> sh);
  return EdWideCfg::kBBits == 16 ? (int)(int16_t)(uint16_t)(w >> sh) : (int)w;
}

__device__ __forceinline__ const ge9_niels* ed_wide_src(const EdWideTab& TA, const EdBWideTab& TB, bool is_b, int row,
                                                        int d) {
  const int a = d < 0 ? -d : d;
  if (a == 0) return &TB.ident;
  return is_b ? &TB.t[row][a - 1] : &TA.t[row][a - 1];
}

__device__ __forceinline__ void ed_double_scalar_wide_pf(ge_p2& out, const uint32_t* __restrict__ dw,
                                                         const EdWideTab& TA, const EdBWideTab& TB, uint8_t* wave_lds,
                                                         uint32_t lane) {
  constexpr int N = EdWideCfg::kOps;
  const uint32_t wl = __builtin_amdgcn_readfirstlane((uint32_t)(uintptr_t)(cg_lds_ptr)wave_lds);
  int widx, sh, row;
  bool is_b;
  ed_wide_op(0, widx, sh, is_b, row);
  int d_cur = ed_wide_digit(dw[widx], sh, is_b);
  ed_glds_niels9(ed_wide_src(TA, TB, is_b, row, d_cur), wl);
  ed_wide_op(1, widx, sh, is_b, row);
  uint32_t w_next = dw[widx];
  ge9_p3 R;
  auto next = [&](int o, ge9_niels& n, bool& neg) {
    asm volatile("s_waitcnt vmcnt(0)" ::: "memory");
    ed_lds_niels9(n, wave_lds, lane);
    asm volatile("s_waitcnt lgkmcnt(0)" ::: "memory");
    neg = d_cur < 0;
    ed_wide_op(o + 1, widx, sh, is_b, row);
    d_cur = ed_wide_digit(w_next, sh, is_b);
    ed_glds_niels9(ed_wide_src(TA, TB, is_b, row, d_cur), wl);
    if (o + 2 < N) {
      ed_wide_op(o + 2, widx, sh, is_b, row);
      w_next = dw[widx];
    }
  };
  {
    ge9_niels n;
    bool neg;
    next(0, n, neg);
    ge9_from_niels_half(R, n, neg != (d_cur < 0));
  }
  for (int o = 1; o + 1 < N; ++o) {
    ge9_niels n;
    bool neg;
    next(o, n, neg);
    ge9_madd_half_flip<true>(R, R, n, neg != (d_cur < 0));
  }
  {
    asm volatile("s_waitcnt vmcnt(0)" ::: "memory");
    ge9_niels n;
    ed_lds_niels9(n, wave_lds, lane);
    ge9_madd_half_flip<false>(R, R, n, d_cur < 0);
  }
  ge9_to_p2(out, R);
}

#ifndef ED_LADDER_WIDE_WAVES
#define ED_LADDER_WIDE_WAVES ED_LADDER_PF_WAVES
#endif
#ifndef ED_LADDER_WIDE_OCC
#define ED_LADDER_WIDE_OCC 4
#endif
__global__ void __launch_bounds__(256, ED_LADDER_WIDE_WAVES) k_ed_ladder_wide(
    const cg_item* __restrict__ items, const uint32_t* __restrict__ perm, const uint32_t* __restrict__ ranges,
    const EdKeyHdr* __restrict__ hdr, const uint32_t* __restrict__ wide_idx, const EdWideSlot* __restrict__ wed,
    const EdBWideTab* __restrict__ btab, uint8_t* __restrict__ status, void* __restrict__ slots, EdCols ec) {
  __shared__ __attribute__((aligned(16))) uint8_t stage[4 * EdOps::kWaveBytes];
  const uint32_t beg = ranges[PLAN_WIDE + PLAN_ED];
  uint8_t* wave_lds = stage + (threadIdx.x >> 6) * EdOps::kWaveBytes;
  for (Walk w = walk_units(ranges[PLAN_ED + 1] - beg); w.u < w.end; w.u += w.step) {
    const uint64_t p = beg + w.u;
    const uint32_t key = ec.key[p];
    if (hdr[key].status != 0) {
      status[perm[p]] = CG_KEY_INVALID;
      ec.pend[p] = 0;
      continue;
    }
    if (!ec.pend[p]) continue;
    ge_p2 q;
    ed_double_scalar_wide_pf(q, (const uint32_t*)((const uint8_t*)slots + (size_t)p * ITEM_SLOT),
                             wed[wide_idx[key]].tab, *btab, wave_lds, __lane_id());
    ((ge_p2*)slots)[p] = q;
  }
}

template <int Mode>
__global__ void __launch_bounds__(256, ED_LADDER_WAVES_PER_SIMD) k_ed_ladder(
    const cg_item* __restrict__ items, const uint32_t* __restrict__ perm, const uint32_t* __restrict__ ranges,
    const EdKeyHdr* __restrict__ hdr, const TabSlot* __restrict__ tabs, const EdBWideTab* __restrict__ btab,
    uint8_t* __restrict__ status, void* __restrict__ slots, EdCols ec) {
  static_assert(Mode == PLAN_MODE_ROW0 || Mode == PLAN_MODE_QUART, "row-0 and quarter tables");
  const uint32_t beg = Mode == PLAN_MODE_QUART ? ranges[PLAN_QUART + PLAN_ED] : ranges[PLAN_ED];
  const uint32_t end = Mode == PLAN_MODE_QUART ? ranges[PLAN_FULL + PLAN_ED] : ranges[PLAN_QUART + PLAN_ED];
  for (Walk w = walk_units(end - beg); w.u < w.end; w.u += w.step) {
    const uint64_t p = beg + w.u;
    const uint32_t key = ec.key[p];
    if (hdr[key].status != 0) {
      status[perm[p]] = CG_KEY_INVALID;
      ec.pend[p] = 0;
      continue;
    }
    if (!ec.pend[p]) continue;
    const EdDigits d = ((const EdDigits*)slots)[p];
    ge_p2 q;
    if (Mode == PLAN_MODE_QUART) {
      ed_double_scalar_fw<ED_W, ED_QK>(q, d.eh, d.es, *(const EdQTab*)&tabs[key].ed, *btab, PickGlobal(),
                                       PickGlobal());
    } else {
      ed_double_scalar_row0w<ED_W, ED_K>(q, d.eh, d.es, tabs[key].ed.t[0], *btab, PickGlobal(), PickGlobal());
    }
    ((ge_p2*)slots)[p] = q;
  }
}

#ifndef ED_FINISH_K
#define ED_FINISH_K 16
#endif
__device__ __forceinline__ void ed_finish_one(uint64_t unit, uint32_t beg, uint32_t end,
                                              const uint32_t* __restrict__ perm, uint8_t* __restrict__ status,
                                              const ge_p2* __restrict__ rin, const EdCols& ec) {
  const uint64_t base = beg + (unit >> 6) * (64 * ED_FINISH_K) + (unit & 63);
  fe acc[ED_FINISH_K];
  fe run;
  fe_1(run);
  uint32_t pend = 0;
  for (uint32_t k = 0; k < ED_FINISH_K; ++k) {
    const uint64_t p = base + 64 * k;
    const bool pd = p < end && ec.pend[p];
    pend |= (uint32_t)pd << k;
    if (pd) fe_mul(run, run, rin[p].Z);
    fe_copy(acc[k], run);
  }
  if (!pend) return;
  fe inv;
  fe_invert(inv, run);
  for (int k = ED_FINISH_K - 1; k >= 0; --k) {
    if (!((pend >> k) & 1u)) continue;
    const uint64_t p = base + 64 * (uint32_t)k;
    const ge_p2 P = rin[p];
    fe zi, t;
    if (k > 0) fe_mul(zi, inv, acc[k - 1]);
    else fe_copy(zi, inv);
    fe_mul(t, inv, P.Z);
    fe_copy(inv, t);
    uint32_t rw[8];
#pragma unroll
    for (int w = 0; w < 8; ++w) rw[w] = ec.r[(size_t)w * ec.n + p];
    status[perm[p]] = (uint8_t)ed_encode_cmp(P, zi, rw);
  }
}

__global__ void __launch_bounds__(256) k_ed_finish(const uint32_t* __restrict__ perm,
                                                   const uint32_t* __restrict__ ranges, uint8_t* __restrict__ status,
                                                   const ge_p2* __restrict__ rin, EdCols ec) {
  const uint32_t beg = ranges[PLAN_ED], end = ranges[PLAN_ED + 1];
  const uint64_t units = ((uint64_t)(end - beg) + 64 * ED_FINISH_K - 1) / (64 * ED_FINISH_K) * 64;
  for (Walk w = walk_units(units); w.u < w.end; w.u += w.step)
    ed_finish_one(w.u, beg, end, perm, status, rin, ec);
}

hipError_t ed_upload_constants() {
  Ed25519Consts h;
  ed_consts_init(h);
  return hipMemcpyToSymbol(HIP_SYMBOL(c_ed), &h, sizeof h, 0, hipMemcpyHostToDevice);
}

hipError_t ed_init_const(void* d_btab, void* d_scratch, hipStream_t stream) {
  const uint32_t lanes = EdBCfgT::kDigits * (EdBCfgT::kMult / 8);
  hipLaunchKernelGGL(k_ed_btab_init, dim3((lanes + 63) / 64), dim3(64), 0, stream, (EdBTab*)d_btab);
  static_assert(EdWideCfg::kBDigits * sizeof(ge_p3) <= sizeof(EcRowScratch), "B row bases fit the scratch");
  ge_p3* bases = (ge_p3*)d_scratch;
  hipLaunchKernelGGL(k_ed_bwide_bases, dim3(1), dim3(64), 0, stream, bases);
  const uint64_t wlanes = (uint64_t)EdWideCfg::kBDigits * (EdWideCfg::kBMult / 8);
  hipLaunchKernelGGL(k_ed_bwide_init, dim3((unsigned)((wlanes + 63) / 64)), dim3(64), 0, stream,
                     (EdBWideTab*)bwide(d_btab), (const ge_p3*)bases);
  return hipGetLastError();
}

void ed_launch_key_abyte(const cg_key* d_keys, uint32_t n_keys, const uint8_t* d_arena, uint64_t arena_len,
                         const KeyWs& w, hipStream_t stream) {
  const uint32_t B = 64;
  hipLaunchKernelGGL(k_ed_key_abyte, dim3((n_keys + B - 1) / B), dim3(B), 0, stream, d_keys, n_keys, d_arena,
                     arena_len, w.hdr);
}

void ed_launch_keyprep_chains(const cg_key* d_keys, uint32_t n_keys, const uint8_t* d_arena, uint64_t arena_len,
                              const KeyWs& w, hipStream_t stream) {
  const uint32_t B = 64;
  hipLaunchKernelGGL(k_ed_keyprep_decode, dim3((n_keys + B - 1) / B), dim3(B), 0, stream, d_keys, n_keys, d_arena,
                     arena_len, w.hdr, w.bases);
  hipLaunchKernelGGL(k_ed_keyprep_chain, dim3((n_keys + B - 1) / B), dim3(B), 0, stream, n_keys, w.hdr,
                     (const uint32_t*)w.full, (const uint32_t*)w.quart, (const uint32_t*)w.full_count, w.bases);
  if (w.cap_ed)
    hipLaunchKernelGGL(k_ed_wide_chain, dim3((w.cap_ed + B - 1) / B), dim3(B), 0, stream, n_keys, w.hdr,
                       (const uint32_t*)w.wide, (const uint32_t*)w.wide_count, (const uint32_t*)w.wide_idx,
                       (const BaseSlot*)w.bases, w.wed);
}

void ed_launch_keyprep_tabs(const cg_key* d_keys, uint32_t n_keys, const KeyWs& w, hipStream_t stream, bool full,
                            bool wide) {
  const uint32_t B = 64;
  if (full)
    hipLaunchKernelGGL(k_ed_keyprep_tab, dim3(w.park_lanes_ed / B), dim3(B), 0, stream, n_keys, w.hdr, w.bases,
                       (const uint32_t*)w.row0, (const uint32_t*)w.full, (const uint32_t*)w.quart,
                       (const uint32_t*)w.full_count, w.tab, w.park_ed, w.park_lanes_ed);
  if (wide && w.cap_ed) {
    const uint64_t rl = (uint64_t)w.cap_ed * EdWideCfg::kRows;
    hipLaunchKernelGGL(k_ed_wide_rows, dim3((unsigned)((rl * ED_WIDE_ROW_LANES + B - 1) / B)), dim3(B), 0, stream,
                       n_keys, w.hdr, (const uint32_t*)w.wide, (const uint32_t*)w.wide_count,
                       (const uint32_t*)w.wide_idx, w.wed);
    kc_launch_commit(PLAN_ED, n_keys, w, stream);
  }
}

void ed_launch_front(const cg_item* d_items, uint64_t n_items, const uint8_t* d_arena, uint64_t arena_len,
                     uint32_t mode, uint8_t* d_status, const KeyWs& w, const uint8_t* d_msgs, uint64_t msgs_len,
                     const ItemWs& iw, hipStream_t stream) {
  const uint32_t B = 256;
  const unsigned grid = walk_grid(n_items, B, WALK_CAP(ED_HASH_WAVES_PER_SIMD));
  if (d_msgs)
    hipLaunchKernelGGL(k_ed_hash<true>, dim3(grid), dim3(B), 0, stream, d_items, iw.perm, iw.ranges, w.hdr, d_arena,
                       arena_len, d_msgs, msgs_len, mode, d_status, (EdDigits*)iw.slots, iw.ed);
  else
    hipLaunchKernelGGL(k_ed_hash<false>, dim3(grid), dim3(B), 0, stream, d_items, iw.perm, iw.ranges, w.hdr, d_arena,
                       arena_len, d_msgs, msgs_len, mode, d_status, (EdDigits*)iw.slots, iw.ed);
}

void ed_launch_ladder(bool full, const cg_item* d_items, uint64_t n_items, uint8_t* d_status, const KeyWs& w,
                      const ItemWs& iw, const void* d_btab, hipStream_t stream) {
  const uint32_t B = 256;
  const unsigned grid = walk_grid(n_items, B, WALK_CAP(full ? ED_LADDER_PF_WAVES : ED_LADDER_WAVES_PER_SIMD));
  if (full) {
    hipLaunchKernelGGL(k_ed_ladder_pf, dim3(grid), dim3(B), 0, stream, d_items, iw.perm, iw.ranges, w.hdr,
                       w.tab, bwide(d_btab), d_status, iw.slots, iw.ed);
  } else {
    hipLaunchKernelGGL(k_ed_ladder<PLAN_MODE_ROW0>, dim3(grid), dim3(B), 0, stream, d_items, iw.perm, iw.ranges,
                       w.hdr, w.tab, bwide(d_btab), d_status, iw.slots, iw.ed);
    hipLaunchKernelGGL(k_ed_ladder<PLAN_MODE_QUART>, dim3(grid), dim3(B), 0, stream, d_items, iw.perm, iw.ranges,
                       w.hdr, w.tab, bwide(d_btab), d_status, iw.slots, iw.ed);
  }
}

void ed_launch_ladder_wide(const cg_item* d_items, uint64_t n_items, uint8_t* d_status, const KeyWs& w,
                           const ItemWs& iw, const void* d_btab, hipStream_t stream) {
  const uint32_t B = 256;
  const unsigned grid = walk_grid(n_items, B, WALK_CAP(ED_LADDER_WIDE_OCC));
  hipLaunchKernelGGL(k_ed_ladder_wide, dim3(grid), dim3(B), 0, stream, d_items, iw.perm, iw.ranges, w.hdr,
                     (const uint32_t*)w.wide_idx, (const EdWideSlot*)w.wed, bwide(d_btab), d_status, iw.slots, iw.ed);
}

void ed_launch_finish(const cg_item* d_items, uint64_t n_items, const uint8_t* d_arena, uint64_t arena_len,
                      uint8_t* d_status, const ItemWs& iw, hipStream_t stream) {
  const uint32_t B = 256;
  const uint64_t units = (n_items + 64 * ED_FINISH_K - 1) / (64 * ED_FINISH_K) * 64;
  const unsigned fgrid = walk_grid(units, B, WALK_CAP(2));
  (void)d_items;
  (void)d_arena;
  (void)arena_len;
  hipLaunchKernelGGL(k_ed_finish, dim3(fgrid), dim3(B), 0, stream, iw.perm, iw.ranges, d_status, (const ge_p2*)iw.slots,
                     iw.ed);
}

}
```

Measured before the change: 463.3 million.

## Fuse plan-key and status writes into txsig item kernels, plus scan/LDS tweaks

The txsig item-building kernels now also compute each item's sort key, sort value and initial status, so the separate plan-key and misc-status kernels are skipped on the planned path. The single-block sig12 scan is rewritten to use wave shuffles instead of a serial-per-thread plus LDS Hillis-Steele scan. Key-use counting gets an LDS-binned variant for up to 8192 keys to cut global atomics. The template midstate kernel appears to be changed to a block-cooperative form, and the ed finish grid cap is lowered. Risks include more register pressure in the item kernels and correctness coupling between the item-build and plan stages.

New measurement: 459.8 million. No clear change (-0.8%).

```diff
diff --git a/corda_amd/csrc/cordagpu.cpp b/corda_amd/csrc/cordagpu.cpp
--- a/corda_amd/csrc/cordagpu.cpp
+++ b/corda_amd/csrc/cordagpu.cpp
@@ -347,7 +347,7 @@
 }
 
 struct ChunkOpts {
-  const std::function<hipError_t(uint64_t, uint64_t, uint64_t)>* prepare = nullptr;
+  const std::function<hipError_t(uint64_t, uint64_t, uint64_t, const cg::ItemPlan&)>* prepare = nullptr;
   const cg::KeyUses* uses = nullptr;
   bool prepare_blocks = false;
 };
@@ -363,6 +363,7 @@
   const std::vector<uint64_t>& bounds;
   const ChunkOpts& o;
   uint64_t half_bytes = 0;
+  bool two = false;
   bool closes_cache = true;
   Clock::time_point h0;
   double prep_ms = 0, front_ms = 0, back_ms = 0;
@@ -375,6 +376,7 @@
     a.n_items = bounds[k + 1] - bounds[k];
     a.d_status = r.d_status + bounds[k];
     a.d_item_ws = (uint8_t*)c->itemws.p + (size_t)half * half_bytes;
+    a.planned = o.prepare != nullptr;
     return a;
   }
   Error at(const char* w, Error e) {
@@ -386,7 +388,8 @@
   Error key_tables() { return c->eng->launch_key_tables(c->fork, s); }
   Error prepare(unsigned k) {
     h0 = Clock::now();
-    const hipError_t w = (*o.prepare)(k, bounds[k], bounds[k + 1] - bounds[k]);
+    const hipError_t w =
+        (*o.prepare)(k, bounds[k], bounds[k + 1] - bounds[k], c->eng->item_plan(chunk(k, two ? int(k & 1) : 0)));
     prep_ms = ms(h0, Clock::now());
     return w;
   }
@@ -436,6 +439,7 @@
   cgs::CallPlan p;
   p.chunks = (unsigned)(bounds.size() - 1);
   p.two = p.chunks > 1 && c->itemws.cap >= 2 * g.half_bytes;
+  g.two = p.two;
   p.hook = o.prepare != nullptr;
   p.hook_blocks = o.prepare_blocks;
   return cgs::chunked(g, p);
@@ -1240,16 +1244,16 @@
   if (d.n_tmpls) e = hipMemcpyAsync(c->tmpls.p, d.tmpls, sizeof(cg_signable_tmpl) * d.n_tmpls, hipMemcpyHostToDevice, s);
   if (e == hipSuccess)
     e = cg::launch_tx_sig_templates(dt, d.n_tmpls, d.arena, d.arena_len, slot, d.ids, d.n_ids, (uint8_t*)c->msgs.p, s);
-  const std::function<hipError_t(uint64_t, uint64_t, uint64_t)> prepare = [&](uint64_t k, uint64_t first,
-                                                                               uint64_t cnt) {
+  const std::function<hipError_t(uint64_t, uint64_t, uint64_t, const cg::ItemPlan&)> prepare =
+      [&](uint64_t k, uint64_t first, uint64_t cnt, const cg::ItemPlan& plan) {
     hipError_t r = p.ready ? (*p.ready)(k, first, cnt) : hipSuccess;
     if (r == hipSuccess && d.sigs.packed())
       r = cg::launch_tx_sig12_range((const cg_txsig_packed*)d.sigs.p, first, cnt, d.sig_bytes_off, d.sig_bytes_len,
                                     p.chunk_base ? (*p.chunk_base)[k] : 0, p.d_bases, dt, d.n_tmpls, d.n_ids,
-                                    d.arena_len, (cg_item*)c->txitems.p, c->sig12ws.p, s);
+                                    d.arena_len, (cg_item*)c->txitems.p, c->sig12ws.p, &plan, s);
     else if (r == hipSuccess)
       r = cg::launch_tx_sig_range((const cg_txsig*)d.sigs.p, first, cnt, dt, d.n_tmpls, nullptr, d.n_ids, d.ids,
-                                  d.arena_len, slot, (cg_item*)c->txitems.p, (uint8_t*)c->msgs.p, s);
+                                  d.arena_len, slot, (cg_item*)c->txitems.p, (uint8_t*)c->msgs.p, &plan, s);
     return r;
   };
   const cg::VerifyReq r = {d.keys, d.n_keys, (const cg_item*)c->txitems.p, d.n_sigs, d.arena, d.arena_len, d.mode,
diff --git a/corda_amd/csrc/engine.h b/corda_amd/csrc/engine.h
--- a/corda_amd/csrc/engine.h
+++ b/corda_amd/csrc/engine.h
@@ -107,6 +107,18 @@
   void* d_item_ws;
   const void* d_btab;
   const WidePool* wide;
+  bool planned = false;
+};
+
+struct ItemPlan {
+  const cg_key* keys;
+  uint32_t n_keys;
+  uint32_t kb;
+  const uint32_t* uses;
+  const uint32_t* wide_idx;
+  uint8_t* status;
+  uint32_t* skey;
+  uint32_t* sval;
 };
 
 struct KeyUses {
@@ -155,6 +167,7 @@
   hipError_t (*launch_items_plan)(const ItemArgs& a, hipStream_t stream, const Fork& fork);
   hipError_t (*launch_items_front)(const ItemArgs& a, hipStream_t stream, const Fork& fork, bool planned);
   hipError_t (*launch_items_back)(const ItemArgs& a, hipStream_t stream, const Fork& fork);
+  ItemPlan (*item_plan)(const ItemArgs& a);
   size_t (*signer_bytes)();
   size_t (*sign_ws_bytes)(uint64_t n);
   hipError_t (*launch_signer_expand)(const uint8_t* d_seeds, uint32_t n, void* d_signers, uint8_t* d_pubkeys,
@@ -169,6 +182,7 @@
 using cgt::EngineVariant;
 using cgt::Fork;
 using cgt::ItemArgs;
+using cgt::ItemPlan;
 using cgt::PendingTabs;
 using cgt::SignArgs;
 using cgt::SigTable;
@@ -236,7 +250,7 @@
 hipError_t launch_tx_sig_range(const cg_txsig* d_sigs, uint64_t first, uint64_t n, const cg_signable_tmpl* d_tmpls,
                                uint32_t n_tmpls, const uint8_t* d_tx_status, uint64_t n_tx, const uint8_t* d_ids,
                                uint64_t arena_len, uint64_t slot, cg_item* d_items, uint8_t* d_msgs,
-                               hipStream_t stream);
+                               const ItemPlan* plan, hipStream_t stream);
 
 size_t tx_sig12_scratch_bytes(uint64_t n);
 hipError_t launch_tx_sig12_bases(const cg_txsig_packed* d_sigs, uint64_t first, uint64_t n, uint64_t base,
@@ -245,7 +259,7 @@
                                  uint64_t sig_bytes_len, uint64_t base, const uint64_t* d_bases,
                                  const cg_signable_tmpl* d_tmpls,
                                  uint32_t n_tmpls, uint64_t n_tx, uint64_t arena_len, cg_item* d_items,
-                                 void* d_scratch, hipStream_t stream);
+                                 void* d_scratch, const ItemPlan* plan, hipStream_t stream);
 
 hipError_t launch_merkle_roots(const uint8_t* d_leaves, const uint64_t* d_first, const uint32_t* d_count,
                                uint64_t n, uint8_t* d_roots, uint8_t* d_status, uint8_t* d_ws,
diff --git a/corda_amd/csrc/keyws.h b/corda_amd/csrc/keyws.h
--- a/corda_amd/csrc/keyws.h
+++ b/corda_amd/csrc/keyws.h
@@ -249,6 +249,34 @@
 #ifndef ED_DIRECT_MAX_USES
 #define ED_DIRECT_MAX_USES 32u
 #endif
+CG_HD int item_first_status(uint32_t key_idx, const cg_key* __restrict__ keys, uint32_t n_keys) {
+  if (key_idx >= n_keys) return CG_NOT_RUN;
+  const uint8_t s = keys[key_idx].scheme;
+  if (s != CG_EDDSA_ED25519_SHA512 && s != CG_ECDSA_SECP256R1_SHA256 && s != CG_ECDSA_SECP256K1_SHA256)
+    return CG_UNSUPPORTED;
+  return s == CG_EDDSA_ED25519_SHA512 ? CG_NOT_RUN : -1;
+}
+CG_HD uint32_t item_plan_key(uint32_t key_idx, uint32_t msg_len, const cg_key* __restrict__ keys, uint32_t n_keys,
+                             uint32_t kb, const uint32_t* __restrict__ uses, const uint32_t* __restrict__ wide_idx) {
+  const uint32_t k = key_idx;
+  uint32_t c = PLAN_CLASSES;
+  if (k < n_keys) {
+    const uint8_t s = keys[k].scheme;
+    c = s == CG_EDDSA_ED25519_SHA512 ? PLAN_ED
+      : s == CG_ECDSA_SECP256R1_SHA256 ? PLAN_R1
+      : s == CG_ECDSA_SECP256K1_SHA256 ? PLAN_K1
+                                       : PLAN_CLASSES;
+  }
+  uint32_t mode = 0;
+  if (c < PLAN_CLASSES)
+    mode = wide_idx[k] != KEY_NOT_WIDE         ? PLAN_MODE_WIDE
+         : uses[k] >= ED_DIRECT_MAX_USES      ? PLAN_MODE_FULL
+         : uses[k] >= KEY_QUARTER_MIN_USES    ? PLAN_MODE_QUART
+                                              : PLAN_MODE_ROW0;
+  const uint32_t lng = msg_len > ITEM_LONG_MIN ? 1u : 0u;
+  return (c << kb) | (c < PLAN_CLASSES ? (mode << (kb - 2)) | (lng << (kb - 3)) | (k & ((1u << (kb - 3)) - 1u)) : 0u);
+}
+
 struct EdWideSlot {
   EdWideTab tab;
   ge_p3 bases[EdWideCfg::kRows];
@@ -398,7 +426,8 @@
          al256(8 * n * sizeof(uint32_t)) + al256(n * sizeof(uint32_t)) + al256(n);
 }
 hipError_t launch_plan(const cg_item* d_items, uint64_t n_items, const cg_key* d_keys, uint32_t n_keys,
-                       const KeyWs& w, const ItemWs& iw, hipStream_t stream);
+                       const KeyWs& w, const ItemWs& iw, bool keyed, hipStream_t stream);
+ItemPlan item_plan(const ItemArgs& a);
 
 #define EC_GTAB_LANES (EC_G_DIGITS * (EC_G_MULT / EC_MULT))
 #define EC_GWIDE_LANES (EC_WIDE_GDIGITS * (EC_WIDE_GMULT / EC_MULT))
diff --git a/corda_amd/csrc/plan_sort.hip b/corda_amd/csrc/plan_sort.hip
--- a/corda_amd/csrc/plan_sort.hip
+++ b/corda_amd/csrc/plan_sort.hip
@@ -22,24 +22,7 @@
                                                    uint32_t* __restrict__ skey, uint32_t* __restrict__ sval) {
   const uint64_t i = (uint64_t)blockIdx.x * blockDim.x + threadIdx.x;
   if (i >= n_items) return;
-  const uint32_t k = items[i].key_idx;
-  uint32_t c = PLAN_CLASSES;
-  if (k < n_keys) {
-    const uint8_t s = keys[k].scheme;
-    c = s == CG_EDDSA_ED25519_SHA512 ? PLAN_ED
-      : s == CG_ECDSA_SECP256R1_SHA256 ? PLAN_R1
-      : s == CG_ECDSA_SECP256K1_SHA256 ? PLAN_K1
-                                       : PLAN_CLASSES;
-  }
-  uint32_t mode = 0;
-  if (c < PLAN_CLASSES)
-    mode = wide_idx[k] != KEY_NOT_WIDE         ? PLAN_MODE_WIDE
-         : uses[k] >= ED_DIRECT_MAX_USES      ? PLAN_MODE_FULL
-         : uses[k] >= KEY_QUARTER_MIN_USES    ? PLAN_MODE_QUART
-                                              : PLAN_MODE_ROW0;
-  const uint32_t lng = items[i].msg_len > ITEM_LONG_MIN ? 1u : 0u;
-  skey[i] = (c << kb) |
-            (c < PLAN_CLASSES ? (mode << (kb - 2)) | (lng << (kb - 3)) | (k & ((1u << (kb - 3)) - 1u)) : 0u);
+  skey[i] = item_plan_key(items[i].key_idx, items[i].msg_len, keys, n_keys, kb, uses, wide_idx);
   sval[i] = (uint32_t)i;
 }
 
@@ -78,12 +61,20 @@
   return bytes;
 }
 
+ItemPlan item_plan(const ItemArgs& a) {
+  const KeyWs w = key_ws((void*)a.d_keyprep, a.n_keys, a.wide);
+  const ItemWs iw = item_ws(a.d_item_ws, a.n_items);
+  return {a.d_keys,   a.n_keys,   key_bits(a.n_keys) + 3, (const uint32_t*)w.uses, (const uint32_t*)w.wide_idx,
+          a.d_status, iw.skey_in, iw.sval_in};
+}
+
 hipError_t launch_plan(const cg_item* d_items, uint64_t n_items, const cg_key* d_keys, uint32_t n_keys,
-                       const KeyWs& w, const ItemWs& iw, hipStream_t stream) {
+                       const KeyWs& w, const ItemWs& iw, bool keyed, hipStream_t stream) {
   const uint32_t B = 256;
   const uint32_t kb = key_bits(n_keys) + 3;
-  hipLaunchKernelGGL(k_plan_keys, dim3((unsigned)((n_items + B - 1) / B)), dim3(B), 0, stream, d_items, n_items,
-                     d_keys, n_keys, kb, (const uint32_t*)w.uses, (const uint32_t*)w.wide_idx, iw.skey_in, iw.sval_in);
+  if (!keyed)
+    hipLaunchKernelGGL(k_plan_keys, dim3((unsigned)((n_items + B - 1) / B)), dim3(B), 0, stream, d_items, n_items,
+                       d_keys, n_keys, kb, (const uint32_t*)w.uses, (const uint32_t*)w.wide_idx, iw.skey_in, iw.sval_in);
   size_t bytes = iw.sort_temp_bytes;
   hipError_t e = rocprim::radix_sort_pairs<PlanSortConfig>(iw.sort_temp, bytes, (const uint32_t*)iw.skey_in, iw.skey_out,
                                            (const uint32_t*)iw.sval_in, iw.perm, (size_t)n_items, 0u, kb + 2,
diff --git a/corda_amd/csrc/txpipe.hip b/corda_amd/csrc/txpipe.hip
--- a/corda_amd/csrc/txpipe.hip
+++ b/corda_amd/csrc/txpipe.hip
@@ -10,10 +10,18 @@
   return in_arena(t.prefix_off, t.prefix_len, arena_len) && in_arena(t.suffix_off, t.suffix_len, arena_len);
 }
 
+__device__ __forceinline__ void item_plan_write(const cg_item& it, uint64_t at, const ItemPlan& p) {
+  const int st = item_first_status(it.key_idx, p.keys, p.n_keys);
+  if (st >= 0) p.status[at] = (uint8_t)st;
+  p.skey[at] = item_plan_key(it.key_idx, it.msg_len, p.keys, p.n_keys, p.kb, p.uses, p.wide_idx);
+  p.sval[at] = (uint32_t)at;
+}
+
+template <bool Plan>
 __global__ void __launch_bounds__(256) k_txsig_items(const cg_txsig* __restrict__ sigs, uint64_t first, uint64_t n_sigs,
                                                      const cg_signable_tmpl* __restrict__ tmpls, uint32_t n_tmpls,
                                                      const uint8_t* __restrict__ tx_status, uint64_t n_tx,
-                                                     uint64_t arena_len, cg_item* __restrict__ items) {
+                                                     uint64_t arena_len, cg_item* __restrict__ items, ItemPlan plan) {
   const uint64_t j = first + (uint64_t)blockIdx.x * blockDim.x + threadIdx.x;
   if (j >= first + n_sigs) return;
   const cg_txsig s = sigs[j];
@@ -41,6 +49,7 @@
     it.reserved0 = 0;
   }
   items[j] = it;
+  if (Plan) item_plan_write(it, j - first, plan);
 }
 
 #define SIG12_BLOCK 256
@@ -72,34 +81,56 @@
   }
 }
 
-__global__ void __launch_bounds__(1024) k_sig12_scan(uint64_t* __restrict__ sums, uint64_t nb, uint64_t base) {
-  __shared__ uint64_t sh[1024];
-  const uint32_t t = threadIdx.x;
-  const uint64_t per = (nb + 1023) / 1024, lo = t * per, hi = lo + per < nb ? lo + per : nb;
+__device__ __forceinline__ uint64_t wave_sum64(uint64_t v) {
+#pragma unroll
+  for (int d = 32; d >= 1; d >>= 1) {
+    const uint32_t lo = __shfl_xor((uint32_t)v, d, 64), hi = __shfl_xor((uint32_t)(v >> 32), d, 64);
+    v += ((uint64_t)hi << 32) | lo;
+  }
+  return v;
+}
+
+#define SIG12_SCAN_WAVES 16
+__global__ void __launch_bounds__(64 * SIG12_SCAN_WAVES) k_sig12_scan(uint64_t* __restrict__ sums, uint64_t nb,
+                                                                      uint64_t base) {
+  __shared__ uint64_t tot[SIG12_SCAN_WAVES];
+  const uint32_t wv = threadIdx.x >> 6, lane = threadIdx.x & 63;
+  const uint64_t run = ((nb + SIG12_SCAN_WAVES - 1) / SIG12_SCAN_WAVES + 63) & ~(uint64_t)63;
+  const uint64_t lo = wv * run < nb ? wv * run : nb, hi = lo + run < nb ? lo + run : nb;
+  constexpr int U = 8;
   uint64_t s = 0;
-  for (uint64_t i = lo; i < hi; ++i) s += sums[i];
-  sh[t] = s;
-  __syncthreads();
-  for (uint32_t d = 1; d < 1024; d <<= 1) {
-    const uint64_t u = t >= d ? sh[t - d] : 0;
-    __syncthreads();
-    sh[t] += u;
-    __syncthreads();
-  }
-  uint64_t run = base + sh[t] - s;
-  for (uint64_t i = lo; i < hi; ++i) {
-    const uint64_t x = sums[i];
-    sums[i] = run;
-    run += x;
-  }
-}
-
+  for (uint64_t i0 = lo + lane; i0 < hi; i0 += 64 * U) {
+    uint64_t x[U];
+#pragma unroll
+    for (int q = 0; q < U; ++q) x[q] = i0 + 64 * q < hi ? sums[i0 + 64 * q] : 0;
+#pragma unroll
+    for (int q = 0; q < U; ++q) s += x[q];
+  }
+  s = wave_sum64(s);
+  if (lane == 0) tot[wv] = s;
+  __syncthreads();
+  uint64_t at = base;
+  for (uint32_t w = 0; w < wv; ++w) at += tot[w];
+  for (uint64_t i0 = lo; i0 < hi; i0 += 64 * U) {
+    uint32_t x[U];
+#pragma unroll
+    for (int q = 0; q < U; ++q) x[q] = i0 + 64 * q + lane < hi ? (uint32_t)sums[i0 + 64 * q + lane] : 0u;
+#pragma unroll
+    for (int q = 0; q < U; ++q) {
+      const uint32_t incl = wave_incl_scan(x[q]);
+      if (i0 + 64 * q + lane < hi) sums[i0 + 64 * q + lane] = at + (incl - x[q]);
+      at += __shfl(incl, 63, 64);
+    }
+  }
+}
+
+template <bool Plan>
 __global__ void __launch_bounds__(SIG12_BLOCK) k_txsig12_items(const cg_txsig_packed* __restrict__ sigs, uint64_t first,
                                                                uint64_t n_sigs, const uint64_t* __restrict__ bases,
                                                                uint64_t sig_region, uint64_t sig_bytes_len,
                                                                const cg_signable_tmpl* __restrict__ tmpls,
                                                                uint32_t n_tmpls, uint64_t n_tx, uint64_t arena_len,
-                                                               cg_item* __restrict__ items) {
+                                                               cg_item* __restrict__ items, ItemPlan plan) {
   const uint64_t jj = (uint64_t)blockIdx.x * SIG12_BLOCK + threadIdx.x;
   const bool live = jj < n_sigs;
   cg_txsig_packed s = {0, 0, 0, 0};
@@ -136,6 +167,7 @@
     it.reserved0 = 0;
   }
   items[first + jj] = it;
+  if (Plan) item_plan_write(it, jj, plan);
 }
 
 size_t tx_sig12_scratch_bytes(uint64_t n) { return 8 * ((n + SIG12_BLOCK - 1) / SIG12_BLOCK + 1); }
@@ -145,7 +177,7 @@
   if (n == 0) return hipSuccess;
   const uint64_t nb = (n + SIG12_BLOCK - 1) / SIG12_BLOCK;
   hipLaunchKernelGGL(k_sig12_blocksum, dim3((unsigned)nb), dim3(SIG12_BLOCK), 0, stream, d_sigs, first, n, d_bases);
-  hipLaunchKernelGGL(k_sig12_scan, dim3(1), dim3(1024), 0, stream, d_bases, nb, base);
+  hipLaunchKernelGGL(k_sig12_scan, dim3(1), dim3(64 * SIG12_SCAN_WAVES), 0, stream, d_bases, nb, base);
   return hipGetLastError();
 }
 
@@ -153,7 +185,7 @@
                                  uint64_t sig_bytes_len, uint64_t base, const uint64_t* d_bases,
                                  const cg_signable_tmpl* d_tmpls,
                                  uint32_t n_tmpls, uint64_t n_tx, uint64_t arena_len, cg_item* d_items,
-                                 void* d_scratch, hipStream_t stream) {
+                                 void* d_scratch, const ItemPlan* plan, hipStream_t stream) {
   if (n == 0) return hipSuccess;
   const uint64_t* bases = d_bases ? d_bases + first / SIG12_BLOCK : (const uint64_t*)d_scratch;
   if (d_bases && first % SIG12_BLOCK) return hipErrorInvalidValue;
@@ -161,9 +193,13 @@
     const hipError_t e = launch_tx_sig12_bases(d_sigs, first, n, base, (uint64_t*)d_scratch, stream);
     if (e != hipSuccess) return e;
   }
-  hipLaunchKernelGGL(k_txsig12_items, dim3((unsigned)((n + SIG12_BLOCK - 1) / SIG12_BLOCK)), dim3(SIG12_BLOCK), 0,
-                     stream, d_sigs, first, n, bases, sig_region, sig_bytes_len, d_tmpls, n_tmpls, n_tx, arena_len,
-                     d_items);
+  const dim3 grid((unsigned)((n + SIG12_BLOCK - 1) / SIG12_BLOCK));
+  if (plan)
+    hipLaunchKernelGGL(k_txsig12_items<true>, grid, dim3(SIG12_BLOCK), 0, stream, d_sigs, first, n, bases, sig_region,
+                       sig_bytes_len, d_tmpls, n_tmpls, n_tx, arena_len, d_items, *plan);
+  else
+    hipLaunchKernelGGL(k_txsig12_items<false>, grid, dim3(SIG12_BLOCK), 0, stream, d_sigs, first, n, bases, sig_region,
+                       sig_bytes_len, d_tmpls, n_tmpls, n_tx, arena_len, d_items, ItemPlan{});
   return hipGetLastError();
 }
 
@@ -204,39 +240,40 @@
     for (int q = 0; q < 4; ++q) v |= byte_at(4ull * w + q) << (8 * q);
     img[w] = v;
   }
+  __shared__ uint32_t mw[64];
+  __syncthreads();
   const bool ed_mid = ok && tm.prefix_len >= TMPL_ED_MID_MIN_PREFIX;
+  if (threadIdx.x < 32) mw[threadIdx.x] = ed_mid ? __builtin_bswap32(img[16 + threadIdx.x]) : 0u;
+  __syncthreads();
   if (threadIdx.x == 1) {
     uint64_t* wk = ((TmplW512*)(msgs + tmpl_w512_off(n_tmpls)) + t)->wk;
     uint64_t w[16];
     for (int j = 0; j < 16; ++j) {
-      uint64_t v = 0;
-      for (int q = 0; q < 8; ++q) v = (v << 8) | (ed_mid ? byte_at(64ull + 8u * j + q) : 0u);
-      w[j] = v;
-      wk[j] = v + cg_k512(j);
+      w[j] = ((uint64_t)mw[2 * j] << 32) | mw[2 * j + 1];
+      wk[j] = w[j] + cg_k512(j);
     }
     for (int r = 16; r < 80; r += 16)
       for (int j = 0; j < 16; ++j) wk[r + j] = sha512_sched(w, j) + cg_k512(r + j);
   }
-  if (threadIdx.x != 0) return;
   TmplMid r;
   sha256_init(r.state);
   r.blocks = 0;
   r.prefix_len = tm.prefix_len;
   r.ed_mid = ed_mid ? 1u : 0u;
   r.pad = 0;
-  if (ok) {
-    for (uint32_t b = 0; b < tm.prefix_len / 64; ++b) {
+  const uint32_t nblk = ok ? tm.prefix_len / 64 : 0u;
+  for (uint32_t b0 = 0; b0 < nblk; b0 += 4) {
+    __syncthreads();
+    if (16 * b0 + threadIdx.x < 16 * nblk) mw[threadIdx.x] = __builtin_bswap32(img[16 * b0 + threadIdx.x]);
+    __syncthreads();
+    for (uint32_t b = b0; threadIdx.x == 0 && b < nblk && b < b0 + 4; ++b) {
       uint32_t w[16];
-      for (int j = 0; j < 16; ++j) {
-        uint32_t v = 0;
-        for (int q = 0; q < 4; ++q) v = (v << 8) | byte_at(64ull * b + 4u * j + q);
-        w[j] = v;
-      }
+      for (int j = 0; j < 16; ++j) w[j] = mw[16 * (b - b0) + j];
       sha256_compress(r.state, w);
       r.blocks = b + 1;
     }
   }
-  ((TmplMid*)(msgs + SPLICE_HDR_BYTES))[t] = r;
+  if (threadIdx.x == 0) ((TmplMid*)(msgs + SPLICE_HDR_BYTES))[t] = r;
 }
 
 hipError_t launch_tx_sig_templates(const cg_signable_tmpl* d_tmpls, uint32_t n_tmpls, const uint8_t* d_arena,
@@ -250,14 +287,19 @@
 hipError_t launch_tx_sig_range(const cg_txsig* d_sigs, uint64_t first, uint64_t n, const cg_signable_tmpl* d_tmpls,
                                uint32_t n_tmpls, const uint8_t* d_tx_status, uint64_t n_tx, const uint8_t* d_ids,
                                uint64_t arena_len, uint64_t slot, cg_item* d_items, uint8_t* d_msgs,
-                               hipStream_t stream) {
+                               const ItemPlan* plan, hipStream_t stream) {
   if (n == 0) return hipSuccess;
   const uint32_t B = 256;
   (void)d_ids;
   (void)slot;
   (void)d_msgs;
-  hipLaunchKernelGGL(k_txsig_items, dim3((unsigned)((n + B - 1) / B)), dim3(B), 0, stream, d_sigs, first, n, d_tmpls,
-                     n_tmpls, d_tx_status, n_tx, arena_len, d_items);
+  const dim3 grid((unsigned)((n + B - 1) / B));
+  if (plan)
+    hipLaunchKernelGGL(k_txsig_items<true>, grid, dim3(B), 0, stream, d_sigs, first, n, d_tmpls, n_tmpls, d_tx_status,
+                       n_tx, arena_len, d_items, *plan);
+  else
+    hipLaunchKernelGGL(k_txsig_items<false>, grid, dim3(B), 0, stream, d_sigs, first, n, d_tmpls, n_tmpls,
+                       d_tx_status, n_tx, arena_len, d_items, ItemPlan{});
   return hipGetLastError();
 }
 
@@ -269,7 +311,7 @@
   hipError_t e = launch_tx_sig_templates(d_tmpls, n_tmpls, d_arena, arena_len, slot, d_ids, n_tx, d_msgs, stream);
   if (e == hipSuccess)
     e = launch_tx_sig_range(d_sigs, 0, n_sigs, d_tmpls, n_tmpls, d_tx_status, n_tx, d_ids, arena_len, slot, d_items,
-                            d_msgs, stream);
+                            d_msgs, nullptr, stream);
   return e;
 }
 
diff --git a/corda_amd/csrc/verify.hip b/corda_amd/csrc/verify.hip
--- a/corda_amd/csrc/verify.hip
+++ b/corda_amd/csrc/verify.hip
@@ -6,16 +6,8 @@
                               uint32_t n_keys, uint8_t* __restrict__ status) {
   const uint64_t i = (uint64_t)blockIdx.x * blockDim.x + threadIdx.x;
   if (i >= n_items) return;
-  const uint32_t ki = items[i].key_idx;
-  if (ki >= n_keys) {
-    status[i] = CG_NOT_RUN;
-    return;
-  }
-  const uint8_t s = keys[ki].scheme;
-  if (s != CG_EDDSA_ED25519_SHA512 && s != CG_ECDSA_SECP256R1_SHA256 && s != CG_ECDSA_SECP256K1_SHA256)
-    status[i] = CG_UNSUPPORTED;
-  else if (s == CG_EDDSA_ED25519_SHA512)
-    status[i] = CG_NOT_RUN;
+  const int s = item_first_status(items[i].key_idx, keys, n_keys);
+  if (s >= 0) status[i] = (uint8_t)s;
 }
 
 __global__ void __launch_bounds__(256) k_key_init(uint32_t n_keys, uint32_t all, uint32_t* __restrict__ uses,
@@ -52,6 +44,41 @@
   if (k >= n_keys) return;
   seen[k] = 1;
   if (((uint32_t)i * 0x9E3779B1u) >> 30 == 0) atomicAdd(&uses[k], KEY_USES_SAMPLE);
+}
+
+#define KEY_USES_LDS_MAX 8192u
+#ifndef KEY_USES_LDS_BLOCKS
+#define KEY_USES_LDS_BLOCKS 256u
+#endif
+#define KEY_USES_LDS_LANES 1024u
+template <class Sig>
+__global__ void __launch_bounds__(KEY_USES_LDS_LANES) k_key_uses_txsig_lds(const Sig* __restrict__ sigs, uint64_t n,
+                                                                           uint32_t n_keys,
+                                                                           uint32_t* __restrict__ uses,
+                                                                           uint8_t* __restrict__ seen) {
+  __shared__ uint32_t bin[KEY_USES_LDS_MAX];
+  __shared__ uint32_t used[KEY_USES_LDS_MAX / 32];
+  for (uint32_t k = threadIdx.x; k < n_keys; k += KEY_USES_LDS_LANES) bin[k] = 0;
+  for (uint32_t k = threadIdx.x; k < (n_keys + 31) / 32; k += KEY_USES_LDS_LANES) used[k] = 0;
+  __syncthreads();
+  const uint64_t step = (uint64_t)gridDim.x * KEY_USES_LDS_LANES;
+  for (uint64_t i0 = (uint64_t)blockIdx.x * KEY_USES_LDS_LANES + threadIdx.x; i0 < n; i0 += 4 * step) {
+    uint32_t k[4];
+#pragma unroll
+    for (int q = 0; q < 4; ++q) k[q] = i0 + q * step < n ? sigs[i0 + q * step].key_idx : 0xffffffffu;
+#pragma unroll
+    for (int q = 0; q < 4; ++q) {
+      if (k[q] >= n_keys) continue;
+      const uint32_t bit = 1u << (k[q] & 31);
+      if (!(used[k[q] >> 5] & bit)) atomicOr(&used[k[q] >> 5], bit);
+      if (((uint32_t)(i0 + q * step) * 0x9E3779B1u) >> 30 == 0) atomicAdd(&bin[k[q]], 1u);
+    }
+  }
+  __syncthreads();
+  for (uint32_t k = threadIdx.x; k < n_keys; k += KEY_USES_LDS_LANES) {
+    if ((used[k >> 5] >> (k & 31)) & 1u) seen[k] = 1;
+    if (bin[k]) atomicAdd(&uses[k], bin[k] * KEY_USES_SAMPLE);
+  }
 }
 
 __global__ void __launch_bounds__(256) k_key_counts(const uint32_t* __restrict__ counts, uint32_t n_keys,
@@ -371,8 +398,16 @@
       case cgs::ST_KEY_USES_TXSIG:
         with_records(key->src->sigs, [&](auto* recs) {
           using Rec = std::remove_const_t<std::remove_pointer_t<decltype(recs)>>;
-          hipLaunchKernelGGL(k_key_uses_txsig<Rec>, dim3((unsigned)((key->src->n + 255) / 256)), dim3(256), 0, s, recs,
-                             key->src->n, key->r.n_keys, key->w.uses, key->w.seen);
+          const uint64_t n = key->src->n;
+          if (key->r.n_keys <= KEY_USES_LDS_MAX) {
+            const uint64_t nb = (n + KEY_USES_LDS_LANES - 1) / KEY_USES_LDS_LANES;
+            const unsigned grid = (unsigned)(nb < KEY_USES_LDS_BLOCKS ? nb : KEY_USES_LDS_BLOCKS);
+            hipLaunchKernelGGL(k_key_uses_txsig_lds<Rec>, dim3(grid), dim3(KEY_USES_LDS_LANES), 0, s, recs, n,
+                               key->r.n_keys, key->w.uses, key->w.seen);
+          } else {
+            hipLaunchKernelGGL(k_key_uses_txsig<Rec>, dim3((unsigned)((n + 255) / 256)), dim3(256), 0, s, recs, n,
+                               key->r.n_keys, key->w.uses, key->w.seen);
+          }
         });
         return kOk;
       case cgs::ST_KC_BEGIN:
@@ -414,12 +449,13 @@
         ed_launch_key_abyte(key->r.d_keys, key->r.n_keys, key->r.d_arena, key->r.arena_len, key->w, s);
         return kOk;
       case cgs::ST_MISC_STATUS:
+        if (a->planned) return kOk;
         hipLaunchKernelGGL(k_misc_status, dim3((unsigned)((a->n_items + 255) / 256)), dim3(256), 0, s, a->d_items,
                            a->n_items, a->d_keys, a->n_keys, a->d_status);
         return kOk;
       case cgs::ST_PLAN: {
         Error e = kOk;
-        CG_TIME(fork, CG_STAGE_PLAN, s, e = launch_plan(a->d_items, a->n_items, a->d_keys, a->n_keys, w, iw, s));
+        CG_TIME(fork, CG_STAGE_PLAN, s, e = launch_plan(a->d_items, a->n_items, a->d_keys, a->n_keys, w, iw, a->planned, s));
         return e;
       }
       case cgs::ST_MID_HOOK: return (*fork.mid_front)();
@@ -559,7 +595,7 @@
   static const EngineVariant v = {(uint32_t)ED_WIDE_BW, upload_constants, keyprep_bytes, wide_bytes, wide_slot_bytes,
                                   make_wide_pool, wide_slots, key_cache_bytes, btab_bytes, btab_scratch_bytes, init_btab, item_ws_bytes,
                                   launch_keyprep, launch_key_tables, launch_items, launch_items_plan,
-                                  launch_items_front, launch_items_back,
+                                  launch_items_front, launch_items_back, item_plan,
                                   signer_bytes, sign_ws_bytes, launch_signer_expand, launch_sign};
   return v;
 }
diff --git a/corda_amd/csrc/verify_ed.hip b/corda_amd/csrc/verify_ed.hip
--- a/corda_amd/csrc/verify_ed.hip
+++ b/corda_amd/csrc/verify_ed.hip
@@ -662,6 +662,9 @@
 #ifndef ED_FINISH_K
 #define ED_FINISH_K 16
 #endif
+#ifndef ED_FINISH_CAP
+#define ED_FINISH_CAP WALK_CAP(1)
+#endif
 __device__ __forceinline__ void ed_finish_one(uint64_t unit, uint32_t beg, uint32_t end,
                                               const uint32_t* __restrict__ perm, uint8_t* __restrict__ status,
                                               const ge_p2* __restrict__ rin, const EdCols& ec) {
@@ -799,7 +802,7 @@
                       uint8_t* d_status, const ItemWs& iw, hipStream_t stream) {
   const uint32_t B = 256;
   const uint64_t units = (n_items + 64 * ED_FINISH_K - 1) / (64 * ED_FINISH_K) * 64;
-  const unsigned fgrid = walk_grid(units, B, WALK_CAP(2));
+  const unsigned fgrid = walk_grid(units, B, ED_FINISH_CAP);
   (void)d_items;
   (void)d_arena;
   (void)arena_len;
```
